# NVlabs/FoundationPose

Hardware: AMD Instinct MI355X
Metric: pose-hypotheses/sec (raster+refine+score), 252 hyp x 160x160 @ 640x480 RGB-D (higher is better)
Workload: dtype f16

## Files before the change

foundationpose_amd/_lib.py:

```python
import ctypes as C
import os

import torch

_HERE = os.path.dirname(os.path.abspath(__file__))
LIB_PATH = os.environ.get("FP_AMD_LIB") or os.path.join(_HERE, "csrc", "libfp_amd.so")
ABI_VERSION = 226
_lib = None

vp, ci, cf, cd, sz = C.c_void_p, C.c_int, C.c_float, C.c_double, C.c_size_t

SIGNATURES = {
    "fp_last_error": (C.c_char_p, []),
    "fp_version": (ci, []),
    "fp_mesh_create": (ci, [vp, vp, vp, vp, vp, vp, vp, ci, ci, ci, ci, C.POINTER(vp)]),
    "fp_mesh_destroy": (None, [vp]),
    "fp_mesh_set_create": (ci, [vp, ci, C.POINTER(vp)]),
    "fp_mesh_set_destroy": (None, [vp]),
    "fp_mesh_set_workspace_bytes": (sz, [vp, ci, ci, ci]),
    "fp_depth_erode": (ci, [vp, vp, ci, ci, ci, cf, cf, cf, vp]),
    "fp_depth_bilateral": (ci, [vp, vp, ci, ci, ci, cf, cf, cf, vp]),
    "fp_depth_to_xyz": (ci, [vp, vp, cf, ci, vp, ci, ci, vp]),
    "fp_crop_windows": (ci, [vp, vp, cd, cd, ci, ci, ci, vp, vp, vp]),
    "fp_crop_windows_multi": (ci, [vp, vp, vp, vp, ci, cd, ci, ci, ci, vp, vp, vp]),
    "fp_depth_erode_frames": (ci, [vp, vp, ci, ci, ci, ci, cf, cf, cf, vp]),
    "fp_depth_bilateral_frames": (ci, [vp, vp, ci, ci, ci, ci, cf, cf, cf, vp]),
    "fp_depth_to_xyz_frames": (ci, [vp, vp, cf, ci, vp, ci, ci, ci, vp]),
    "fp_mask_depth_stats": (ci, [vp, vp, vp, ci, ci, ci, ci, cf, vp, vp]),
    "fp_crop_windows_views": (ci, [vp, vp, vp, ci, vp, vp, ci, cd, ci, ci, ci, vp, vp, vp]),
    "fp_render_crops_views": (ci, [vp, vp, vp, vp, vp, ci, vp, vp, ci, ci, ci, ci, ci, cf, cf, cf, ci, vp, vp, vp, vp, vp, vp, vp, vp, sz, vp]),
    "fp_warp_crops_views": (ci, [vp, vp, vp, vp, vp, vp, ci, vp, vp, vp, ci, ci, ci, ci, ci, ci, ci, ci, vp, vp]),
    "fp_pose_update_views": (ci, [vp, vp, vp, ci, ci, vp, cf, vp, vp, ci, ci, vp, vp, vp, ci, vp, vp, ci, vp, cf, vp]),
    "fp_depth_agreement": (ci, [vp, vp, vp, vp, ci, ci, ci, ci, ci, ci, cf, vp, vp]),
    "fp_icp_workspace_bytes": (sz, [ci, ci, ci]),
    "fp_icp_point_plane": (ci, [vp, vp, vp, vp, vp, ci, ci, ci, vp, ci, ci, ci, cf, cd, ci, vp, vp, vp, sz, vp]),
    "fp_pose_errors_workspace_bytes": (sz, [ci, ci, ci]),
    "fp_pose_errors": (ci, [vp, ci, vp, ci, vp, vp, vp, ci, ci, ci, vp, vp, sz, vp]),
    "fp_vsd_counts": (ci, [vp, vp, vp, ci, ci, ci, ci, vp, vp, ci, ci, ci, ci, cf, vp, ci, vp, vp]),
    "fp_mspd": (ci, [vp, ci, vp, ci, vp, vp, vp, ci, ci, vp, vp, vp]),
    "fp_tsdf_integrate": (ci, [vp, vp, vp, vp, vp, ci, ci, ci, ci, ci, ci, vp, cf, cf, cf, vp, vp, vp, vp, vp]),
    "fp_tsdf_count_triangles": (ci, [vp, vp, ci, ci, ci, cf, vp, vp]),
    "fp_tsdf_emit_triangles": (ci, [vp, vp, vp, vp, ci, ci, ci, vp, cf, cf, vp, C.c_longlong, vp, vp, vp, vp, vp]),
    "fp_texture_bake": (ci, [vp, ci, vp, ci, vp, vp, vp, vp, vp, vp, ci, ci, ci, ci, ci, cf, cf, cf, vp, vp, vp]),
    "fp_workspace_bytes": (sz, [ci, ci, ci, ci, ci]),
    "fp_raster_lds_bytes": (sz, [ci]),
    "fp_render_crops": (ci, [vp, vp, vp, vp, ci, ci, ci, ci, ci, cf, cf, cf, cf, ci, vp, vp, vp, vp, vp, vp, vp, vp, sz, vp]),
    "fp_render_crops_multi": (ci, [vp, vp, vp, vp, vp, vp, ci, ci, ci, ci, ci, cf, cf, cf, ci, vp, vp, vp, vp, vp, vp, vp, vp, sz, vp]),
    "fp_warp_crops": (ci, [vp, vp, vp, vp, vp, vp, cf, ci, ci, ci, ci, ci, ci, ci, vp, vp]),
    "fp_warp_crops_multi": (ci, [vp, vp, vp, vp, vp, vp, vp, vp, ci, ci, ci, ci, ci, ci, ci, ci, vp, vp]),
    "fp_pose_update": (ci, [vp, vp, vp, ci, ci, vp, cf, cf, ci, vp, vp, vp, ci, vp, vp, cf, vp]),
    "fp_pose_update_multi": (ci, [vp, vp, vp, ci, ci, vp, cf, vp, vp, ci, ci, vp, vp, vp, ci, vp, vp, cf, vp]),
    "fp_conv7x7s2_bn_relu_fwd": (ci, [vp, vp, vp, vp, vp, vp, ci, ci, ci, ci, vp]),
    "fp_igemm_f16_fwd": (ci, [vp, vp, vp, vp, vp, ci, ci, ci, ci, vp, vp]),
    "fp_pack_conv3x3_tiles_f16": (ci, [vp, vp, ci, ci, vp]),
    "fp_conv3x3_sw_lds_bytes": (ci, []),
    "fp_igemm_splitk_workspace_bytes": (sz, [ci, ci, ci]),
    "fp_igemm_f16_splitk_fwd": (ci, [vp, vp, vp, vp, vp, ci, ci, ci, ci, vp, ci, vp, sz, vp]),
    "fp_add_pe_f16_fwd": (ci, [vp, vp, vp, ci, ci, ci, vp]),
    "fp_replicate_rows_f16": (ci, [vp, vp, ci, ci, ci, ci, ci, C.c_longlong, vp]),
    "fp_replicate_segments_f16": (ci, [vp, vp, ci, ci, ci, ci, ci, C.c_longlong, vp]),
    "fp_layernorm_res_fwd": (ci, [vp, vp, vp, ci, vp, vp, vp, cf, vp, vp, ci, ci, vp]),
    "fp_pack_linear512_f16": (ci, [vp, vp, vp]),
    "fp_linear512_f16_fwd": (ci, [vp, vp, vp, vp, ci, ci, ci, vp]),
    "fp_linear_layernorm_fwd": (ci, [vp, vp, vp, vp, vp, vp, ci, vp, vp, cf, vp, vp, ci, ci, ci, ci, vp]),
    "fp_ffn_layernorm_mean_fwd": (ci, [vp, vp, vp, vp, vp, vp, vp, vp, cf, vp, vp, C.c_size_t, ci, ci, vp]),
    "fp_encoder_tail_workspace_bytes": (sz, [ci, ci]),
    "fp_encoder_tail_mean_fwd": (ci, [vp, ci, vp, vp, vp, vp, vp, vp, vp, vp, vp, vp, vp, vp, cf, vp, vp, sz, ci, ci, vp]),
    "fp_colmean_f16_fwd": (ci, [vp, vp, vp, vp, cf, vp, ci, ci, ci, vp]),
    "fp_rows_linear_fwd": (ci, [vp, vp, vp, vp, ci, ci, ci, ci, vp]),
    "fp_attention_f16_fwd": (ci, [vp, vp, ci, ci, ci, ci, ci, vp]),
    "fp_attention_segments_f16_fwd": (ci, [vp, vp, vp, ci, ci, ci, ci, ci, vp]),
    "fp_cluster_poses": (ci, [cf, cf, vp, ci, vp, ci, vp]),
}


class FpAmdError(RuntimeError):
    pass


def lib():
    global _lib
    if _lib is None:
        if not os.path.exists(LIB_PATH):
            raise FpAmdError(
                f"{LIB_PATH} is missing: the HIP extension is not built (run __graft_entry__.build() or "
                f"`make -C foundationpose_amd/csrc`). There is no CPU fallback.")
        handle = C.CDLL(LIB_PATH)
        for name, (res, args) in SIGNATURES.items():
            fn = getattr(handle, name)
            fn.restype = res
            fn.argtypes = args
        got = int(handle.fp_version())
        if got != ABI_VERSION:
            raise FpAmdError(f"{LIB_PATH} reports ABI version {got}, this binding was written for {ABI_VERSION}: rebuild the library "
                             f"(`make -C foundationpose_amd/csrc`) -- entry points changed meaning between versions (include/fp_amd.h)")
        _lib = handle
    return _lib


def check(status, what):
    if status != 0:
        msg = lib().fp_last_error()
        raise FpAmdError(f"{what} failed ({status}): {msg.decode() if msg else '?'}")
```

foundationpose_amd/csrc/conv_sw.hip:

```cpp
#include <hip/hip_fp16.h>
#include <stdlib.h>
#include <string.h>
#include <type_traits>
#include "igemm_common.h"
#include "igemm_epilogue.h"

#ifdef FP_PROFILE_BUILD
__device__ unsigned long long sw_dbg[8];
extern "C" int fp_dbg_conv_sw(unsigned long long* out, int reset) {
  if (reset) { unsigned long long z[8] = {0, 0, 0, 0, 0, 0, ~0ull, 0}; return (int)hipMemcpyToSymbol(HIP_SYMBOL(sw_dbg), z, sizeof(z)); }
  return (int)hipMemcpyFromSymbol(out, HIP_SYMBOL(sw_dbg), 8 * sizeof(unsigned long long));
}
extern "C" int fp_dbg_conv_sw_epilogue(unsigned long long* out, int reset) {
  if (reset) { unsigned long long z[8] = {0, 0, 0, 0, 0, 0, 0, 0}; return (int)hipMemcpyToSymbol(HIP_SYMBOL(ig_epi_dbg), z, sizeof(z)); }
  return (int)hipMemcpyFromSymbol(out, HIP_SYMBOL(ig_epi_dbg), 8 * sizeof(unsigned long long));
}
#define SW_CLK(t) const unsigned long long t = wall_clock64()
#else
#define SW_CLK(t)
#endif

#ifndef SW_DEFAULT_VARIANT
#define SW_DEFAULT_VARIANT 0
#endif

namespace {

constexpr int SW_BK = 32, SW_NSTW = 4;
constexpr int sw_prows(int BM) { return BM == 256 ? 512 : 768; }

template <int N>
__device__ __forceinline__ void sw_wait_vm() {
  static_assert(N >= 0 && N < 64, "vmcnt is a 6-bit field");
  asm volatile("s_waitcnt vmcnt(%0)" ::"n"(N) : "memory");
}

typedef float sw_float4 __attribute__((ext_vector_type(4)));
__device__ __forceinline__ void sw_mfma16(sw_float4& acc, const half8& a, const half8& b) {
  asm volatile("v_mfma_f32_16x16x32_f16 %0, %1, %2, %0" : "+v"(acc) : "v"(a), "v"(b));
}

__device__ __forceinline__ int sw_div(int n, unsigned mul, unsigned shr) { return (int)(__umulhi((unsigned)n, mul) >> shr); }

struct SwGeom {
  int HoWo, Wo, Hp, Wp;
  unsigned mulP, shrP, mulW, shrW;
};

template <typename G>
__device__ __forceinline__ int sw_q(const G& g, int m) {
  const int b = sw_div(m, g.mulP, g.shrP);
  const int r = m - b * g.HoWo;
  const int oy = sw_div(r, g.mulW, g.shrW);
  const int ox = r - oy * g.Wo;
  return (b * g.Hp + oy) * g.Wp + ox;
}

template <int BM, int BN, int TM, bool S16>
__global__ __launch_bounds__(512, 1) void k_conv_sw(IgemmParams p) {
  constexpr int BK = SW_BK, NW = 8, THREADS = 512;
  constexpr int NWN = BN / 64;
  static_assert((BM / (32 * TM)) * NWN == NW, "8 waves");
  constexpr int ROWB = BK * 2;
  constexpr int W_BYTES = BN * ROWB;
  constexpr int SW_PROWS = sw_prows(BM);
  constexpr int SW_PATCH_BYTES = SW_PROWS * ROWB;
  constexpr int WI = BN / 16 / NW;
  constexpr int PI = SW_PROWS / 16 / NW;
  static_assert(WI >= 1 && PI >= 1 && PI <= 7 && SW_PROWS == PI * 16 * NW, "tile shape");
  constexpr int STAGES_BYTES = 2 * SW_PATCH_BYTES + SW_NSTW * W_BYTES;
  constexpr int LDS_MAIN = ig_lds_main_slim<BM, BN>(STAGES_BYTES);
  auto swz = [](int row) { return (row >> 2) & 3; };
  auto swzp = [](int row) { return S16 ? (row >> 1) & 2 : (row >> 2) & 3; };
  extern __shared__ __attribute__((aligned(16))) unsigned char smem[];
  SW_CLK(t_start);
  unsigned char* const patch = smem;
  unsigned char* const wring = smem + 2 * SW_PATCH_BYTES;
  const int tid = threadIdx.x, lane = tid & 63;
  const int wid = __builtin_amdgcn_readfirstlane(tid >> 6);
  const int grp = wid >> 2;
  const int wm = wid / NWN, wn = wid - wm * NWN;
  float* bias_lds = reinterpret_cast<float*>(smem + LDS_MAIN);

  const _Float16* A_ = p.A;
  const _Float16* W_ = p.Wt;
  const _Float16* Wpk_ = p.Wpk;
  const float* bias_ = p.bias;
  const float* bnsc_ = p.bn_scale;
  const float* bnsh_ = p.bn_shift;
  const int M = p.M, N = p.N, Cin = p.Cin, cstride = p.in.cstride, coff = p.in.coff;
  const SwGeom gi = {p.in.HoWo, p.in.Wo, p.in.Hp, p.in.Wp, p.in.mulP, p.in.shrP, p.in.mulW, p.in.shrW};
  asm volatile("" ::"s"(A_), "s"(W_), "s"(Wpk_), "s"(bias_), "s"(bnsc_), "s"(bnsh_), "s"(M), "s"(N), "s"(Cin), "s"(cstride), "s"(coff),
               "s"(gi.HoWo), "s"(gi.Wo), "s"(gi.Hp), "s"(gi.Wp), "s"(gi.mulP), "s"(gi.shrP), "s"(gi.mulW), "s"(gi.shrW));
  __builtin_amdgcn_sched_barrier(0);

  const int tiles_n = N / BN;
  const int nwg = (int)(((unsigned)M + BM - 1) / BM) * tiles_n;
  const int xcd = blockIdx.x & 7, loc = blockIdx.x >> 3;
  const int qd8 = nwg >> 3, r8 = nwg & 7;
  const int tile = (xcd < r8 ? xcd * (qd8 + 1) : r8 * (qd8 + 1) + (xcd - r8) * qd8) + loc;
  const int bm = __builtin_popcount(tiles_n) == 1 ? tile >> __builtin_ctz(tiles_n) : tile / tiles_n, bn = tile - bm * tiles_n;
  const int m0 = bm * BM, n0 = bn * BN;
  const int Ktot = 9 * Cin, Wp = gi.Wp;
  const int ncc = Cin / BK;
  ig_bias_to_lds(bias_, bnsc_, bnsh_, N, n0, bias_lds, wid, lane);

  const int q0 = sw_q(gi, m0);
  const int qmax = sw_div(M, gi.mulP, gi.shrP) * gi.Hp * Wp - 1;
  unsigned poff32[PI], woff32[WI];
  {
    const int row0 = wid * PI * 16 + (lane >> 2);
    const int c = (lane & 3) ^ swzp(row0);
    static_assert(((16 >> 1) & 2) == 0 && ((16 >> 2) & 3) == 0, "swzp(row0 + 16 j) == swzp(row0)");
    const unsigned ps2 = (unsigned)cstride * 2, omax = (unsigned)qmax * ps2, lane_off = (unsigned)(coff + c * 8) * 2;
    const unsigned o0 = (unsigned)(q0 + row0) * ps2;
#pragma unroll
    for (int j = 0; j < PI; ++j) {
      const unsigned o = o0 + j * 16 * ps2;
      poff32[j] = (o < omax ? o : omax) + lane_off;
    }
  }
#pragma unroll
  for (int j = 0; j < WI; ++j) {
    const int row = (wid * WI + j) * 16 + (lane >> 2);
    const int c = (lane & 3) ^ swz(row);
    woff32[j] = (unsigned)((((size_t)(n0 + row) * Ktot) + c * 8) * 2);
  }
  const bool wpk = (BN == 128) && Wpk_ != nullptr;
  if (wpk) {
#pragma unroll
    for (int j = 0; j < WI; ++j) woff32[j] = (unsigned)(((wid * WI + j) * 64 + lane) * 16);
  }
  const int wpk_base = wpk ? bn * (ncc * 9) * W_BYTES : 0;
  const __amdgpu_buffer_rsrc_t rsA = __builtin_amdgcn_make_buffer_rsrc(const_cast<_Float16*>(A_), 0, 0x7FFFFFFF, 0x00020000);
  const __amdgpu_buffer_rsrc_t rsW = __builtin_amdgcn_make_buffer_rsrc(const_cast<_Float16*>(wpk ? Wpk_ : W_), 0, 0x7FFFFFFF, 0x00020000);

  auto stage_patch = [&](int cc, int j) {
    unsigned char* dst = patch + (cc & 1) * SW_PATCH_BYTES + (wid * PI + j) * 1024;
    __builtin_amdgcn_raw_ptr_buffer_load_lds(rsA, (__attribute__((address_space(3))) void*)dst, 16, (int)poff32[j],
                                             cc * (BK * 2), 0, 0);
  };
  auto stage_w = [&](int cc, int tap, int slot) {
    const int wsoff = wpk ? wpk_base + (cc * 9 + tap) * W_BYTES : (tap * Cin + cc * BK) * 2;
    unsigned char* dst = wring + slot * W_BYTES + wid * (WI * 1024);
#pragma unroll
    for (int j = 0; j < WI; ++j)
      __builtin_amdgcn_raw_ptr_buffer_load_lds(rsW, (__attribute__((address_space(3))) void*)(dst + j * 1024), 16,
                                               (int)woff32[j], wsoff, 0, 0);
  };

#pragma unroll
  for (int j = 0; j < PI; ++j) stage_patch(0, j);
  stage_w(0, 0, 0);
  stage_w(0, 1, 1);
  stage_w(0, 2, 2);
  __builtin_amdgcn_sched_barrier(0);
  SW_CLK(t_issue);

  constexpr int NFA = S16 ? 2 * TM : TM, NFW = S16 ? 4 : 2;
  constexpr int FR = S16 ? 16 : 32;
  typedef float float4_ __attribute__((ext_vector_type(4)));
  typedef typename std::conditional<S16, float4_, float16_>::type acc_t;
  acc_t acc[NFW][NFA];
#pragma unroll
  for (int i = 0; i < NFW; ++i)
#pragma unroll
    for (int j = 0; j < NFA; ++j)
#pragma unroll
      for (int e = 0; e < (S16 ? 4 : 16); ++e) acc[i][j][e] = 0.f;

  const int frow = lane & (FR - 1), fhalf = lane >> (S16 ? 4 : 5);
  int arow[NFA], w_off[2][2];
#pragma unroll
  for (int t = 0; t < NFA; ++t) {
    int m = m0 + wm * (32 * TM) + t * FR + frow;
    m = m < M ? m : M - 1;
    arow[t] = sw_q(gi, m) - q0;
    if constexpr (S16) arow[t] = (arow[t] << 6) + (fhalf << 4);
  }
  if constexpr (S16) {
    const int quad = (0x1320 >> (4 * (frow >> 2))) & 3;
#pragma unroll
    for (int t = 0; t < 4; ++t) {
      const int rw = wn * 64 + t * 16 + 4 * quad + (frow & 3);
      w_off[t >> 1][t & 1] = rw * ROWB + ((fhalf ^ swz(rw)) << 4);
    }
  } else {
#pragma unroll
    for (int t = 0; t < 2; ++t) {
      const int rw = wn * 64 + t * 32 + frow;
#pragma unroll
      for (int kk = 0; kk < 2; ++kk) w_off[t][kk] = rw * ROWB + (((2 * kk + fhalf) ^ swz(rw)) << 4);
    }
  }
  static_assert(TM == 4, "the fragment addresses of the next tap are computed behind the MFMA groups of a k-step, one per group of four");
  int anext[NFA], aflip[NFA];
#pragma unroll
  for (int t = 0; t < NFA; ++t) {
    anext[t] = S16 ? arow[t] : (arow[t] << 6) + ((fhalf ^ swz(arow[t])) << 4);
    aflip[t] = S16 ? (arow[t] >> 3) & 32 : 0;
  }

#pragma unroll
  for (int t = 0; t < NFA; ++t) {
    asm volatile("" : "+v"(arow[t]), "+v"(anext[t]));
    if constexpr (S16) asm volatile("" : "+v"(aflip[t]));
  }
  asm volatile("" : "+v"(w_off[0][0]), "+v"(w_off[0][1]), "+v"(w_off[1][0]), "+v"(w_off[1][1]));
#pragma unroll
  for (int i = 0; i < NFW; ++i)
#pragma unroll
    for (int j = 0; j < NFA; ++j) asm volatile("" : "+v"(acc[i][j]));
  __builtin_amdgcn_sched_barrier(0);

  sw_wait_vm<2 * WI>();
  __builtin_amdgcn_s_barrier();
  SW_CLK(t_cold);
  if (grp) __builtin_amdgcn_s_barrier();

  half8 fa[2][TM], fw[2][2];
  auto kstep = [&](int cc, auto tap_c, auto last_c) {
    constexpr int T = decltype(tap_c)::value;
    constexpr bool LAST = decltype(last_c)::value;
    constexpr int ky = T / 3, kx = T - 3 * ky;
    const int s = cc * 9 + T;
    const unsigned char* pb = patch + (cc & 1) * SW_PATCH_BYTES;
    const unsigned char* wb = wring + (s & (SW_NSTW - 1)) * W_BYTES;
    const int shift = ky * Wp + kx;
    if constexpr (S16) {
#pragma unroll
      for (int t = 0; t < NFA; ++t) fa[t >> 2][t & 3] = *reinterpret_cast<const half8*>(pb + (anext[t] ^ aflip[t]));
#pragma unroll
      for (int t = 0; t < 4; ++t) fw[t >> 1][t & 1] = *reinterpret_cast<const half8*>(wb + w_off[t >> 1][t & 1]);
    } else {
#pragma unroll
      for (int t = 0; t < TM; ++t) {
        const int a0 = anext[t];
        fa[0][t] = *reinterpret_cast<const half8*>(pb + a0);
        fa[1][t] = *reinterpret_cast<const half8*>(pb + (a0 ^ 32));
      }
#pragma unroll
      for (int kk = 0; kk < 2; ++kk)
#pragma unroll
        for (int t = 0; t < 2; ++t) fw[kk][t] = *reinterpret_cast<const half8*>(wb + w_off[t][kk]);
    }
    (void)shift;
    if constexpr (!LAST) {
      if constexpr (T < PI) stage_patch(cc + 1, T);
      if constexpr (T + 3 < 9) stage_w(cc, T + 3, (s + 3) & (SW_NSTW - 1));
      else stage_w(cc + 1, T - 6, (s + 3) & (SW_NSTW - 1));
      constexpr int NP = (T < PI ? 1 : 0) + ((T >= 1 && T - 1 < PI) ? 1 : 0);
      sw_wait_vm<2 * WI + NP>();
    } else {
      if constexpr (T + 3 < 9) stage_w(cc, T + 3, (s + 3) & (SW_NSTW - 1));
      constexpr int NYOUNGER = T <= 5 ? 2 : (T == 6 ? 1 : 0);
      sw_wait_vm<NYOUNGER * WI>();
    }
    asm volatile("s_waitcnt lgkmcnt(0)" ::: "memory");
    __builtin_amdgcn_sched_barrier(0);
    __builtin_amdgcn_s_barrier();
    __builtin_amdgcn_sched_barrier(0);
    __builtin_amdgcn_s_setprio(1);
    {
      constexpr int TN = (T + 1) % 9, kyn = TN / 3, kxn = TN - 3 * kyn;
      const int shift_n = kyn * Wp + kxn;
      if constexpr (S16) {
        int sh = shift_n << 6;
        asm volatile("" : "+s"(sh));
#pragma unroll
        for (int i = 0; i < 4; ++i)
#pragma unroll
          for (int jh = 0; jh < 2; ++jh) {
            const int t = i * 2 + jh;
            int x, y;
            sw_mfma16(acc[i][jh * 4 + 0], fw[i >> 1][i & 1], fa[jh][0]);
            asm volatile("v_add_u32 %0, %1, %2" : "=v"(x) : "s"(sh), "v"(arow[t]));
            sw_mfma16(acc[i][jh * 4 + 1], fw[i >> 1][i & 1], fa[jh][1]);
            asm volatile("v_lshrrev_b32 %0, 3, %1" : "=v"(y) : "v"(x));
            sw_mfma16(acc[i][jh * 4 + 2], fw[i >> 1][i & 1], fa[jh][2]);
            asm volatile("v_and_b32 %0, 32, %0" : "+v"(y));
            sw_mfma16(acc[i][jh * 4 + 3], fw[i >> 1][i & 1], fa[jh][3]);
            anext[t] = x; aflip[t] = y;
          }
      } else {
#pragma unroll
      for (int kk = 0; kk < 2; ++kk)
#pragma unroll
        for (int i = 0; i < 2; ++i) {
#pragma unroll
          for (int j = 0; j < TM; ++j)
            acc[i][j] = __builtin_amdgcn_mfma_f32_32x32x16_f16(fw[kk][i], fa[kk][j], acc[i][j], 0, 0, 0);
          const int t = kk * 2 + i;
          {
            int ar = arow[t];
            asm volatile("" : "+v"(ar));
            const int pr = ar + shift_n;
            anext[t] = (pr << 6) + ((fhalf ^ swz(pr)) << 4);
          }
        }
      }
    }
    __builtin_amdgcn_s_setprio(0);
    __builtin_amdgcn_sched_barrier(0);
    __builtin_amdgcn_s_barrier();
    __builtin_amdgcn_sched_barrier(0);
  };
  auto chunk = [&](int cc, auto last_c) {
    kstep(cc, std::integral_constant<int, 0>{}, last_c);
    kstep(cc, std::integral_constant<int, 1>{}, last_c);
    kstep(cc, std::integral_constant<int, 2>{}, last_c);
    kstep(cc, std::integral_constant<int, 3>{}, last_c);
    kstep(cc, std::integral_constant<int, 4>{}, last_c);
    kstep(cc, std::integral_constant<int, 5>{}, last_c);
    kstep(cc, std::integral_constant<int, 6>{}, last_c);
    kstep(cc, std::integral_constant<int, 7>{}, last_c);
    kstep(cc, std::integral_constant<int, 8>{}, last_c);
  };
  for (int cc = 0; cc + 1 < ncc; ++cc) chunk(cc, std::false_type{});
  chunk(ncc - 1, std::true_type{});
  if (!grp) __builtin_amdgcn_s_barrier();
  __syncthreads();
  SW_CLK(t_loop);
  ig_epilogue<BM, BN, TM, THREADS, 0, true>(p, acc, smem, m0, n0, wm, wn, tid, lane, bias_lds);
#ifdef FP_PROFILE_BUILD
  asm volatile("s_waitcnt vmcnt(0)" ::: "memory");
  SW_CLK(t_end);
  if (tid == 0) {
    atomicAdd(&sw_dbg[0], t_cold - t_start); atomicAdd(&sw_dbg[1], t_loop - t_cold); atomicAdd(&sw_dbg[2], t_end - t_loop);
    atomicAdd(&sw_dbg[3], 1ull); atomicAdd(&sw_dbg[4], t_issue - t_start); atomicMin(&sw_dbg[6], t_start); atomicMax(&sw_dbg[7], t_end);
  }
#endif
}

constexpr int LS_PROWS = 448, LS_NSTW = 3;

template <int BM, int BN, int TM>
__global__ __launch_bounds__(256, 2) void k_conv_sw_ls(IgemmParams p) {
  constexpr int BK = SW_BK, NW = 4, THREADS = 256;
  constexpr int NWN = BN / 64;
  static_assert((BM / (32 * TM)) * NWN == NW, "4 waves");
  constexpr int ROWB = BK * 2;
  constexpr int W_BYTES = BN * ROWB;
  constexpr int PATCH_BYTES = LS_PROWS * ROWB;
  constexpr int WI = BN / 16 / NW;
  constexpr int PI = LS_PROWS / 16 / NW;
  static_assert(WI >= 1 && PI >= 1 && PI <= 8 && LS_PROWS == PI * 16 * NW, "tile shape");
  constexpr int STAGES_BYTES = 2 * PATCH_BYTES + LS_NSTW * W_BYTES;
  static_assert(STAGES_BYTES >= BM * BN * 2 + BM * 16 + IG_BIAS_LDS, "the epilogue tile, its tables and the vectors reuse the staging area");
  auto swz = [](int row) { return (row >> 2) & 3; };
  extern __shared__ __attribute__((aligned(16))) unsigned char smem[];
  unsigned char* const patch = smem;
  unsigned char* const wring = smem + 2 * PATCH_BYTES;
  const int tid = threadIdx.x, lane = tid & 63;
  const int wid = __builtin_amdgcn_readfirstlane(tid >> 6);
  const int wm = wid / NWN, wn = wid - wm * NWN;

  const int tiles_n = p.N / BN;
  const int nwg = gridDim.x;
  const int xcd = blockIdx.x & 7, loc = blockIdx.x >> 3;
  const int qd8 = nwg >> 3, r8 = nwg & 7;
  const int tile = (xcd < r8 ? xcd * (qd8 + 1) : r8 * (qd8 + 1) + (xcd - r8) * qd8) + loc;
  const int bm = tile / tiles_n, bn = tile - bm * tiles_n;
  const int m0 = bm * BM, n0 = bn * BN;
  const int Cin = p.Cin, Ktot = 9 * Cin, Wp = p.in.Wp;
  const int ncc = Cin / BK;

  const int q0 = sw_q(p.in, m0);
  const int qmax = (p.M / p.in.HoWo) * p.in.Hp * Wp - 1;
  unsigned poff32[PI], woff32[WI];
#pragma unroll
  for (int j = 0; j < PI; ++j) {
    const int row = (wid * PI + j) * 16 + (lane >> 2);
    const int c = (lane & 3) ^ swz(row);
    int q = q0 + row;
    q = q < qmax ? q : qmax;
    poff32[j] = (unsigned)(((long long)q * p.in.cstride + p.in.coff + c * 8) * 2);
  }
#pragma unroll
  for (int j = 0; j < WI; ++j) {
    const int row = (wid * WI + j) * 16 + (lane >> 2);
    const int c = (lane & 3) ^ swz(row);
    woff32[j] = (unsigned)((((size_t)(n0 + row) * Ktot) + c * 8) * 2);
  }
  const __amdgpu_buffer_rsrc_t rsA = __builtin_amdgcn_make_buffer_rsrc(const_cast<_Float16*>(p.A), 0, 0x7FFFFFFF, 0x00020000);
  const __amdgpu_buffer_rsrc_t rsW = __builtin_amdgcn_make_buffer_rsrc(const_cast<_Float16*>(p.Wt), 0, 0x7FFFFFFF, 0x00020000);

  auto stage_patch = [&](int cc, int j) {
    unsigned char* dst = patch + (cc & 1) * PATCH_BYTES + (wid * PI + j) * 1024;
    __builtin_amdgcn_raw_ptr_buffer_load_lds(rsA, (__attribute__((address_space(3))) void*)dst, 16, (int)poff32[j],
                                             cc * (BK * 2), 0, 0);
  };
  auto stage_w = [&](int cc, int tap, int slot) {
    const int wsoff = (tap * Cin + cc * BK) * 2;
    unsigned char* dst = wring + slot * W_BYTES + wid * (WI * 1024);
#pragma unroll
    for (int j = 0; j < WI; ++j)
      __builtin_amdgcn_raw_ptr_buffer_load_lds(rsW, (__attribute__((address_space(3))) void*)(dst + j * 1024), 16,
                                               (int)woff32[j], wsoff, 0, 0);
  };

  float16_ acc[2][TM];
#pragma unroll
  for (int i = 0; i < 2; ++i)
#pragma unroll
    for (int j = 0; j < TM; ++j)
#pragma unroll
      for (int e = 0; e < 16; ++e) acc[i][j][e] = 0.f;

  const int frow = lane & 31, fhalf = lane >> 5;
  int arow[TM], w_off[2][2];
#pragma unroll
  for (int t = 0; t < TM; ++t) {
    int m = m0 + wm * (32 * TM) + t * 32 + frow;
    m = m < p.M ? m : p.M - 1;
    arow[t] = sw_q(p.in, m) - q0;
  }
#pragma unroll
  for (int t = 0; t < 2; ++t) {
    const int rw = wn * 64 + t * 32 + frow;
#pragma unroll
    for (int kk = 0; kk < 2; ++kk) w_off[t][kk] = rw * ROWB + (((2 * kk + fhalf) ^ swz(rw)) << 4);
  }

#pragma unroll
  for (int j = 0; j < PI; ++j) stage_patch(0, j);
  stage_w(0, 0, 0);
  stage_w(0, 1, 1);

  auto kstep = [&](int cc, auto tap_c, auto last_c, auto first_c) {
    constexpr int T = decltype(tap_c)::value;
    constexpr bool LAST = decltype(last_c)::value;
    constexpr bool FIRST = decltype(first_c)::value;
    constexpr int ky = T / 3, kx = T - 3 * ky;
    {
      constexpr bool prev_w = FIRST || T == 0 || !LAST || (T - 1) + 2 < 9;
      constexpr bool prev_p = !FIRST && T >= 1 && !LAST && (T - 1) < PI;
      sw_wait_vm<(prev_w ? WI : 0) + (prev_p ? 1 : 0)>();
    }
    __builtin_amdgcn_sched_barrier(0);
    __builtin_amdgcn_s_barrier();
    __builtin_amdgcn_sched_barrier(0);
    if constexpr (!LAST) {
      if constexpr (T < PI) stage_patch(cc + 1, T);
      if constexpr (T + 2 < 9) stage_w(cc, T + 2, (T + 2) % LS_NSTW);
      else stage_w(cc + 1, T - 7, (T + 2) % LS_NSTW);
    } else {
      if constexpr (T + 2 < 9) stage_w(cc, T + 2, (T + 2) % LS_NSTW);
    }
    const unsigned char* pb = patch + (cc & 1) * PATCH_BYTES;
    const unsigned char* wb = wring + (T % LS_NSTW) * W_BYTES;
    const int shift = ky * Wp + kx;
    half8 fa[2][TM], fw[2][2];
    int a0[TM];
#pragma unroll
    for (int t = 0; t < TM; ++t) {
      int ar = arow[t];
      asm volatile("" : "+v"(ar));
      const int pr = ar + shift;
      a0[t] = (pr << 6) + ((fhalf ^ swz(pr)) << 4);
    }
#pragma unroll
    for (int t = 0; t < TM; ++t) fa[0][t] = *reinterpret_cast<const half8*>(pb + a0[t]);
#pragma unroll
    for (int t = 0; t < 2; ++t) fw[0][t] = *reinterpret_cast<const half8*>(wb + w_off[t][0]);
#pragma unroll
    for (int t = 0; t < TM; ++t) fa[1][t] = *reinterpret_cast<const half8*>(pb + (a0[t] ^ 32));
#pragma unroll
    for (int t = 0; t < 2; ++t) fw[1][t] = *reinterpret_cast<const half8*>(wb + w_off[t][1]);
    __builtin_amdgcn_sched_barrier(0);
#pragma unroll
    for (int kk = 0; kk < 2; ++kk)
#pragma unroll
      for (int i = 0; i < 2; ++i)
#pragma unroll
        for (int j = 0; j < TM; ++j)
          acc[i][j] = __builtin_amdgcn_mfma_f32_32x32x16_f16(fw[kk][i], fa[kk][j], acc[i][j], 0, 0, 0);
    __builtin_amdgcn_sched_barrier(0);
  };
  auto chunk = [&](int cc, auto last_c, auto first_c) {
    kstep(cc, std::integral_constant<int, 0>{}, last_c, first_c);
    kstep(cc, std::integral_constant<int, 1>{}, last_c, std::false_type{});
    kstep(cc, std::integral_constant<int, 2>{}, last_c, std::false_type{});
    kstep(cc, std::integral_constant<int, 3>{}, last_c, std::false_type{});
    kstep(cc, std::integral_constant<int, 4>{}, last_c, std::false_type{});
    kstep(cc, std::integral_constant<int, 5>{}, last_c, std::false_type{});
    kstep(cc, std::integral_constant<int, 6>{}, last_c, std::false_type{});
    kstep(cc, std::integral_constant<int, 7>{}, last_c, std::false_type{});
    kstep(cc, std::integral_constant<int, 8>{}, last_c, std::false_type{});
  };
  chunk(0, std::false_type{}, std::true_type{});
  for (int cc = 1; cc + 1 < ncc; ++cc) chunk(cc, std::false_type{}, std::false_type{});
  chunk(ncc - 1, std::true_type{}, std::false_type{});
  __syncthreads();
  float* bias_lds = reinterpret_cast<float*>(smem + BM * BN * 2 + BM * 16);
  ig_bias_to_lds(p, n0, bias_lds, wid, lane);
  asm volatile("s_waitcnt vmcnt(0)" ::: "memory");
  ig_epilogue<BM, BN, TM, THREADS, 0>(p, acc, smem, m0, n0, wm, wn, tid, lane, bias_lds);
}

template <int BM, int BN, int TM>
int sw_ls_launch(const IgemmParams& p, hipStream_t stream) {
  constexpr int LDS = 2 * LS_PROWS * SW_BK * 2 + LS_NSTW * BN * SW_BK * 2;
  static_assert(2 * LDS <= 160 * 1024, "two workgroups per CU");
  const long long tiles = (long long)fp_cdiv(p.M, BM) * (p.N / BN);
  FP_REQUIRE(tiles < (1ll << 31), "fp_igemm_f16_fwd: too many tiles");
  FP_SET_MAX_LDS((k_conv_sw_ls<BM, BN, TM>), LDS);
  hipLaunchKernelGGL((k_conv_sw_ls<BM, BN, TM>), dim3((unsigned)tiles), dim3(256), LDS, stream, p);
  FP_CHECK_LAUNCH("fp_igemm_f16_fwd(conv_sw_ls)");
  return FP_OK;
}

constexpr int sw_lds_bytes(int BM, int BN) {
  return (BM == 256 ? ig_lds_main_slim<256, 256>(2 * sw_prows(256) * SW_BK * 2 + SW_NSTW * 256 * SW_BK * 2)
                    : ig_lds_main_slim<512, 128>(2 * sw_prows(512) * SW_BK * 2 + SW_NSTW * 128 * SW_BK * 2)) + IG_BIAS_LDS;
}

template <int BM, int BN, int TM, bool S16>
int sw_launch(const IgemmParams& p, hipStream_t stream) {
  static_assert((BM == 256 && BN == 256) || (BM == 512 && BN == 128), "tile shapes of sw_lds_bytes");
  constexpr int LDS = sw_lds_bytes(BM, BN);
  static_assert(LDS <= 160 * 1024, "does not fit the 160 KiB LDS");
  const long long tiles = (long long)fp_cdiv(p.M, BM) * (p.N / BN);
  FP_REQUIRE(tiles < (1ll << 31), "fp_igemm_f16_fwd: too many tiles");
  FP_SET_MAX_LDS((k_conv_sw<BM, BN, TM, S16>), LDS);
  hipLaunchKernelGGL((k_conv_sw<BM, BN, TM, S16>), dim3((unsigned)tiles), dim3(512), LDS, stream, p);
  FP_CHECK_LAUNCH("fp_igemm_f16_fwd(conv_sw)");
  return FP_OK;
}

}

static int sw_span(const IgemmGeom& g, int BM) {
  const int row_cross = (BM - 1) / g.Wo + 1, img_cross = (BM - 1) / g.HoWo + 1;
  return (BM - 1) + 2 * row_cross + (2 * g.Wp + 2) * img_cross + 2 * g.Wp + 3;
}

static int sw_variant(const IgemmParams& p) {
  int v = SW_DEFAULT_VARIANT;
#ifdef FP_PROFILE_BUILD
  static int forced = -2;
  if (forced == -2) {
    const char* e = getenv("FP_CONV_SW");
    forced = e ? (!strcmp(e, "ls") ? 1 : (!strcmp(e, "pp") ? 0 : -1)) : -1;
  }
  if (forced >= 0) v = forced;
#endif
  if (v == 2) v = p.Cin <= 128 ? 1 : 0;
  if (v == 3) v = p.Cin <= 256 ? 1 : 0;
  if (v == 1 && sw_span(p.in, 256) > LS_PROWS) v = 0;
  return v;
}

#ifndef SW_FORCE_512
#define SW_FORCE_512 1
#endif
static bool sw_use_256(const IgemmParams& p) { return (p.N % 256) == 0 && (!SW_FORCE_512 || p.M < 2 * 512); }
static int sw_tile_rows(const IgemmParams& p) { return sw_variant(p) == 1 ? 256 : (sw_use_256(p) ? 256 : 512); }

bool fp_conv3x3_sw_applicable(const IgemmParams& p) {
  const IgemmGeom& g = p.in;
  if (p.taps != 9 || g.stride != 1 || g.off != 0 || g.bsplit != 0) return false;
  if (g.HoWo % g.Wo != 0 || g.Wp != g.Wo + 2 || g.Hp != g.HoWo / g.Wo + 2) return false;
  if (g.Wo < 2) return false;
  const int BM = sw_tile_rows(p);
  if (p.M % g.HoWo != 0 || p.M < 2 * BM) return false;
  if (p.Cin % 64 != 0 || p.N % 128 != 0) return false;
  const long long bytes = (long long)(p.M / g.HoWo) * g.Hp * g.Wp * g.cstride * 2;
  if (bytes >= (1ll << 31)) return false;
  if (g.cstride >= (1 << 19)) return false;
  const IgemmGeom& o = p.out;
  const long long imgs = o.bsplit > 0 ? o.bsplit : p.M / g.HoWo, groups = o.bsplit > 0 ? (p.M / g.HoWo) / o.bsplit + 1 : 0;
  if (imgs * o.Hp * o.Wp * o.cstride + o.coff + groups * (long long)o.cgroup >= (1ll << 31)) return false;
  if (p.R) {
    const IgemmGeom& r = p.res;
    const long long rimgs = r.bsplit > 0 ? r.bsplit : p.M / g.HoWo, rgroups = r.bsplit > 0 ? (p.M / g.HoWo) / r.bsplit + 1 : 0;
    if (rimgs * r.Hp * r.Wp * r.cstride + r.coff + rgroups * (long long)r.cgroup >= (1ll << 31)) return false;
  }
  return sw_span(g, BM) <= (sw_variant(p) == 1 ? LS_PROWS : sw_prows(BM));
}

int fp_conv3x3_sw_tile_rows(const IgemmParams& p) { return sw_tile_rows(p); }

extern "C" int fp_conv3x3_sw_lds_bytes(void) { return sw_lds_bytes(512, 128); }

int fp_conv3x3_sw_launch(const IgemmParams& p, hipStream_t stream) {
  if (sw_variant(p) == 1) return sw_ls_launch<256, 128, 4>(p, stream);
  if (sw_use_256(p)) return p.mfma16 ? sw_launch<256, 256, 4, true>(p, stream) : sw_launch<256, 256, 4, false>(p, stream);
  return p.mfma16 ? sw_launch<512, 128, 4, true>(p, stream) : sw_launch<512, 128, 4, false>(p, stream);
}

__global__ __launch_bounds__(256) void k_pack_conv3x3_tiles(const _Float16* __restrict__ w, _Float16* __restrict__ out, int N, int Cin) {
  const int nk = 9 * (Cin / 32);
  const long long total = (long long)N * nk * 4;
  const long long q = (long long)blockIdx.x * 256 + threadIdx.x;
  if (q >= total) return;
  const int pc = (int)(q & 3);
  const int r = (int)((q >> 2) & 127);
  const long long blk = q >> 9;
  const int s = (int)(blk % nk), bn = (int)(blk / nk);
  const int cc = s / 9, tap = s - 9 * cc;
  const int lc = pc ^ ((r >> 2) & 3);
  const half8 v = *reinterpret_cast<const half8*>(w + (size_t)(bn * 128 + r) * (9 * Cin) + tap * Cin + cc * 32 + lc * 8);
  *reinterpret_cast<half8*>(out + q * 8) = v;
}

extern "C" int fp_pack_conv3x3_tiles_f16(const void* w, void* w_tiles, int N, int Cin, void* stream) {
  FP_REQUIRE(w && w_tiles && w != w_tiles, "fp_pack_conv3x3_tiles_f16: NULL tensor or in-place repack");
  FP_REQUIRE(N > 0 && N % 128 == 0 && Cin > 0 && Cin % 32 == 0, "fp_pack_conv3x3_tiles_f16: N=%d must be a multiple of 128, Cin=%d of 32", N, Cin);
  FP_REQUIRE((((size_t)w | (size_t)w_tiles) & 15) == 0, "fp_pack_conv3x3_tiles_f16: tensors must be 16-byte aligned");
  const long long total = (long long)N * 9 * (Cin / 32) * 4;
  hipLaunchKernelGGL(k_pack_conv3x3_tiles, dim3((unsigned)((total + 255) / 256)), dim3(256), 0, (hipStream_t)stream, (const _Float16*)w,
                     (_Float16*)w_tiles, N, Cin);
  FP_CHECK_LAUNCH("fp_pack_conv3x3_tiles_f16");
  return FP_OK;
}
```

foundationpose_amd/csrc/igemm.hip:

```cpp
#include <hip/hip_fp16.h>
#include <stdlib.h>
#include <string.h>
#include "igemm_common.h"
#include "igemm_epilogue.h"

int fp_igemm_pp_launch(const IgemmParams& p, int variant, hipStream_t stream);
int fp_conv3x3_sw_launch(const IgemmParams& p, hipStream_t stream);
bool fp_conv3x3_sw_applicable(const IgemmParams& p);
int fp_conv3x3_sw_tile_rows(const IgemmParams& p);

template <int BM, int BN, int TM, int NST, int BK, bool SPLITK = false>
__global__ __launch_bounds__((BM / (32 * TM)) * (BN / 64) * 64, ((BM / (32 * TM)) * (BN / 64) == 4 && TM == 4) ? 2 : 1) void k_igemm_f16(IgemmParams p) {
  constexpr int NWN = BN / 64;
  constexpr int NW = (BM / (32 * TM)) * NWN;
  constexpr int THREADS = NW * 64;
  constexpr int ROWB = BK * 2;
  constexpr int CPK = BK / 8;
  constexpr int RPI = 1024 / ROWB;
  constexpr int KK = BK / 16;
  constexpr int A_BYTES = BM * ROWB;
  constexpr int STAGE_BYTES = A_BYTES + BN * ROWB;
  constexpr int AI = BM / RPI / NW;
  constexpr int WI = BN / RPI / NW;
  static_assert(AI >= 1 && WI >= 1, "tile too small for this wave count");
// ... 163 lines not shown
  typedef _Float16 half2_ __attribute__((ext_vector_type(2)));
  const size_t t = (size_t)blockIdx.x * 256 + threadIdx.x;
  const int lane = (int)(t & 63);
  size_t q = t >> 6;
  const int j = (int)(q % TM); q /= TM;
  const int g = (int)(q & 3); q >>= 2;
  const int i = (int)(q & 1); q >>= 1;
  const int wid = (int)(q % NW);
  const int tile = (int)(q / NW);
  if (tile >= ntiles) return;
  const int tiles_n = p.N / BN;
  const int bm = tile / tiles_n, bn = tile - bm * tiles_n;
  const int wm = wid / NWN, wn = wid - wm * NWN;
  const int m = bm * BM + wm * (32 * TM) + j * 32 + (lane & 31);
  const int n = bn * BN + wn * 64 + i * 32 + 8 * g + 4 * (lane >> 5);
  if (m >= p.M) return;
  const float4_* src = reinterpret_cast<const float4_*>(p.slab) + t;
  const size_t per_split = (size_t)ntiles * NW * (8 * TM) * 64;
  float4_ a = src[0];
  for (int s = 1; s < p.nsplit; ++s) {
    const float4_ b = src[(size_t)s * per_split];
    a[0] += b[0]; a[1] += b[1]; a[2] += b[2]; a[3] += b[3];
  }
  float4_ bv = {0.f, 0.f, 0.f, 0.f};
  if (p.bias) bv = *reinterpret_cast<const float4_*>(p.bias + n);
  half4 v;
  if (p.round_acc) {
    const half2_ b01 = {(_Float16)bv[0], (_Float16)bv[1]}, b23 = {(_Float16)bv[2], (_Float16)bv[3]};
    half2_ t01 = {(_Float16)a[0], (_Float16)a[1]};
    half2_ t23 = {(_Float16)a[2], (_Float16)a[3]};
    t01 = t01 + b01;
    t23 = t23 + b23;
    if (p.bn_scale) {
      const float4_ sc = *reinterpret_cast<const float4_*>(p.bn_scale + n), sh = *reinterpret_cast<const float4_*>(p.bn_shift + n);
      v[0] = (_Float16)fmaf((float)t01[0], sc[0], sh[0]);
      v[1] = (_Float16)fmaf((float)t01[1], sc[1], sh[1]);
      v[2] = (_Float16)fmaf((float)t23[0], sc[2], sh[2]);
      v[3] = (_Float16)fmaf((float)t23[1], sc[3], sh[3]);
    } else {
      v[0] = t01[0]; v[1] = t01[1]; v[2] = t23[0]; v[3] = t23[1];
    }
  } else {
#pragma unroll
    for (int e = 0; e < 4; ++e) v[e] = (_Float16)(a[e] + bv[e]);
  }
  if (p.R) v = v + *reinterpret_cast<const half4*>(p.R + ig_row_off(p.res, m) + n);
  if (p.relu) {
    const half4 zero = {0, 0, 0, 0};
    v = __builtin_elementwise_max(v, zero);
  }
  *reinterpret_cast<half4*>(p.Y + ig_row_off(p.out, m) + n) = v;
  if (p.Ype) {
    const float4_ e0 = *reinterpret_cast<const float4_*>(p.pe + (size_t)(m % p.pe_period) * p.N + n);
    half4 w;
#pragma unroll
    for (int e = 0; e < 4; ++e) w[e] = (_Float16)((float)v[e] + e0[e]);
    *reinterpret_cast<half4*>(p.Ype + (size_t)m * p.N + n) = w;
  }
}

constexpr int SK_BM = 128, SK_BN = 128, SK_TM = 2, SK_NST = 2, SK_BK = 64;
static size_t ig_splitk_bytes(int M, int N, int splits) {
  return (size_t)splits * fp_cdiv(M, SK_BM) * (N / SK_BN) * (size_t)(SK_BM * SK_BN * 4);
}
static int ig_launch_splitk(const IgemmParams& p, hipStream_t stream) {
  constexpr int LDS = ig_lds_main<SK_BM, SK_BN>(SK_NST * (SK_BM + SK_BN) * SK_BK * 2) + IG_BIAS_LDS;
  const long long tiles = (long long)fp_cdiv(p.M, SK_BM) * (p.N / SK_BN);
  FP_REQUIRE(tiles * p.nsplit < (1ll << 31) && p.nsplit <= 65535, "fp_igemm_f16_splitk_fwd: too many tiles");
  FP_SET_MAX_LDS((k_igemm_f16<SK_BM, SK_BN, SK_TM, SK_NST, SK_BK, true>), LDS);
  hipLaunchKernelGGL((k_igemm_f16<SK_BM, SK_BN, SK_TM, SK_NST, SK_BK, true>), dim3((unsigned)tiles, (unsigned)p.nsplit), dim3(256), LDS, stream, p);
  FP_CHECK_LAUNCH("fp_igemm_f16_splitk_fwd(partial products)");
  const long long threads = tiles * 4 * (8 * SK_TM) * 64;
  hipLaunchKernelGGL((k_splitk_epilogue<SK_BM, SK_BN, SK_TM>), dim3((unsigned)((threads + 255) / 256)), dim3(256), 0, stream, p, (int)tiles);
  FP_CHECK_LAUNCH("fp_igemm_f16_splitk_fwd(reduce + epilogue)");
  return FP_OK;
}

static int ig_check_geom(const fp_igemm_geom* g, const char* what, const char* who) {
  FP_REQUIRE(g->pixels_per_image > 0 && g->width > 0 && g->padded_h > 0 && g->padded_w > 0 && g->cstride > 0 &&
                 g->stride > 0 && g->offset >= 0 && g->coff >= 0 && g->bsplit >= 0,
             "%s: bad %s geometry", who, what);
  FP_REQUIRE((g->cstride % 8) == 0 && (g->coff % 8) == 0 && (g->cgroup % 8) == 0,
             "%s: %s channel stride/offset must be multiples of 8 (16-byte rows)", who, what);
  return FP_OK;
}

static IgemmGeom ig_geom(const fp_igemm_geom* g) {
  IgemmGeom o;
  o.HoWo = g->pixels_per_image; o.Wo = g->width; o.Hp = g->padded_h; o.Wp = g->padded_w; o.stride = g->stride;
  o.off = g->offset; o.cstride = g->cstride; o.coff = g->coff; o.bsplit = g->bsplit; o.cgroup = g->cgroup;
  ig_fastdiv_init(o.HoWo, &o.mulP, &o.shrP);
  ig_fastdiv_init(o.Wo, &o.mulW, &o.shrW);
  ig_fastdiv_init(o.bsplit, &o.mulB, &o.shrB);
  return o;
}

static int ig_dispatch(IgemmParams& p, hipStream_t stream) {
  int sel = 0;
#ifdef FP_PROFILE_BUILD
  static int forced = -1;
  if (forced < 0) {
    const char* e = getenv("FP_IGEMM_TILE");
    forced = 0;
    if (e) {
      if (!strcmp(e, "128x128")) forced = 1;
      else if (!strcmp(e, "256x128")) forced = 2;
      else if (!strcmp(e, "256x256")) forced = 3;
      else if (!strcmp(e, "ls256x128")) forced = 4;
      else if (!strcmp(e, "pp256x256")) forced = 7;
      else if (!strcmp(e, "pp256x128")) forced = 9;
      else if (!strcmp(e, "generic")) forced = 100;
    }
  }
  sel = forced;
#endif
  const bool sw = sel == 0 && fp_conv3x3_sw_applicable(p);
  if (sel >= 100) sel = 0;
  if (!sw && sel == 0) {
    const bool wide = (p.N % 256) == 0;
    const bool pp = wide && (p.M >= 150000 || p.N >= 1024 || (p.taps == 9 && p.Cin >= 256) || (p.taps == 1 && p.M < 75000 && p.M >= 4096));
    sel = pp ? 7 : 1;
    if ((p.taps == 9 && p.in.stride == 2 && p.Cin <= 64) || (p.taps == 1 && p.N >= 1024)) sel = 4;
  }
  if (sel == 3 && (p.N % 256) != 0) sel = 2;
  if (sel == 7 && (p.N % 256) != 0) sel = 9;
  if (sw) return fp_conv3x3_sw_launch(p, stream);
  if (sel >= 7) return fp_igemm_pp_launch(p, sel - 7, stream);
#ifdef FP_PROFILE_BUILD
  if (sel == 2) return ig_launch<256, 128, 2, 3, 64>(p, stream);
  if (sel == 3) return ig_launch<256, 256, 4, 2, 64>(p, stream);
#endif
  if (sel == 4) return ig_launch<256, 128, 4, 3, 32>(p, stream);
  return ig_launch<128, 128, 2, 2, 64>(p, stream);
}


static int ig_epilogue_mode(const IgemmParams& p, int flags) {
  if (flags & FP_IGEMM_EPILOGUE_GENERIC) return 0;
  if (!p.round_acc || !p.bias || !p.relu || (p.Ype && !p.R)) return 0;
  return IG_EPI_CONV | (p.bn_scale ? IG_EPI_BN : 0) | (p.R ? IG_EPI_RES : 0) | (p.Ype ? IG_EPI_PE : 0);
}

static int ig_build_params(const void* x, const fp_igemm_geom* x_geom, const void* w, void* y, const fp_igemm_geom* y_geom,
                           int M, int N, int Cin, int taps, const fp_igemm_epilogue* ep, IgemmParams& p, const char* who) {
  FP_REQUIRE(x && w && y && x_geom && y_geom, "%s: NULL tensor / geometry", who);
  FP_REQUIRE(taps == 1 || taps == 9, "%s: taps must be 1 (GEMM) or 9 (3x3 conv), got %d", who, taps);
  FP_REQUIRE(N > 0 && N % 128 == 0, "%s: N=%d must be a multiple of 128", who, N);
  FP_REQUIRE(Cin > 0 && Cin % 64 == 0, "%s: Cin=%d must be a multiple of 64", who, Cin);
  static const fp_igemm_epilogue no_epilogue = {nullptr, nullptr, nullptr, nullptr, nullptr, 0, nullptr, 0, nullptr, nullptr};
  const fp_igemm_epilogue& e = ep ? *ep : no_epilogue;
  FP_REQUIRE(!e.residual || e.r_geom, "%s: residual without geometry", who);
  FP_REQUIRE((e.bn_scale == nullptr) == (e.bn_shift == nullptr), "%s: bn_scale and bn_shift go together", who);
  FP_REQUIRE(!e.bn_scale || (e.flags & FP_IGEMM_ROUND_ACC), "%s: BatchNorm needs FP_IGEMM_ROUND_ACC (conv semantics)", who);
  FP_REQUIRE((e.flags & ~(FP_IGEMM_RELU | FP_IGEMM_ROUND_ACC | FP_IGEMM_HAS_W_TILES | FP_IGEMM_MFMA_16X16X32 | FP_IGEMM_MFMA_32X32X16 | FP_IGEMM_EPILOGUE_GENERIC)) == 0,
             "%s: unknown flags 0x%x", who, e.flags);
  FP_REQUIRE((e.flags & (FP_IGEMM_MFMA_16X16X32 | FP_IGEMM_MFMA_32X32X16)) != (FP_IGEMM_MFMA_16X16X32 | FP_IGEMM_MFMA_32X32X16),
             "%s: FP_IGEMM_MFMA_16X16X32 and FP_IGEMM_MFMA_32X32X16 exclude each other", who);
  FP_REQUIRE((e.pe == nullptr) == (e.y_pe == nullptr) && (!e.pe || e.pe_period > 0), "%s: pe, pe_period and y_pe go together", who);
  FP_REQUIRE((((size_t)x | (size_t)w | (size_t)y | (size_t)e.residual | (size_t)e.bias | (size_t)e.bn_scale | (size_t)e.bn_shift |
               (size_t)e.pe | (size_t)e.y_pe) & 15) == 0, "%s: tensors must be 16-byte aligned", who);
  if (int err = ig_check_geom(x_geom, "input", who)) return err;
  if (int err = ig_check_geom(y_geom, "output", who)) return err;
  if (e.residual) if (int err = ig_check_geom(e.r_geom, "residual", who)) return err;
  const void* w_tiles = (e.flags & FP_IGEMM_HAS_W_TILES) ? e.w_tiles : nullptr;
  FP_REQUIRE(!w_tiles || (taps == 9 && (((size_t)w_tiles) & 15) == 0 && w_tiles != w), "%s: w_tiles is for 3x3 convolutions, 16-byte aligned, not w itself", who);
  p.A = (const _Float16*)x; p.Wt = (const _Float16*)w; p.Wpk = (const _Float16*)w_tiles; p.bias = e.bias; p.bn_scale = e.bn_scale; p.bn_shift = e.bn_shift;
  p.R = (const _Float16*)e.residual; p.Y = (_Float16*)y;
  p.pe = e.pe; p.Ype = (_Float16*)e.y_pe; p.pe_period = e.pe_period;
  p.M = M; p.N = N; p.Cin = Cin; p.taps = taps; p.relu = (e.flags & FP_IGEMM_RELU) ? 1 : 0;
  p.round_acc = (e.flags & FP_IGEMM_ROUND_ACC) ? 1 : 0;
  p.mfma16 = (e.flags & FP_IGEMM_MFMA_32X32X16) ? 0 : ((e.flags & FP_IGEMM_MFMA_16X16X32) ? 1 : SW_DEFAULT_MFMA16);
  p.in = ig_geom(x_geom); p.out = ig_geom(y_geom); p.res = e.residual ? ig_geom(e.r_geom) : ig_geom(y_geom);
  p.slab = nullptr; p.nsplit = 0;
  p.epi = ig_epilogue_mode(p, e.flags);
  ig_fastdiv_init(p.pe_period, &p.pe_mul, &p.pe_shr);
  return FP_OK;
}

extern "C" int fp_igemm_f16_fwd(const void* x, const fp_igemm_geom* x_geom, const void* w, void* y, const fp_igemm_geom* y_geom,
                                int M, int N, int Cin, int taps, const fp_igemm_epilogue* ep, void* stream) {
  FP_REQUIRE(M >= 0, "fp_igemm_f16_fwd: M < 0");
  if (M == 0) return FP_OK;
  IgemmParams p;
  if (int err = ig_build_params(x, x_geom, w, y, y_geom, M, N, Cin, taps, ep, p, "fp_igemm_f16_fwd")) return err;
  return ig_dispatch(p, (hipStream_t)stream);
}

extern "C" size_t fp_igemm_splitk_workspace_bytes(int M, int N, int splits) {
  if (M <= 0 || N <= 0 || N % SK_BN != 0 || splits <= 0) return 0;
  return ig_splitk_bytes(M, N, splits);
}

extern "C" int fp_igemm_f16_splitk_fwd(const void* x, const fp_igemm_geom* x_geom, const void* w, void* y, const fp_igemm_geom* y_geom,
                                       int M, int N, int Cin, int taps, const fp_igemm_epilogue* ep, int splits, void* workspace,
                                       size_t workspace_bytes, void* stream) {
  FP_REQUIRE(M >= 0, "fp_igemm_f16_splitk_fwd: M < 0");
  if (M == 0) return FP_OK;
  IgemmParams p;
  if (int err = ig_build_params(x, x_geom, w, y, y_geom, M, N, Cin, taps, ep, p, "fp_igemm_f16_splitk_fwd")) return err;
  FP_REQUIRE(!p.Wpk, "fp_igemm_f16_splitk_fwd: w_tiles is the operand layout of the shifted-window kernel; the split-K kernels do not take it");
  const int nk = taps * (Cin / SK_BK);
  FP_REQUIRE(splits >= 1 && splits <= nk, "fp_igemm_f16_splitk_fwd: splits=%d must be in [1, %d] (k-steps of 64)", splits, nk);
  const size_t need = ig_splitk_bytes(M, N, splits);
  if (!workspace || workspace_bytes < need || ((size_t)workspace & 15)) {
    fp_set_error("fp_igemm_f16_splitk_fwd: workspace too small or unaligned (%zu < %zu bytes, see fp_igemm_splitk_workspace_bytes)", workspace_bytes, need);
    return FP_ERR_WORKSPACE;
  }
  p.slab = (float*)workspace; p.nsplit = splits;
  return ig_launch_splitk(p, (hipStream_t)stream);
}
```

foundationpose_amd/csrc/igemm_common.h:

```cpp
#pragma once
#include <hip/hip_fp16.h>
#include <stddef.h>
#include "fp_common.h"

typedef _Float16 half8 __attribute__((ext_vector_type(8)));
typedef _Float16 half4 __attribute__((ext_vector_type(4)));
typedef float float16_ __attribute__((ext_vector_type(16)));

#define IG_BK 64
#ifndef SW_DEFAULT_MFMA16
#define SW_DEFAULT_MFMA16 1
#endif

struct IgemmGeom {
  int HoWo, Wo;
  int Hp, Wp;
  int stride;
  int off;
  int cstride;
  int coff;
  int bsplit;
  int cgroup;
  unsigned mulP, shrP;
  unsigned mulW, shrW;
  unsigned mulB, shrB;
};

static inline void ig_fastdiv_init(int d, unsigned* mul, unsigned* shr) {
  if (d <= 1) { *mul = 0; *shr = 0; return; }
  int lg = 0;
  while ((1u << lg) < (unsigned)d) ++lg;
  const int p = 31 + lg;
  *mul = (unsigned)(((1ull << p) + (unsigned)d - 1) / (unsigned)d);
  *shr = (unsigned)(p - 32);
}
__device__ __forceinline__ int ig_fastdiv(int n, unsigned mul, unsigned shr) {
  return mul ? (int)(__umulhi((unsigned)n, mul) >> shr) : n;
}

struct IgemmParams {
  const _Float16* A;
  const _Float16* Wt;
  const _Float16* Wpk;
  const float* bias;
  const float* bn_scale;
  const float* bn_shift;
  int M, N, Cin, taps;
  IgemmGeom in;
  IgemmGeom out, res;
  const _Float16* R;
  _Float16* Y;
  const float* pe;
  _Float16* Ype;
  int pe_period;
  int relu;
  int round_acc;
  int mfma16;
  int epi;
  unsigned pe_mul, pe_shr;
  float* slab;
  int nsplit;
};
static_assert(sizeof(IgemmGeom) == 64 && offsetof(IgemmParams, in) == 64 && offsetof(IgemmParams, out) == 128, "the head of IgemmParams is its first 128 bytes");

#define IG_EPI_SPEC 1
#define IG_EPI_ROUND_ACC 2
#define IG_EPI_BIAS 4
#define IG_EPI_BN 8
#define IG_EPI_RES 16
#define IG_EPI_RELU 32
#define IG_EPI_PE 64
#define IG_EPI_CONV (IG_EPI_SPEC | IG_EPI_ROUND_ACC | IG_EPI_BIAS | IG_EPI_RELU)

__device__ __forceinline__ long long ig_row_off(const IgemmGeom& g, int m) {
  const int b = ig_fastdiv(m, g.mulP, g.shrP);
  const int r = m - b * g.HoWo;
  const int oy = ig_fastdiv(r, g.mulW, g.shrW);
  const int ox = r - oy * g.Wo;
  int bb = b, cg = 0;
  if (g.bsplit > 0) { cg = ig_fastdiv(b, g.mulB, g.shrB); bb = b - cg * g.bsplit; }
  return (((long long)bb * g.Hp + (oy * g.stride + g.off)) * g.Wp + (ox * g.stride + g.off)) * g.cstride + g.coff +
         (long long)cg * g.cgroup;
}
```

foundationpose_amd/csrc/igemm_epilogue.h:

```cpp
#pragma once
#include <type_traits>
#include "igemm_common.h"

#ifdef FP_PROFILE_BUILD
static __device__ unsigned long long ig_epi_dbg[8];
#define IG_CLK(t) const unsigned long long t = wall_clock64()
#else
#define IG_CLK(t)
#endif

#define IG_VEC_FLOATS 256
#define IG_BIAS_LDS (3 * IG_VEC_FLOATS * 4)

template <int BM, int BN>
constexpr int ig_lds_main(int stage_bytes) {
  return stage_bytes > BM * BN * 2 + BM * 16 ? stage_bytes : BM * BN * 2 + BM * 16;
}

template <int BM, int BN>
constexpr int ig_lds_main_slim(int stage_bytes) {
  return stage_bytes > BM * BN * 2 + BM * 4 ? stage_bytes : BM * BN * 2 + BM * 4;
}
#define IG_ROW_NONE ((int)0x80000000)

typedef float ig_float4 __attribute__((ext_vector_type(4)));
struct IgEpiArgs {
  IgemmGeom out, res;
  const _Float16* R;
  _Float16* Y;
  const float* pe;
  _Float16* Ype;
  int pe_period;
  unsigned pe_mul, pe_shr;
  int N;
};

template <typename T>
__device__ __forceinline__ T* ig_uniform_ptr(const T* ptr) {
  const unsigned long long a = reinterpret_cast<unsigned long long>(ptr);
  const unsigned lo = __builtin_amdgcn_readfirstlane((unsigned)a), hi = __builtin_amdgcn_readfirstlane((unsigned)(a >> 32));
  return reinterpret_cast<T*>(((unsigned long long)hi << 32) | lo);
}

__device__ __forceinline__ half8 ig_relu8(const half8& v) {
  typedef _Float16 half2_ __attribute__((ext_vector_type(2)));
  half8 r;
#pragma unroll
  for (int e = 0; e < 4; ++e) {
    const half2_ x = {v[2 * e], v[2 * e + 1]};
    half2_ y;
    asm("v_pk_max_f16 %0, %1, 0" : "=v"(y) : "v"(x));
    r[2 * e] = y[0]; r[2 * e + 1] = y[1];
  }
  return r;
}

template <int BM, int BN, int TM, int THREADS, bool SLIM, int EPI, typename Acc>
__device__ __forceinline__ void ig_epilogue_spec(const IgEpiArgs& p, Acc& acc, unsigned char* smem, int m0, int n0,
                                                 int wm, int wn, int tid, int lane, const float* bias_lds) {
  constexpr bool S16 = std::is_same<Acc, ig_float4[4][2 * TM]>::value;
  static_assert(S16 || std::is_same<Acc, float16_[2][TM]>::value, "accumulator layout");
  static_assert((EPI & IG_EPI_SPEC) && (EPI & IG_EPI_BIAS), "a layer kind with a bias");
  constexpr bool ROUND_ACC = (EPI & IG_EPI_ROUND_ACC) != 0, HAS_BN = (EPI & IG_EPI_BN) != 0, RES = (EPI & IG_EPI_RES) != 0;
  constexpr bool RELU = (EPI & IG_EPI_RELU) != 0, PE = (EPI & IG_EPI_PE) != 0;
  static_assert(ROUND_ACC || !HAS_BN, "BatchNorm follows the conv rounding");
  constexpr int CPR = BN / 8;
  constexpr int NIT = (BM * CPR) / THREADS;
  constexpr int RPI = THREADS / CPR;
  static_assert(THREADS % CPR == 0 && RPI % 16 == 0 && NIT * RPI == BM, "the store loop's swizzle term must not depend on the iteration");
  constexpr int ROWB = 2 * BN;
  typedef float float4_ __attribute__((ext_vector_type(4)));
  typedef _Float16 half2_ __attribute__((ext_vector_type(2)));
  typedef unsigned uint4_ __attribute__((ext_vector_type(4)));
  unsigned char* E = smem;
  long long* rowY = reinterpret_cast<long long*>(smem + BM * ROWB);
  long long* rowR = SLIM ? reinterpret_cast<long long*>(smem) : rowY + BM;
  int* rowY32 = reinterpret_cast<int*>(smem + BM * ROWB);
  const long long baseY = SLIM ? ig_row_off(p.out, m0) + n0 : 0;
  IG_CLK(te0);
  for (int r = tid; r < BM; r += THREADS) {
    const int m = m0 + r;
    if constexpr (SLIM) rowY32[r] = (int)(ig_row_off(p.out, m) + n0 - baseY);
    else rowY[r] = ig_row_off(p.out, m) + n0;
    if constexpr (RES) rowR[r] = ig_row_off(p.res, m) + n0;
  }
  __syncthreads();
  IG_CLK(te1);
  const int ml0 = tid / CPR, ch = tid % CPR;
  half8 rv[RES ? NIT : 1];
  constexpr int NRG = S16 ? 4 : 8;
  static_assert(NIT % NRG == 0, "residual loads per channel group");
  unsigned roff[RES && SLIM ? NIT : 1];
  const __amdgpu_buffer_rsrc_t rsR = __builtin_amdgcn_make_buffer_rsrc(ig_uniform_ptr(p.R), 0, -1, 0x00020000);
  auto res_group = [&](int g) {
    if constexpr (RES && SLIM) {
#pragma unroll
      for (int it = g * (NIT / NRG); it < (g + 1) * (NIT / NRG); ++it)
        rv[it] = __builtin_bit_cast(half8, __builtin_amdgcn_raw_buffer_load_b128(rsR, (int)roff[it], 0, 0));
      __builtin_amdgcn_sched_barrier(0);
    }
  };
  if constexpr (RES) {
    if constexpr (SLIM) {
      const int* rR = reinterpret_cast<const int*>(rowR + ml0);
#pragma unroll
      for (int it = 0; it < NIT; ++it) roff[it] = ((unsigned)rR[it * RPI * 2] + ch * 8) << 1;
      __builtin_amdgcn_sched_barrier(0);
      asm volatile("s_waitcnt lgkmcnt(0)" ::: "memory");
      __builtin_amdgcn_s_barrier();
      __builtin_amdgcn_sched_barrier(0);
    } else {
      const long long* rR = rowR + ml0;
#pragma unroll
      for (int it = 0; it < NIT; ++it) rv[it] = *reinterpret_cast<const half8*>(p.R + rR[it * RPI] + ch * 8);
    }
  }
  IG_CLK(te2);
  struct Vecs { float4_ bv, sc, sh; half2_ b01, b23; };
  auto vecs = [&](int nl) {
    Vecs c;
    c.bv = *reinterpret_cast<const float4_*>(bias_lds + nl);
    c.b01 = half2_{(_Float16)c.bv[0], (_Float16)c.bv[1]};
    c.b23 = half2_{(_Float16)c.bv[2], (_Float16)c.bv[3]};
    if constexpr (HAS_BN) {
      c.sc = *reinterpret_cast<const float4_*>(bias_lds + IG_VEC_FLOATS + nl);
      c.sh = *reinterpret_cast<const float4_*>(bias_lds + 2 * IG_VEC_FLOATS + nl);
    }
    return c;
  };
  auto put4 = [&](unsigned char* dst, float a0, float a1, float a2, float a3, const Vecs& c) {
    half4 v;
    if constexpr (ROUND_ACC) {
      half2_ t01 = {(_Float16)a0, (_Float16)a1};
      half2_ t23 = {(_Float16)a2, (_Float16)a3};
      t01 = t01 + c.b01;
      t23 = t23 + c.b23;
      if constexpr (HAS_BN) {
        v[0] = (_Float16)fmaf((float)t01[0], c.sc[0], c.sh[0]);
        v[1] = (_Float16)fmaf((float)t01[1], c.sc[1], c.sh[1]);
        v[2] = (_Float16)fmaf((float)t23[0], c.sc[2], c.sh[2]);
        v[3] = (_Float16)fmaf((float)t23[1], c.sc[3], c.sh[3]);
      } else {
        v[0] = t01[0]; v[1] = t01[1]; v[2] = t23[0]; v[3] = t23[1];
      }
    } else {
      v[0] = (_Float16)(a0 + c.bv[0]); v[1] = (_Float16)(a1 + c.bv[1]); v[2] = (_Float16)(a2 + c.bv[2]); v[3] = (_Float16)(a3 + c.bv[3]);
    }
    *reinterpret_cast<half4*>(dst) = v;
  };
  const int r15 = lane & 15;
  if constexpr (S16) {
    const int quad = (0x1320 >> (4 * (lane >> 4))) & 3;
    unsigned char* Erow = E + (wm * (32 * TM) + r15) * ROWB + ((quad & 1) << 3);
    const int cx = (wn * 8 + (quad >> 1)) ^ r15;
#pragma unroll
    for (int i = 0; i < 4; ++i) {
      res_group(i);
      const Vecs c = vecs(wn * 64 + i * 16 + 4 * quad);
      unsigned char* Ei = Erow + ((cx ^ (2 * i)) << 4);
#pragma unroll
      for (int j = 0; j < 2 * TM; ++j) put4(Ei + j * (16 * ROWB), acc[i][j][0], acc[i][j][1], acc[i][j][2], acc[i][j][3], c);
    }
  } else {
    unsigned char* Erow = E + (wm * (32 * TM) + (lane & 31)) * ROWB + ((lane >> 5) << 3);
    const int cx = (wn * 8) ^ r15;
#pragma unroll
    for (int i = 0; i < 2; ++i) {
#pragma unroll
      for (int g = 0; g < 4; ++g) {
        res_group(i * 4 + g);
        const Vecs c = vecs(wn * 64 + i * 32 + 8 * g + 4 * (lane >> 5));
        unsigned char* Ei = Erow + ((cx ^ (4 * i + g)) << 4);
#pragma unroll
        for (int j = 0; j < TM; ++j)
          put4(Ei + j * (32 * ROWB), acc[i][j][g * 4 + 0], acc[i][j][g * 4 + 1], acc[i][j][g * 4 + 2], acc[i][j][g * 4 + 3], c);
      }
    }
  }
  __syncthreads();
  IG_CLK(te3);
  const unsigned char* Erd = E + ml0 * ROWB + ((ch ^ (ml0 & 15)) << 4);
  const __amdgpu_buffer_rsrc_t rsY = __builtin_amdgcn_make_buffer_rsrc(ig_uniform_ptr(p.Y), 0, -1, 0x00020000);
  const unsigned cbY = ((unsigned)baseY + ch * 8) << 1;
#pragma unroll
  for (int it = 0; it < NIT; ++it) {
    half8 v = *reinterpret_cast<const half8*>(Erd + it * (RPI * ROWB));
    if constexpr (RES) v = v + rv[it];
    if constexpr (RELU) v = ig_relu8(v);
    if constexpr (SLIM) __builtin_amdgcn_raw_buffer_store_b128(__builtin_bit_cast(uint4_, v), rsY, (int)(cbY + ((unsigned)rowY32[ml0 + it * RPI] << 1)), 0, 0);
    else *reinterpret_cast<half8*>(p.Y + rowY[ml0 + it * RPI] + ch * 8) = v;
    if constexpr (PE) {
      const int m = m0 + ml0 + it * RPI;
      const int mp = m - ig_fastdiv(m, p.pe_mul, p.pe_shr) * p.pe_period;
      const float* per = p.pe + (size_t)mp * p.N + n0 + ch * 8;
      const float4_ e0 = *reinterpret_cast<const float4_*>(per), e1 = *reinterpret_cast<const float4_*>(per + 4);
      half8 w;
#pragma unroll
      for (int e = 0; e < 4; ++e) { w[e] = (_Float16)((float)v[e] + e0[e]); w[4 + e] = (_Float16)((float)v[4 + e] + e1[e]); }
      *reinterpret_cast<half8*>(p.Ype + (size_t)m * p.N + n0 + ch * 8) = w;
      __builtin_amdgcn_sched_barrier(0);
    }
  }
#ifdef FP_PROFILE_BUILD
  IG_CLK(te4);
  if (tid == 0) {
    atomicAdd(&ig_epi_dbg[0], te1 - te0); atomicAdd(&ig_epi_dbg[1], te2 - te1); atomicAdd(&ig_epi_dbg[2], te3 - te2);
    atomicAdd(&ig_epi_dbg[3], te4 - te3); atomicAdd(&ig_epi_dbg[4], 1ull);
  }
#endif
}
template <int BM, int BN, int TM, int THREADS, int DBG, bool FULL, bool SLIM, int EPI = 0, typename Acc, typename P>
__device__ __forceinline__ void ig_epilogue_body(const P& p, Acc& acc, unsigned char* smem, int m0, int n0,
                                                 int wm, int wn, int tid, int lane, const float* bias_lds) {
  if constexpr (EPI != 0) {
    static_assert(FULL && std::is_same<P, IgEpiArgs>::value, "the layer-kind bodies take whole tiles and their own argument block");
    ig_epilogue_spec<BM, BN, TM, THREADS, SLIM, EPI>(p, acc, smem, m0, n0, wm, wn, tid, lane, bias_lds);
  } else {
  static_assert(std::is_same<P, IgemmParams>::value, "the generic body reads IgemmParams");
  constexpr bool S16 = std::is_same<Acc, ig_float4[4][2 * TM]>::value;
  static_assert(S16 || std::is_same<Acc, float16_[2][TM]>::value, "accumulator layout");
  constexpr int CPR = BN / 8;
  constexpr int NIT = (BM * CPR) / THREADS;
  unsigned char* E = smem;
  typedef float float4_ __attribute__((ext_vector_type(4)));
  const bool round_acc = p.round_acc != 0, has_bn = p.bn_scale != nullptr;
  long long* rowY = reinterpret_cast<long long*>(smem + BM * 2 * BN);
  long long* rowR = SLIM ? reinterpret_cast<long long*>(smem) : rowY + BM;
  int* rowY32 = reinterpret_cast<int*>(smem + BM * 2 * BN);
  const long long baseY = SLIM ? ig_row_off(p.out, m0) + n0 : 0;
  auto row_exists = [&](int ml) { return SLIM ? rowY32[ml] != IG_ROW_NONE : rowY[ml] >= 0; };
  IG_CLK(te0);
  for (int r = tid; r < BM; r += THREADS) {
    const int m = m0 + r;
    const bool in = m < p.M;
    if constexpr (SLIM) rowY32[r] = in ? (int)(ig_row_off(p.out, m) + n0 - baseY) : IG_ROW_NONE;
    else rowY[r] = in ? ig_row_off(p.out, m) + n0 : -1;
    if (p.R) rowR[r] = in ? ig_row_off(p.res, m) + n0 : 0;
  }
  __syncthreads();
  IG_CLK(te1);
  half8 rv[NIT];
  if (p.R) {
#pragma unroll
    for (int it = 0; it < NIT; ++it) {
      const int qd = tid + it * THREADS;
      const int ml = qd / CPR, ch = qd % CPR;
      if (FULL || row_exists(ml)) rv[it] = *reinterpret_cast<const half8*>(p.R + rowR[ml] + ch * 8);
    }
    if constexpr (SLIM) {
      __builtin_amdgcn_sched_barrier(0);
      asm volatile("s_waitcnt lgkmcnt(0)" ::: "memory");
      __builtin_amdgcn_s_barrier();
      __builtin_amdgcn_sched_barrier(0);
    }
  }
  IG_CLK(te2);
  auto put4 = [&](int nl, int ml, float a0, float a1, float a2, float a3, const float4_& bv, const float4_& sc, const float4_& sh) {
    half4 v;
    if (round_acc) {
      typedef _Float16 half2_ __attribute__((ext_vector_type(2)));
      const half2_ b01 = {(_Float16)bv[0], (_Float16)bv[1]}, b23 = {(_Float16)bv[2], (_Float16)bv[3]};
      half2_ t01 = {(_Float16)a0, (_Float16)a1};
      half2_ t23 = {(_Float16)a2, (_Float16)a3};
      t01 = t01 + b01;
      t23 = t23 + b23;
      if (has_bn) {
        v[0] = (_Float16)fmaf((float)t01[0], sc[0], sh[0]);
        v[1] = (_Float16)fmaf((float)t01[1], sc[1], sh[1]);
        v[2] = (_Float16)fmaf((float)t23[0], sc[2], sh[2]);
        v[3] = (_Float16)fmaf((float)t23[1], sc[3], sh[3]);
      } else {
        v[0] = t01[0]; v[1] = t01[1]; v[2] = t23[0]; v[3] = t23[1];
      }
    } else {
      v[0] = (_Float16)(a0 + bv[0]); v[1] = (_Float16)(a1 + bv[1]); v[2] = (_Float16)(a2 + bv[2]); v[3] = (_Float16)(a3 + bv[3]);
    }
    const int chunk = (nl >> 3) ^ (ml & 15);
    *reinterpret_cast<half4*>(E + ml * (2 * BN) + (chunk << 4) + ((nl & 4) << 1)) = v;
  };
  auto vecs = [&](int nl, float4_& bv, float4_& sc, float4_& sh) {
    bv = *reinterpret_cast<const float4_*>(bias_lds + nl);
    sc = float4_{1.f, 1.f, 1.f, 1.f}; sh = float4_{0.f, 0.f, 0.f, 0.f};
    if (has_bn) {
      sc = *reinterpret_cast<const float4_*>(bias_lds + IG_VEC_FLOATS + nl);
      sh = *reinterpret_cast<const float4_*>(bias_lds + 2 * IG_VEC_FLOATS + nl);
    }
  };
  if constexpr (S16) {
    const int quad = (0x1320 >> (4 * (lane >> 4))) & 3;
#pragma unroll
    for (int i = 0; i < 4; ++i) {
      const int nl = wn * 64 + i * 16 + 4 * quad;
      float4_ bv, sc, sh;
      vecs(nl, bv, sc, sh);
#pragma unroll
      for (int j = 0; j < 2 * TM; ++j) {
        const int ml = wm * (32 * TM) + j * 16 + (lane & 15);
        put4(nl, ml, acc[i][j][0], acc[i][j][1], acc[i][j][2], acc[i][j][3], bv, sc, sh);
      }
    }
  } else {
#pragma unroll
    for (int i = 0; i < 2; ++i) {
#pragma unroll
      for (int g = 0; g < 4; ++g) {
        const int nl = wn * 64 + i * 32 + 8 * g + 4 * (lane >> 5);
        float4_ bv, sc, sh;
        vecs(nl, bv, sc, sh);
#pragma unroll
        for (int j = 0; j < TM; ++j) {
          const int ml = wm * (32 * TM) + j * 32 + (lane & 31);
          put4(nl, ml, acc[i][j][g * 4 + 0], acc[i][j][g * 4 + 1], acc[i][j][g * 4 + 2], acc[i][j][g * 4 + 3], bv, sc, sh);
        }
      }
    }
  }
  __syncthreads();
  IG_CLK(te3);
  const half8 zero = {0, 0, 0, 0, 0, 0, 0, 0};
#pragma unroll
  for (int it = 0; it < NIT; ++it) {
    const int qd = tid + it * THREADS;
    const int ml = qd / CPR, ch = qd % CPR;
    if (!FULL && !row_exists(ml)) continue;
    const long long yo = SLIM ? baseY + rowY32[ml] : rowY[ml];
    half8 v = *reinterpret_cast<const half8*>(E + ml * (2 * BN) + ((ch ^ (ml & 15)) << 4));
    if (p.R) v = v + rv[it];
    if (p.relu) v = __builtin_elementwise_max(v, zero);
    *reinterpret_cast<half8*>(p.Y + yo + ch * 8) = v;
    if (p.Ype) {
      const int m = m0 + ml;
      const float* per = p.pe + (size_t)(m % p.pe_period) * p.N + n0 + ch * 8;
      const float4_ e0 = *reinterpret_cast<const float4_*>(per), e1 = *reinterpret_cast<const float4_*>(per + 4);
      half8 w;
#pragma unroll
      for (int e = 0; e < 4; ++e) { w[e] = (_Float16)((float)v[e] + e0[e]); w[4 + e] = (_Float16)((float)v[4 + e] + e1[e]); }
      *reinterpret_cast<half8*>(p.Ype + (size_t)m * p.N + n0 + ch * 8) = w;
    }
  }
#ifdef FP_PROFILE_BUILD
  IG_CLK(te4);
  if (tid == 0) {
    atomicAdd(&ig_epi_dbg[0], te1 - te0); atomicAdd(&ig_epi_dbg[1], te2 - te1); atomicAdd(&ig_epi_dbg[2], te3 - te2);
    atomicAdd(&ig_epi_dbg[3], te4 - te3); atomicAdd(&ig_epi_dbg[4], 1ull);
  }
#endif
  }
}

template <int BM, int BN, int TM, int THREADS, int DBG = 0, bool SLIM = false, typename Acc>
__device__ __forceinline__ void ig_epilogue(const IgemmParams& p, Acc& acc, unsigned char* smem, int m0, int n0,
                                            int wm, int wn, int tid, int lane, const float* bias_lds) {
  if (m0 + BM <= p.M) {
    if constexpr (DBG == 0) {
#define IG_EPI_CASE(E) case E: ig_epilogue_body<BM, BN, TM, THREADS, DBG, true, SLIM, E>(q, acc, smem, m0, n0, wm, wn, tid, lane, bias_lds); return
      const IgEpiArgs q = {p.out, p.res, p.R, p.Y, p.pe, p.Ype, p.pe_period, p.pe_mul, p.pe_shr, p.N};
      switch (p.epi) {
        IG_EPI_CASE(IG_EPI_CONV);
        IG_EPI_CASE(IG_EPI_CONV | IG_EPI_RES);
        IG_EPI_CASE(IG_EPI_CONV | IG_EPI_RES | IG_EPI_PE);
        IG_EPI_CASE(IG_EPI_CONV | IG_EPI_BN);
        IG_EPI_CASE(IG_EPI_CONV | IG_EPI_BN | IG_EPI_RES);
        IG_EPI_CASE(IG_EPI_CONV | IG_EPI_BN | IG_EPI_RES | IG_EPI_PE);
// ... 25 lines not shown
```

foundationpose_amd/engine.py:

```python
import contextlib

import torch
import torch.nn.functional as F

from . import ops

USE_MIOPEN = False


FUSED_OUT_PROJ_LN = True


FUSED_FFN = True


ROWS_QKV = True
ROWS_QKV_MIN_ROWS = 4096
PACKED_CONV_TILES = True
MERGED_HEAD_QKV = True
FUSED_TAIL = True
CONV_MFMA_16X16X32 = True
SPECIALIZED_EPILOGUE = True


def _conv_backend():
    if USE_MIOPEN or not torch.backends.cudnn.is_available():
        return contextlib.nullcontext()
    return torch.backends.cudnn.flags(enabled=False)


def _bn_affine(sd, bn_p):
    if bn_p is None or (bn_p + ".weight") not in sd:
        return None, None
    scale = sd[bn_p + ".weight"].float() / torch.sqrt(sd[bn_p + ".running_var"].float() + 1e-5)
    shift = sd[bn_p + ".bias"].float() - sd[bn_p + ".running_mean"].float() * scale
    return scale.contiguous(), shift.contiguous()


def _r16(t):
    return t.to(torch.float16).to(torch.float32).contiguous()


class _Conv:

    def __init__(self, sd, conv_p, bn_p, stride, dtype, channels_last):
        w = sd[conv_p + ".weight"].float()
        b = sd.get(conv_p + ".bias")
        b = torch.zeros(w.shape[0], device=w.device) if b is None else b.float()
        scale, shift = _bn_affine(sd, bn_p)
        if scale is not None:
            w, b = w * scale[:, None, None, None], b * scale + shift
        wf = w.to(dtype)
        self.w = wf.contiguous(memory_format=torch.channels_last) if channels_last else wf.contiguous()
        self.b = b.to(dtype)
        self.stride = stride
        self.pad = (w.shape[-1] - 1) // 2

    def __call__(self, x, relu=True):
        y = F.conv2d(x, self.w, self.b, stride=self.stride, padding=self.pad)
        return F.relu_(y) if relu else y


class _Block:
    def __init__(self, sd, p, dtype, cl):
        self.c1 = _Conv(sd, p + ".conv1", p + ".bn1", 1, dtype, cl)
        self.c2 = _Conv(sd, p + ".conv2", p + ".bn2", 1, dtype, cl)

    def __call__(self, x):
        y = self.c2(self.c1(x), relu=False)
        y += x
        return F.relu_(y)


class _Encoder:

    def __init__(self, sd, stem, joint, dtype, channels_last):
        cl = channels_last
        self.dtype, self.cl = dtype, cl
        self.c1 = _Conv(sd, stem + ".0.net.0", stem + ".0.net.1", 2, dtype, cl)
        self.c2 = _Conv(sd, stem + ".1.net.0", stem + ".1.net.1", 2, dtype, cl)
        self.s2, self.s3 = _Block(sd, stem + ".2", dtype, cl), _Block(sd, stem + ".3", dtype, cl)
        self.j0, self.j1 = _Block(sd, joint + ".0", dtype, cl), _Block(sd, joint + ".1", dtype, cl)
        self.j2 = _Conv(sd, joint + ".2.net.0", joint + ".2.net.1", 2, dtype, cl)
        self.j3, self.j4 = _Block(sd, joint + ".3", dtype, cl), _Block(sd, joint + ".4", dtype, cl)
        self.pe = sd["pos_embed.pe"].to(dtype)

    def __call__(self, AB):
        n = AB.shape[0] // 2
        if self.cl:
            AB = AB.contiguous(memory_format=torch.channels_last)
        x = self.s3(self.s2(self.c2(self.c1(AB))))
        ab = torch.cat((x[:n], x[n:]), dim=1)
        ab = self.j4(self.j3(self.j2(self.j1(self.j0(ab)))))
        tok = ab.permute(0, 2, 3, 1).reshape(n, -1, ab.shape[1])
        return tok + self.pe[:, : tok.shape[1]]


class _TorchMHA:

    def __init__(self, sd, p, dtype, nhead=4):
        self.wi, self.bi = sd[p + ".in_proj_weight"].to(dtype), sd[p + ".in_proj_bias"].to(dtype)
        self.wo, self.bo = sd[p + ".out_proj.weight"].to(dtype), sd[p + ".out_proj.bias"].to(dtype)
        self.nhead = nhead

    def __call__(self, x):
        Bn, L, D = x.shape
        hd = D // self.nhead
        qkv = F.linear(x, self.wi, self.bi).reshape(Bn, L, 3, self.nhead, hd)
        q, k, v = (qkv[:, :, i].permute(0, 2, 1, 3) for i in range(3))
        ctx = F.scaled_dot_product_attention(q, k, v).permute(0, 2, 1, 3).reshape(Bn, L, D)
        return F.linear(ctx, self.wo, self.bo)


class _TorchEncoderLayer:

    def __init__(self, sd, p, dtype):
        self.att = _TorchMHA(sd, p + ".self_attn", dtype)
        self.l1 = (sd[p + ".linear1.weight"].to(dtype), sd[p + ".linear1.bias"].to(dtype))
        self.l2 = (sd[p + ".linear2.weight"].to(dtype), sd[p + ".linear2.bias"].to(dtype))
        self.n1 = (sd[p + ".norm1.weight"].to(dtype), sd[p + ".norm1.bias"].to(dtype))
        self.n2 = (sd[p + ".norm2.weight"].to(dtype), sd[p + ".norm2.bias"].to(dtype))

    def __call__(self, x):
        x = F.layer_norm(x + self.att(x), (x.shape[-1],), self.n1[0], self.n1[1], 1e-5)
        ff = F.linear(F.relu(F.linear(x, *self.l1)), *self.l2)
        return F.layer_norm(x + ff, (x.shape[-1],), self.n2[0], self.n2[1], 1e-5)


def _conv_params(sd, conv_p, bn_p):
    w = sd[conv_p + ".weight"].float()
    b = sd.get(conv_p + ".bias")
    scale, shift = _bn_affine(sd, bn_p)
    wk = w.permute(0, 2, 3, 1).reshape(w.shape[0], -1).to(torch.float16).contiguous()
    tiles = None
    if wk.is_cuda and w.shape[2] == 3 and w.shape[3] == 3 and w.shape[0] % 128 == 0 and w.shape[1] % 32 == 0 and PACKED_CONV_TILES:
        tiles = ops.pack_conv3x3_tiles(wk, w.shape[0], w.shape[1])
    return dict(w=wk, w_tiles=tiles, bias=None if b is None else _r16(b.float()), scale=scale, shift=shift)


SPLITK_MAX_HYPS = 12
HEADS_TWO_STREAMS_MAX_HYPS = 12
SPLITK_TARGET_WGS = 384
SMALL_CALL_CEILING = 31

_SWITCHES = ("FUSED_OUT_PROJ_LN", "FUSED_FFN", "ROWS_QKV", "PACKED_CONV_TILES", "MERGED_HEAD_QKV", "FUSED_TAIL", "CONV_MFMA_16X16X32", "SPECIALIZED_EPILOGUE", "SPLITK_MAX_HYPS", "HEADS_TWO_STREAMS_MAX_HYPS")


@contextlib.contextmanager
def overrides(**kw):
    g = globals()
    for k, v in kw.items():
        if k not in _SWITCHES:
            raise KeyError(f"engine.overrides: unknown switch {k!r} (known: {', '.join(_SWITCHES)})")
        if k.endswith("_MAX_HYPS") and not (0 <= int(v) <= SMALL_CALL_CEILING):
            raise ValueError(f"engine.overrides: {k} = {v} is outside 0..{SMALL_CALL_CEILING}")
    saved = {k: g[k] for k in kw}
    g.update(kw)
    try:
        yield
    finally:
        g.update(saved)


def small_call(n, limit):
    return n <= min(int(limit), SMALL_CALL_CEILING)


def splitk_pieces(rows, cout, cin):
    tiles = -(-rows // 128) * (cout // 128)
    nk = 9 * cin // 64
    return max(1, min(nk // 2, round(SPLITK_TARGET_WGS / tiles)))


class _HipEncoder:

    def __init__(self, sd, stem, joint, device):
        c1 = sd[stem + ".0.net.0.weight"].float()
        self.c1_w = c1.to(torch.float16).reshape(64, -1).contiguous()
        b1 = sd.get(stem + ".0.net.0.bias")
        self.c1_b = None if b1 is None else _r16(b1.float())
        self.c1_scale, self.c1_shift = _bn_affine(sd, stem + ".0.net.1")
        names = [("c2", stem + ".1.net.0", stem + ".1.net.1")]
        for blk, pre in (("s2", stem + ".2"), ("s3", stem + ".3"), ("j0", joint + ".0"), ("j1", joint + ".1"),
                         ("j3", joint + ".3"), ("j4", joint + ".4")):
            names += [(blk + "a", pre + ".conv1", pre + ".bn1"), (blk + "b", pre + ".conv2", pre + ".bn2")]
        names.append(("j2", joint + ".2.net.0", joint + ".2.net.1"))
        self.w = {k: _conv_params(sd, c, b) for k, c, b in names}
        self.pe = sd["pos_embed.pe"].float().reshape(-1, sd["pos_embed.pe"].shape[-1]).contiguous()
        self.device = device
        self._bufs = {}

    def _buffers(self, n, H, W, slot, small=True):
        small = bool(small) and small_call(n, SPLITK_MAX_HYPS)
        key = (n, H, W, slot, small)
        b = self._bufs.get(key)
        if b is None:
            z = lambda *shape: torch.zeros(shape, dtype=torch.float16, device=self.device)
            h1, w1, h2, w2, h3, w3 = H // 2, W // 2, H // 4, W // 4, H // 8, W // 8
            sk = None
            if small:
                need = max(ops.igemm_splitk_workspace_bytes(r, co, splitk_pieces(r, co, ci))
                           for r, co, ci in ((2 * n * h2 * w2, 128, 64), (2 * n * h2 * w2, 128, 128), (n * h2 * w2, 256, 256),
                                             (n * h3 * w3, 512, 256), (n * h3 * w3, 512, 512)))
                sk = torch.empty(need, dtype=torch.uint8, device=self.device)
            b = dict(SK=sk, P1=z(2 * n, h1 + 2, w1 + 2, 64), P2=z(2 * n, h2 + 2, w2 + 2, 128), P3=z(2 * n, h2 + 2, w2 + 2, 128),
                     T=z(2 * n, h2 + 2, w2 + 2, 128), CAT=z(n, h2 + 2, w2 + 2, 256), J0=z(n, h2 + 2, w2 + 2, 256),
                     T2=z(n, h2 + 2, w2 + 2, 256), Q0=z(n, h3 + 2, w3 + 2, 512), Q1=z(n, h3 + 2, w3 + 2, 512),
                     T3=z(n, h3 + 2, w3 + 2, 512), dims=(h1, w1, h2, w2, h3, w3))
            self._bufs[key] = b
        return b

    def _conv(self, name, x, Bn, Ho, Wo, Cin, Cout, y, stride=1, res=None, relu=True, gout=None, gres=None, pe=None, y_pe=None, sk=None,
              sk_rows=None):
        c = self.w[name]
        G = ops.IgemmGeom.image
        gin = G(Ho, Wo, 1, Cin, stride=stride, offset=0)
        gout = gout if gout is not None else G(Ho, Wo, 1, Cout)
        if res is not None and gres is None:
            gres = G(Ho, Wo, 1, Cout)
        if sk is not None:
            return ops.igemm_f16_splitk(x, gin, c["w"], c["bias"], y, gout, Bn * Ho * Wo, Cout, Cin, 9,
                                        splitk_pieces(sk_rows if sk_rows is not None else Bn * Ho * Wo, Cout, Cin), sk,
                                        relu=relu, residual=res, r_geom=gres, bn_scale=c["scale"], bn_shift=c["shift"],
                                        conv_rounding=True, pe=pe, y_pe=y_pe)
        return ops.igemm_f16(x, gin, c["w"], c["bias"], y, gout, Bn * Ho * Wo, Cout, Cin, 9, relu=relu, residual=res, r_geom=gres,
                             bn_scale=c["scale"], bn_shift=c["shift"], conv_rounding=True, pe=pe, y_pe=y_pe,
                             w_tiles=c["w_tiles"] if stride == 1 else None)

    def __call__(self, AB, slot=0, shared_b=False, small_calls=True):
        n2, _, H, W = AB.shape
        segs = shared_b if isinstance(shared_b, ops.Segments) else None
        if segs is not None:
            n = n2 - len(segs)
            if segs.total != n:
                raise ValueError(f"shared_b: {n2} images and {len(segs)} segments, but the segments cover {segs.total} pairs")
        else:
            n = n2 - 1 if shared_b else n2 // 2
        b = self._buffers(n, H, W, slot, small_calls)
        h1, w1, h2, w2, h3, w3 = b["dims"]
        G = ops.IgemmGeom.image
        ops.conv7x7s2_bn_relu(AB, self.c1_w, self.c1_b, self.c1_scale, self.c1_shift, b["P1"][:n2], 1)
        self._conv("c2", b["P1"], n2, h2, w2, 64, 128, b["P2"], stride=2, sk=b["SK"], sk_rows=2 * n * h2 * w2)
        self._conv("s2a", b["P2"], n2, h2, w2, 128, 128, b["T"], sk=b["SK"], sk_rows=2 * n * h2 * w2)
        self._conv("s2b", b["T"], n2, h2, w2, 128, 128, b["P3"], res=b["P2"], sk=b["SK"], sk_rows=2 * n * h2 * w2)
        self._conv("s3a", b["P3"], n2, h2, w2, 128, 128, b["T"], sk=b["SK"], sk_rows=2 * n * h2 * w2)
        self._conv("s3b", b["T"], n2, h2, w2, 128, 128, b["CAT"], res=b["P3"],
                   gout=G(h2, w2, 1, 256, bsplit=n, cgroup=128), gres=G(h2, w2, 1, 128), sk=b["SK"], sk_rows=2 * n * h2 * w2)
        if segs is not None:
            ops.replicate_segments(b["CAT"], segs, 128, 256)
        elif shared_b and n > 1:
            ops.replicate_channels(b["CAT"], n, 128, 256)
        self._conv("j0a", b["CAT"], n, h2, w2, 256, 256, b["T2"], sk=b["SK"])
        self._conv("j0b", b["T2"], n, h2, w2, 256, 256, b["J0"], res=b["CAT"], sk=b["SK"])
        self._conv("j1a", b["J0"], n, h2, w2, 256, 256, b["T2"], sk=b["SK"])
        self._conv("j1b", b["T2"], n, h2, w2, 256, 256, b["CAT"], res=b["J0"], sk=b["SK"])
        self._conv("j2", b["CAT"], n, h3, w3, 256, 512, b["Q0"], stride=2, sk=b["SK"])
        self._conv("j3a", b["Q0"], n, h3, w3, 512, 512, b["T3"], sk=b["SK"])
        self._conv("j3b", b["T3"], n, h3, w3, 512, 512, b["Q1"], res=b["Q0"], sk=b["SK"])
        self._conv("j4a", b["Q1"], n, h3, w3, 512, 512, b["T3"], sk=b["SK"])
        tok = torch.empty((n, h3 * w3, 512), dtype=torch.float16, device=AB.device)
        x16 = torch.empty_like(tok)
        self._conv("j4b", b["T3"], n, h3, w3, 512, 512, tok, res=b["Q1"], gout=G(h3, w3, 0, 512), gres=G(h3, w3, 1, 512),
                   pe=self.pe[: h3 * w3], y_pe=x16, sk=b["SK"])
        return tok, x16


class _HipLinear:

    def __init__(self, w, b):
        assert w.shape[0] % 128 == 0 and w.shape[1] % 64 == 0
        self.w = w.to(torch.float16).contiguous()
        self.b = _r16(b.float())

    def __call__(self, x, relu=False):
        x2 = x.reshape(-1, x.shape[-1])
        M, K = x2.shape
        No = self.w.shape[0]
        y = torch.empty((M, No), dtype=torch.float16, device=x.device)
        Gm = ops.IgemmGeom.matrix
        ops.igemm_f16(x2, Gm(K), self.w, self.b, y, Gm(No), M, No, K, 1, relu=relu)
        return y.reshape(*x.shape[:-1], No)


class _HipRowsLinear:

    def __init__(self, w, b):
        self.w = w.to(torch.float16).contiguous()
        self.b = _r16(b.float())

    def __call__(self, x, round_f16=True, out_f16=False, out=None):
        return ops.rows_linear(x, self.w, self.b, round_f16=round_f16, out_f16=out_f16, out=out)


class _HipMHA:
    def __init__(self, sd, p, fp16_scores, nhead=4, small_calls=True):
        self.qkv = _HipLinear(sd[p + ".in_proj_weight"], sd[p + ".in_proj_bias"])
        self.out = _HipLinear(sd[p + ".out_proj.weight"], sd[p + ".out_proj.bias"])
        self.out_rows = _HipRowsLinear(sd[p + ".out_proj.weight"], sd[p + ".out_proj.bias"])
        self.nhead, self.fp16_scores = nhead, fp16_scores
        self.qkv_p = ops.PackedLinear512(self.qkv.w) if tuple(self.qkv.w.shape) == (1536, 512) else None
        self.small_calls = small_calls
        self._sk = {}

    def context(self, x16, slot=0, small_calls=True):
        Bn, L, D = x16.shape
        qkv = self.in_proj(x16, slot, small_calls)
        return ops.attention_f16(qkv.reshape(Bn, L, 3 * D), self.nhead, fp16_scores=self.fp16_scores)

    def in_proj(self, x16, slot=0, small_calls=True):
        Bn, L, D = x16.shape
        if ROWS_QKV and self.qkv_p is not None and Bn * L >= ROWS_QKV_MIN_ROWS:
            qkv = ops.linear512(x16, self.qkv_p, self.qkv.b)
        elif self.small_calls and small_calls and small_call(Bn, SPLITK_MAX_HYPS) and D % 64 == 0 and D // 64 >= 4:
            M, No = Bn * L, self.qkv.w.shape[0]
            pieces = max(1, min(D // 64 // 2, round(SPLITK_TARGET_WGS / (-(-M // 128) * (No // 128)))))
            key = (M, No, pieces, x16.device, slot)
            ws = self._sk.get(key)
            if ws is None:
                ws = self._sk[key] = torch.empty(ops.igemm_splitk_workspace_bytes(M, No, pieces), dtype=torch.uint8, device=x16.device)
            qkv = torch.empty((M, No), dtype=torch.float16, device=x16.device)
            Gm = ops.IgemmGeom.matrix
            ops.igemm_f16_splitk(x16.reshape(M, D), Gm(D), self.qkv.w, self.qkv.b, qkv, Gm(No), M, No, D, 1, pieces, ws)
        else:
            qkv = self.qkv(x16)
        return qkv

    def __call__(self, x16, slot=0, small_calls=True):
        return self.out(self.context(x16, slot, small_calls))


class _HipEncoderLayer:

    def __init__(self, sd, p):
        self.att = _HipMHA(sd, p + ".self_attn", fp16_scores=False)
        self.l1 = _HipLinear(sd[p + ".linear1.weight"], sd[p + ".linear1.bias"])
        self.l2 = _HipLinear(sd[p + ".linear2.weight"], sd[p + ".linear2.bias"])
        self.n1 = (sd[p + ".norm1.weight"].float().contiguous(), sd[p + ".norm1.bias"].float().contiguous())
        self.n2 = (sd[p + ".norm2.weight"].float().contiguous(), sd[p + ".norm2.bias"].float().contiguous())
        self.out_p, self.l1_p, self.l2_p = (ops.PackedLinear512(m.w) for m in (self.att.out, self.l1, self.l2))

    def pooled(self, tok16, x16, pe, slot=0, small_calls=True):
        return self.pooled_from_context(self.att.context(x16, slot, small_calls), tok16, pe)

    def pooled_from_context(self, ctx16, tok16, pe):
        if FUSED_TAIL and FUSED_OUT_PROJ_LN and FUSED_FFN and ctx16.shape[1] % 16 == 0 and tuple(pe.shape) == (ctx16.shape[1], 512):
            return ops.encoder_tail_mean(ctx16, self.out_p, self.att.out.b, tok16, pe, self.n1[0], self.n1[1], self.l1_p, self.l1.b,
                                         self.l2_p, self.l2.b, self.n2[0], self.n2[1], 1e-5)
        if FUSED_OUT_PROJ_LN:
            y32, y16 = ops.linear_layernorm_res(ctx16, self.out_p, self.att.out.b, self.n1[0], self.n1[1], 1e-5, tok16=tok16, pe=pe)
        else:
            sa = self.att.out(ctx16.contiguous())
            y32, y16 = ops.layernorm_res(sa, self.n1[0], self.n1[1], 1e-5, tok16=tok16, pe=pe)
        if FUSED_FFN and y16.shape[1] % 16 == 0:
            return ops.ffn_layernorm_mean(y16, self.l1_p, self.l1.b, self.l2_p, self.l2.b, y32, self.n2[0], self.n2[1], 1e-5)
        ff = self.l2(self.l1(y16, relu=True))
        return ops.colmean_f16(ff, self.n2[0], self.n2[1], 1e-5, resid32=y32)


def _check_precision(precision):
    if precision not in ("fp16", "fp32", "torch_amp"):
        raise ValueError(f"precision must be 'fp16', 'fp32' or 'torch_amp', got {precision!r}")


def _dev_sd(module_or_sd, device):
    sd = module_or_sd.state_dict() if hasattr(module_or_sd, "state_dict") else module_or_sd
    return {k: v.detach().to(device) for k, v in sd.items()}


class RefinePlan:
    small_calls = True

    def __init__(self, model, device, precision="fp16", channels_last=True):
        _check_precision(precision)
        self.dtype = torch.float16 if precision == "fp16" else torch.float32
        self.hip = self.dtype == torch.float16
        self.module = model if precision == "torch_amp" else None
        if self.module is not None:
            return
        sd = _dev_sd(model, device)
        self.heads = {}
# ... 155 lines not shown
```

foundationpose_amd/ops.py:

```python
import ctypes as C
from typing import NamedTuple

import numpy as np
import torch

from . import _lib

FLAG_NORMALIZE_XYZ = 1
FLAG_OUT_F16 = 2
MODE_REFINE = 0
MODE_SCORE = 1
ROT_AXIS_ANGLE = 0
ROT_6D = 1
TRANS_TRACKNET, TRANS_DEEPIM, TRANS_RAW = 0, 1, 2


def _stream(t=None):
    if t is None:
        return C.c_void_p(torch.cuda.current_stream().cuda_stream)
    dev = t.device
    if dev.index is not None and dev.index != torch.cuda.current_device():
        raise _lib.FpAmdError(f"tensor on {dev} but the current device is cuda:{torch.cuda.current_device()}: wrap the call in "
                              f"`with torch.cuda.device({dev.index}):` (kernels launch on the current device)")
    return C.c_void_p(torch.cuda.current_stream(dev).cuda_stream)
# ... 960 lines not shown
    bx, by = torch.remainder(f, Bx), torch.div(f, Bx, rounding_mode="floor")
    dx = torch.tensor([0.0, T - 1.0, 0.0], dtype=torch.float64, device=device)
    dy = torch.tensor([0.0, 0.0, T - 1.0], dtype=torch.float64, device=device)
    uv = torch.stack([(bx[:, None] * T + 0.5 + dx[None]) / Wt, (by[:, None] * T + 0.5 + dy[None]) / Ht], -1)
    return uv.reshape(3 * int(F), 2).float().contiguous(), torch.arange(3 * int(F), dtype=torch.int32, device=device).view(int(F), 3)


def texture_bake(pos, faces, vertex_color, depth, rgb, masks, ob_in_cams, Ks, tol, min_cos, texels=4, Bx=None, min_depth=0.001):
    what = "texture_bake"
    for name, t, nd in (("pos", pos, 2), ("faces", faces, 2), ("depth", depth, 3), ("rgb", rgb, 4), ("ob_in_cams", ob_in_cams, 3)):
        if not torch.is_tensor(t):
            raise _lib.FpAmdError(f"{what}: {name} must be a tensor, got {type(t).__name__}")
        if t.dim() != nd:
            raise _lib.FpAmdError(f"{what}: {name} must have {nd} dimensions, got {tuple(t.shape)}")
    if pos.shape[1] != 3 or faces.shape[1] != 3:
        raise _lib.FpAmdError(f"{what}: pos must be (Nv,3) and faces (F,3), got {tuple(pos.shape)} and {tuple(faces.shape)}")
    Nv, F = int(pos.shape[0]), int(faces.shape[0])
    if vertex_color is not None and (not torch.is_tensor(vertex_color) or tuple(vertex_color.shape) != (Nv, 3)):
        raise _lib.FpAmdError(f"{what}: vertex_color must be a ({Nv},3) tensor like pos or None")
    V, H, W = (int(x) for x in depth.shape)
    if V > 4096:
        raise _lib.FpAmdError(f"{what}: {V} views in one call, at most 4096")
    if H < 1 or W < 1 or H * W > 1 << 28:
        raise _lib.FpAmdError(f"{what}: frames of {H} x {W} pixels (1 .. 2^28 pixels are supported)")
    if tuple(rgb.shape) != (V, H, W, 3):
        raise _lib.FpAmdError(f"{what}: rgb must be ({V},{H},{W},3) like depth, got {tuple(rgb.shape)}")
    if masks is not None and (not torch.is_tensor(masks) or tuple(masks.shape) != (V, H, W)):
        raise _lib.FpAmdError(f"{what}: masks must be a ({V},{H},{W}) tensor like depth or None")
    if tuple(ob_in_cams.shape) != (V, 4, 4):
        raise _lib.FpAmdError(f"{what}: ob_in_cams must be ({V},4,4), got {tuple(ob_in_cams.shape)}")
    Bx, Ht, Wt = texture_atlas_layout(F, texels, Bx)
    tl, mc, md = float(tol), float(min_cos), float(min_depth)
    if not (np.isfinite(tl) and tl >= 0 and np.isfinite(np.float32(tl))):
        raise ValueError(f"{what}: tol must be finite and >= 0 (metres), got {tol!r}")
    if not (0 < np.float32(mc) <= 1):
        raise ValueError(f"{what}: min_cos must be in (0, 1], got {min_cos!r}")
    if not (np.isfinite(md) and md >= 0):
        raise ValueError(f"{what}: min_depth must be finite and >= 0 (metres), got {min_depth!r}")
    K_dev = None
    if torch.is_tensor(Ks) and Ks.is_cuda:
        if tuple(Ks.shape) != (V, 3, 3):
            raise _lib.FpAmdError(f"{what}: device Ks must be ({V},3,3), got {tuple(Ks.shape)}")
        K_dev = Ks
    else:
        Kh = [_hostK33(K, what, "the projection of a texel is defined without one") for K in Ks]
        if len(Kh) != V:
            raise _lib.FpAmdError(f"{what}: {len(Kh)} intrinsic matrices for {V} views")
    p = _dev(pos, torch.float32, "pos")
    fc = _dev(faces, torch.int32, "faces")
    vc = _dev(vertex_color, torch.float32, "vertex_color")
    d = _dev(depth, torch.float32, "depth")
    c = _dev(rgb, torch.float32, "rgb")
    m = _dev(masks, torch.uint8, "masks")
    P = _dev(ob_in_cams, torch.float32, "ob_in_cams")
    K_dev = _dev(K_dev, torch.float64, "Ks")
    tex = torch.empty((Ht, Wt, 3), dtype=torch.float32, device=p.device)
    coverage = torch.empty((Ht, Wt), dtype=torch.uint8, device=p.device)
    uv, uv_idx = texture_atlas_uv(F, texels, Bx, p.device)
    if F == 0:
        return tex, coverage, uv, uv_idx
    if K_dev is None and V > 0:
        K_dev = torch.as_tensor(np.stack(Kh), device=p.device)
    _lib.check(_lib.lib().fp_texture_bake(_ptr(p), Nv, _ptr(fc), F, _ptr(vc), _ptr(d), _ptr(c), _ptr(m), _ptr(P), _ptr(K_dev), V, H, W,
                                          int(texels), Bx, tl, mc, md, _ptr(tex), _ptr(coverage), _stream(p)), "fp_texture_bake")
    return tex, coverage, uv, uv_idx


def pose_update(trans, rot, poses, rot_rep="axis_angle", normalize_xyz=True, trans_normalizer=(1.0, 1.0, 1.0),
                rot_normalizer=1.0, mesh_diameter=1.0, out=None, trans_delta_out=None, rot_delta_out=None, trans_rep="tracknet",
                K=None, tf_to_crops=None, input_w=0, obj=None, views=None):
    if _overlap(out, poses):
        raise _lib.FpAmdError("pose_update: out must not overlap poses (poses_in / poses_out are __restrict__; there is no in-place update)")
    tr = _dev(trans, torch.float32, "trans")
    ro = _dev(rot, torch.float32, "rot")
    P = _dev(poses, torch.float32, "poses")
    N = int(P.shape[0])
    if rot_rep == "axis_angle":
        rr = ROT_AXIS_ANGLE
    elif rot_rep == "6d":
        rr = ROT_6D
    else:
        raise RuntimeError(f"unknown rot_rep {rot_rep}")
    tn = np.ascontiguousarray(np.broadcast_to(np.asarray(trans_normalizer, dtype=np.float32).reshape(-1), (3,)))
    O = out if out is not None else torch.empty_like(P)
    deepim = trans_rep == "deepim"
    K9 = _hostK32(K) if deepim and views is None else None
    tf = _dev(tf_to_crops, torch.float32, "tf_to_crops") if deepim else None
    tro = TRANS_DEEPIM if deepim else (TRANS_TRACKNET if trans_rep == "tracknet" else TRANS_RAW)
    if views is not None:
        vt = _views(views, "pose_update", N)
        d, o, M = _objects_views(mesh_diameter, obj, "pose_update")
        st = _lib.lib().fp_pose_update_views(_ptr(tr), _ptr(ro), _ptr(P), rr, int(bool(normalize_xyz)), tn.ctypes.data_as(C.c_void_p),
                                             float(rot_normalizer), _ptr(d), _ptr(o), M, N, _ptr(O),
                                             _ptr(_dev(trans_delta_out, torch.float32, "trans_delta_out")),
                                             _ptr(_dev(rot_delta_out, torch.float32, "rot_delta_out")), tro, _ptr(vt.K32), _ptr(vt.dev),
                                             vt.V, _ptr(tf), float(input_w), _stream(P))
        _lib.check(st, "fp_pose_update_views")
        return O
    objs = _objects(mesh_diameter, obj, "pose_update")
    if objs is not None:
        d, o, M = objs
        st = _lib.lib().fp_pose_update_multi(_ptr(tr), _ptr(ro), _ptr(P), rr, int(bool(normalize_xyz)), tn.ctypes.data_as(C.c_void_p),
                                             float(rot_normalizer), _ptr(d), _ptr(o), M, N, _ptr(O),
                                             _ptr(_dev(trans_delta_out, torch.float32, "trans_delta_out")),
                                             _ptr(_dev(rot_delta_out, torch.float32, "rot_delta_out")), tro,
                                             K9.ctypes.data_as(C.c_void_p) if deepim else None, _ptr(tf), float(input_w), _stream(P))
        _lib.check(st, "fp_pose_update_multi")
        return O
    st = _lib.lib().fp_pose_update(_ptr(tr), _ptr(ro), _ptr(P), rr, int(bool(normalize_xyz)),
                                   tn.ctypes.data_as(C.c_void_p), float(rot_normalizer), float(np.float32(mesh_diameter)),
                                   N, _ptr(O), _ptr(_dev(trans_delta_out, torch.float32, "trans_delta_out")),
                                   _ptr(_dev(rot_delta_out, torch.float32, "rot_delta_out")), tro,
                                   K9.ctypes.data_as(C.c_void_p) if deepim else None, _ptr(tf), float(input_w), _stream(P))
    _lib.check(st, "fp_pose_update")
    return O


def conv7x7s2_bn_relu(x, w_flat, bias, scale, shift, out, pad):
    x = _dev(x, torch.float16, "x")
    w = _dev(w_flat, torch.float16, "w")
    y = _dev(out, torch.float16, "out")
    Bn, Cin, H, W = x.shape
    if Cin != 6:
        raise _lib.FpAmdError("conv7x7s2_bn_relu: C_in must be 6")
    if tuple(y.shape) != (Bn, H // 2 + 2 * pad, W // 2 + 2 * pad, 64):
        raise _lib.FpAmdError(f"conv7x7s2_bn_relu: out has shape {tuple(y.shape)}")
    st = _lib.lib().fp_conv7x7s2_bn_relu_fwd(_ptr(x), _ptr(w), _ptr(_dev(bias, torch.float32, "bias")),
                                             _ptr(_dev(scale, torch.float32, "scale")), _ptr(_dev(shift, torch.float32, "shift")),
                                             _ptr(y), int(Bn), int(H), int(W), int(pad), _stream(x))
    _lib.check(st, "fp_conv7x7s2_bn_relu_fwd")
    return y


class IgemmGeom(C.Structure):
    _fields_ = [(n, C.c_int) for n in ("pixels_per_image", "width", "padded_h", "padded_w", "stride", "offset", "cstride",
                                       "coff", "bsplit", "cgroup")]

    @staticmethod
    def matrix(ld):
        return IgemmGeom(1, 1, 1, 1, 1, 0, int(ld), 0, 0, 0)

    @staticmethod
    def image(Ho, Wo, pad, C_, stride=1, offset=None, coff=0, bsplit=0, cgroup=0):
        return IgemmGeom(Ho * Wo, Wo, Ho * stride + 2 * pad, Wo * stride + 2 * pad, stride, pad if offset is None else offset,
                         C_, coff, bsplit, cgroup)


IGEMM_RELU = 1
IGEMM_ROUND_ACC = 2
IGEMM_HAS_W_TILES = 4
IGEMM_MFMA_16X16X32 = 16
IGEMM_MFMA_32X32X16 = 32
IGEMM_EPILOGUE_GENERIC = 64


class IgemmEpilogue(C.Structure):
    _fields_ = [("bias", C.c_void_p), ("bn_scale", C.c_void_p), ("bn_shift", C.c_void_p), ("residual", C.c_void_p),
                ("r_geom", C.POINTER(IgemmGeom)), ("flags", C.c_int), ("pe", C.c_void_p), ("pe_period", C.c_int), ("y_pe", C.c_void_p),
                ("w_tiles", C.c_void_p)]


def pack_conv3x3_tiles(w, N, Cin):
    w = _dev(w, torch.float16, "w")
    out = torch.empty_like(w)
    _lib.check(_lib.lib().fp_pack_conv3x3_tiles_f16(_ptr(w), _ptr(out), int(N), int(Cin), _stream(w)), "fp_pack_conv3x3_tiles_f16")
    return out


def _igemm_epilogue(bias, residual, r_geom, bn_scale, bn_shift, pe, y_pe, flags, w_tiles=None):
    pe = _dev(pe, torch.float32, "pe")
    ep = IgemmEpilogue()
    ep.bias, ep.bn_scale = _ptr(_dev(bias, torch.float32, "bias")), _ptr(_dev(bn_scale, torch.float32, "bn_scale"))
    ep.bn_shift, ep.residual = _ptr(_dev(bn_shift, torch.float32, "bn_shift")), _ptr(_dev(residual, torch.float16, "residual"))
    ep.r_geom = C.pointer(r_geom) if r_geom is not None else None
    ep.flags = flags
    ep.pe, ep.pe_period, ep.y_pe = _ptr(pe), (int(pe.shape[-2]) if pe is not None else 0), _ptr(_dev(y_pe, torch.float16, "y_pe"))
    ep.w_tiles = _ptr(_dev(w_tiles, torch.float16, "w_tiles"))
    return ep


def igemm_f16(x, x_geom, w, bias, y, y_geom, M, N, Cin, taps, relu=False, residual=None, r_geom=None, bn_scale=None,
              bn_shift=None, conv_rounding=False, pe=None, y_pe=None, w_tiles=None, mfma16=None):
    x = _dev(x, torch.float16, "x"); w = _dev(w, torch.float16, "w"); y = _dev(y, torch.float16, "y")
    from . import engine
    if mfma16 is None:
        mfma16 = engine.CONV_MFMA_16X16X32
    ep = _igemm_epilogue(bias, residual, r_geom, bn_scale, bn_shift, pe, y_pe,
                         (IGEMM_RELU if relu else 0) | (IGEMM_ROUND_ACC if conv_rounding else 0) | IGEMM_HAS_W_TILES |
                         (IGEMM_MFMA_16X16X32 if mfma16 else IGEMM_MFMA_32X32X16) |
                         (0 if engine.SPECIALIZED_EPILOGUE else IGEMM_EPILOGUE_GENERIC), w_tiles)
    st = _lib.lib().fp_igemm_f16_fwd(_ptr(x), C.byref(x_geom), _ptr(w), _ptr(y), C.byref(y_geom), int(M), int(N), int(Cin),
                                     int(taps), C.byref(ep), _stream(x))
    _lib.check(st, "fp_igemm_f16_fwd")
    return y


def igemm_splitk_workspace_bytes(M, N, splits):
    return int(_lib.lib().fp_igemm_splitk_workspace_bytes(int(M), int(N), int(splits)))


def igemm_f16_splitk(x, x_geom, w, bias, y, y_geom, M, N, Cin, taps, splits, workspace, relu=False, residual=None, r_geom=None,
                     bn_scale=None, bn_shift=None, conv_rounding=False, pe=None, y_pe=None):
    x = _dev(x, torch.float16, "x"); w = _dev(w, torch.float16, "w"); y = _dev(y, torch.float16, "y")
    ws = _dev(workspace, torch.uint8, "workspace")
    ep = _igemm_epilogue(bias, residual, r_geom, bn_scale, bn_shift, pe, y_pe, (IGEMM_RELU if relu else 0) | (IGEMM_ROUND_ACC if conv_rounding else 0))
    st = _lib.lib().fp_igemm_f16_splitk_fwd(_ptr(x), C.byref(x_geom), _ptr(w), _ptr(y), C.byref(y_geom), int(M), int(N), int(Cin),
                                            int(taps), C.byref(ep), int(splits), _ptr(ws), ws.numel(), _stream(x))
    _lib.check(st, "fp_igemm_f16_splitk_fwd")
    return y


def _work_igemm_splitk(x, x_geom, w, bias, y, y_geom, M, N, Cin, taps, splits, workspace, relu=False, residual=None, r_geom=None, **k):
    return _work_igemm(x, x_geom, w, bias, y, y_geom, M, N, Cin, taps, relu=relu, residual=residual, r_geom=r_geom)


def _work_igemm(x, x_geom, w, bias, y, y_geom, M, N, Cin, taps, relu=False, residual=None, r_geom=None, **k):
    by = 2 * (M * Cin * (1 if taps == 1 else 1.0 / (x_geom.stride ** 2)) + N * Cin * taps + M * N * (2 if residual is not None else 1))
    return by, 2.0 * M * N * Cin * taps


def add_pe_f16(tok, pe):
    tok = _dev(tok, torch.float16, "tok")
    pe = _dev(pe, torch.float32, "pe")
    S, D = int(pe.shape[-2]), int(pe.shape[-1])
    M = tok.numel() // D
    out = torch.empty_like(tok)
    _lib.check(_lib.lib().fp_add_pe_f16_fwd(_ptr(tok), _ptr(pe), _ptr(out), M, S, D, _stream(tok)), "fp_add_pe_f16_fwd")
    return out


def replicate_channels(buf, n, c0, c1):
    buf = _dev(buf, torch.float16, "buf")
    if buf.dim() != 4 or not buf.is_contiguous() or buf.shape[0] < n:
        raise _lib.FpAmdError(f"replicate_channels: buf must be a contiguous (>= {n}, Hp, Wp, C) tensor, got {tuple(buf.shape)}")
    if n <= 1:
        return buf
    _, Hp, Wp, Ct = (int(v) for v in buf.shape)
    src = buf.data_ptr() + 2 * int(c0)
    st = _lib.lib().fp_replicate_rows_f16(C.c_void_p(src), C.c_void_p(src + 2 * Hp * Wp * Ct), int(n) - 1, Hp * Wp, int(c1) - int(c0), Ct, Ct,
                                          Hp * Wp * Ct, _stream(buf))
    _lib.check(st, "fp_replicate_rows_f16")
    return buf


def replicate_segments(buf, segments, c0, c1):
    buf = _dev(buf, torch.float16, "buf")
    n = int(segments.total)
    if buf.dim() != 4 or not buf.is_contiguous() or buf.shape[0] < n:
        raise _lib.FpAmdError(f"replicate_segments: buf must be a contiguous (>= {n}, Hp, Wp, C) tensor, got {tuple(buf.shape)}")
    if int(segments.lengths.min()) < 1:
        raise _lib.FpAmdError("replicate_segments: every segment must hold at least one image (its source)")
    if segments.dev.device != buf.device:
        raise _lib.FpAmdError(f"replicate_segments: offsets on {segments.dev.device}, buf on {buf.device}")
    _, Hp, Wp, Ct = (int(v) for v in buf.shape)
    st = _lib.lib().fp_replicate_segments_f16(C.c_void_p(buf.data_ptr() + 2 * int(c0)), _ptr(segments.dev), len(segments), n, Hp * Wp,
                                              int(c1) - int(c0), Ct, Hp * Wp * Ct, _stream(buf))
    _lib.check(st, "fp_replicate_segments_f16")
    return buf


def layernorm_res(branch16, gamma, beta, eps=1e-5, x32=None, tok16=None, pe=None, want32=True, want16=True):
    br = _dev(branch16, torch.float16, "branch16")
    D = int(br.shape[-1])
    M = br.numel() // D
    x32 = _dev(x32, torch.float32, "x32"); tok16 = _dev(tok16, torch.float16, "tok16"); pe = _dev(pe, torch.float32, "pe")
    S = int(pe.shape[-2]) if pe is not None else 0
    y32 = torch.empty(br.shape, dtype=torch.float32, device=br.device) if want32 else None
    y16 = torch.empty_like(br) if want16 else None
    st = _lib.lib().fp_layernorm_res_fwd(_ptr(x32), _ptr(tok16), _ptr(pe), S, _ptr(br), _ptr(_dev(gamma, torch.float32, "gamma")),
                                         _ptr(_dev(beta, torch.float32, "beta")), float(eps), _ptr(y32), _ptr(y16), M, D, _stream(br))
    _lib.check(st, "fp_layernorm_res_fwd")
    return y32, y16


class PackedLinear512:

    def __init__(self, w16):
        w = _dev(w16, torch.float16, "w16")
        if w.dim() != 2 or int(w.shape[1]) != 512 or int(w.shape[0]) % 512 or int(w.shape[0]) == 0:
            raise _lib.FpAmdError(f"PackedLinear512: weight {tuple(w.shape)}, must be (512 n, 512)")
        self.out_features = int(w.shape[0])
        self.data = torch.empty_like(w)
        for blk in range(self.out_features // 512):
            _lib.check(_lib.lib().fp_pack_linear512_f16(_ptr(w[blk * 512:]), _ptr(self.data[blk * 512:]), _stream(w)), "fp_pack_linear512_f16")


def _packed(w, name, out_features=512):
    if not isinstance(w, PackedLinear512):
        raise _lib.FpAmdError(f"{name}: the weight must be a PackedLinear512 (ops.PackedLinear512(w16))")
    if out_features is not None and w.out_features != out_features:
        raise _lib.FpAmdError(f"{name}: packed weight has {w.out_features} output features, expected {out_features}")
    return w.data


def linear512(x16, w_packed, bias, relu=False, out=None):
    x = _dev(x16, torch.float16, "x16")
    w = _packed(w_packed, "linear512", None)
    if int(x.shape[-1]) != 512:
        raise _lib.FpAmdError(f"linear512: x16 (..., {int(x.shape[-1])}), must be (..., 512)")
    N = w_packed.out_features
    M = x.numel() // 512
    y = out if out is not None else torch.empty(tuple(x.shape[:-1]) + (N,), dtype=torch.float16, device=x.device)
    if y.dtype != torch.float16 or y.numel() != M * N or not y.is_contiguous():
        raise _lib.FpAmdError("linear512: out must be a contiguous fp16 tensor of M x N elements")
    _lib.check(_lib.lib().fp_linear512_f16_fwd(_ptr(x), _ptr(w), _ptr(_dev(bias, torch.float32, "bias")), _ptr(y), M, N, 1 if relu else 0,
                                               _stream(x)), "fp_linear512_f16_fwd")
    return y


def linear_layernorm_res(x16, w_packed, bias, gamma, beta, eps=1e-5, x32=None, tok16=None, pe=None, want32=True, want16=True):
    w = _packed(w_packed, "linear_layernorm_res")
    if not (torch.is_tensor(x16) and x16.is_cuda and x16.dtype == torch.float16):
        raise _lib.FpAmdError("linear_layernorm_res: x16 must be a CUDA float16 tensor")
    K = int(x16.shape[-1])
    D = 512
    if K != 512:
        raise _lib.FpAmdError(f"linear_layernorm_res: x16 (..., {K}), must be (..., 512)")
    M = x16.numel() // K
    x, ldx = x16, _column_block(x16, "linear_layernorm_res: x16", sep="")
    x32 = _dev(x32, torch.float32, "x32"); tok16 = _dev(tok16, torch.float16, "tok16"); pe = _dev(pe, torch.float32, "pe")
    S = int(pe.shape[-2]) if pe is not None else 0
    shape = tuple(x.shape[:-1]) + (D,)
    y32 = torch.empty(shape, dtype=torch.float32, device=x.device) if want32 else None
    y16 = torch.empty(shape, dtype=torch.float16, device=x.device) if want16 else None
    st = _lib.lib().fp_linear_layernorm_fwd(_ptr(x), _ptr(w), _ptr(_dev(bias, torch.float32, "bias")), _ptr(x32), _ptr(tok16), _ptr(pe), S,
                                            _ptr(_dev(gamma, torch.float32, "gamma")), _ptr(_dev(beta, torch.float32, "beta")), float(eps),
                                            _ptr(y32), _ptr(y16), M, K, D, ldx, _stream(x))
    _lib.check(st, "fp_linear_layernorm_fwd")
    return y32, y16


def ffn_layernorm_mean(y16, w1_packed, b1, w2_packed, b2, x32, gamma, beta, eps=1e-5):
    y = _dev(y16, torch.float16, "y16")
    G_, R, D = (int(v) for v in y.shape)
    if D != 512:
        raise _lib.FpAmdError("ffn_layernorm_mean: d_model must be 512")
    x32 = _dev(x32, torch.float32, "x32")
    out = torch.empty((G_, D), dtype=torch.float32, device=y.device)
    if R % 16:
        raise _lib.FpAmdError(f"ffn_layernorm_mean: {R} rows per group, must be a multiple of 16")
    ws = torch.empty((max(G_ * R // 16, 1), 512), dtype=torch.float32, device=y.device)
    st = _lib.lib().fp_ffn_layernorm_mean_fwd(_ptr(y), _ptr(_packed(w1_packed, "ffn_layernorm_mean")), _ptr(_dev(b1, torch.float32, "b1")),
                                              _ptr(_packed(w2_packed, "ffn_layernorm_mean")), _ptr(_dev(b2, torch.float32, "b2")), _ptr(x32),
# ... 283 lines not shown
```

include/fp_amd.h:

```cpp
#ifndef FP_AMD_H
#define FP_AMD_H

#include <stddef.h>
#include <stdint.h>

#ifdef __cplusplus
extern "C" {
#endif

typedef enum {
  FP_OK = 0,
  FP_ERR_INVALID_ARG = -1,
  FP_ERR_WORKSPACE = -2,
  FP_ERR_LAUNCH = -3,
  FP_ERR_UNSUPPORTED = -4
} fp_status;

#define FP_FLAG_NORMALIZE_XYZ 1
#define FP_FLAG_OUT_F16 2

#define FP_MODE_REFINE 0
#define FP_MODE_SCORE 1

#define FP_ROT_AXIS_ANGLE 0
#define FP_ROT_6D 1
#define FP_TRANS_TRACKNET 0
#define FP_TRANS_DEEPIM 1
#define FP_TRANS_RAW 2

#define FP_SUBPIXEL_BITS 4
#define FP_ZBUF_STEPS_PER_METRE 1048576
#define FP_ZBUF_EMPTY 0xFFFFFFFFu

typedef struct fp_mesh fp_mesh;
typedef struct fp_mesh_set fp_mesh_set;

const char* fp_last_error(void);
#define FP_AMD_ABI_VERSION 226
int fp_version(void);

int fp_mesh_create(const float* pos , const float* nrm , const int32_t* faces ,
                   const float* uv , const int32_t* uv_idx ,
                   const float* tex , const float* vcol , int V, int T, int Ht,
                   int Wt, fp_mesh** out);
void fp_mesh_destroy(fp_mesh* mesh);

#define FP_MESH_SET_MAX_ELEMS (1 << 26)
int fp_mesh_set_create(const fp_mesh* const* meshes , int M, fp_mesh_set** out);
void fp_mesh_set_destroy(fp_mesh_set* set);
size_t fp_mesh_set_workspace_bytes(const fp_mesh_set* set, int N, int oh, int ow);

int fp_depth_erode(const float* depth , float* out , int H, int W, int radius,
                   float depth_diff_thres, float ratio_thres, float zfar, void* stream);
int fp_depth_bilateral(const float* depth , float* out , int H, int W, int radius,
                       float zfar, float sigmaD, float sigmaR, void* stream);
int fp_depth_to_xyz(const float* depth , const double* K , float zfar,
                    int f64_internal, float* xyz , int H, int W, void* stream);

int fp_depth_erode_frames(const float* depth , float* out , int H, int W, int V, int radius,
                          float depth_diff_thres, float ratio_thres, float zfar, void* stream);
int fp_depth_bilateral_frames(const float* depth , float* out , int H, int W, int V, int radius,
                              float zfar, float sigmaD, float sigmaR, void* stream);
int fp_depth_to_xyz_frames(const float* depth , const double* Ks , float zfar, int f64_internal,
                           float* xyz , int H, int W, int V, void* stream);

int fp_mask_depth_stats(const float* depth , const uint8_t* masks , const int32_t* view ,
                        int V, int M, int H, int W, float min_depth, int32_t* out , void* stream);

int fp_crop_windows_views(const float* poses , const double* Ks , const int32_t* view , int V,
                          const double* diameters , const int32_t* obj , int M, double crop_ratio, int out_w,
                          int out_h, int N, float* tf_to_crops , float* bbox2d , void* stream);
int fp_render_crops_views(const fp_mesh_set* set, const int32_t* obj , const double* diameters ,
                          const float* Ks , const int32_t* view , int V, const float* poses ,
                          const float* bbox2d , int H, int W, int N, int oh, int ow, float w_ambient, float w_diffuse,
                          float xyz_thr, int flags, void* A , float* color , float* depth , float* xyz ,
                          float* normal , uint32_t* zbuf , int32_t* tri_id , void* workspace ,
                          size_t workspace_bytes, void* stream);
int fp_warp_crops_views(const float* rgb , const float* xyz_map , const float* depth ,
                        const float* tf_to_crops , const float* Ks , const int32_t* view , int V,
                        const float* poses , const double* diameters , const int32_t* obj , int M,
                        int flags, int mode, int H, int W, int N, int oh, int ow, void* B , void* stream);
int fp_depth_agreement(const float* depth_crops , const float* xyz_map , const float* tf_to_crops ,
                       const int32_t* view , int V, int H, int W, int N, int oh, int ow, float tol,
                       int32_t* counts , void* stream);
size_t fp_icp_workspace_bytes(int N, int oh, int ow);
int fp_icp_point_plane(const float* xyz_crops , const float* normal_crops ,
                       const float* xyz_map , const float* tf_to_crops ,
                       const int32_t* view , int V, int H, int W, const float* poses_in ,
                       int N, int oh, int ow, float max_dist, double damping, int min_pairs,
                       double* system , float* poses_out ,
                       void* workspace, size_t workspace_bytes, void* stream);
#define FP_ERR_ADD 1
#define FP_ERR_ADDS 2
#define FP_ERR_SYM 4
size_t fp_pose_errors_workspace_bytes(int N, int P, int S);
int fp_pose_errors(const float* model_pts , int P, const double* sym_tfs , int S,
                   const float* poses , const double* gt , const int32_t* gt_index , int G, int N,
                   int flags, double* out , void* workspace , size_t workspace_bytes, void* stream);
#define FP_VSD_MAX_T 16
int fp_vsd_counts(const float* est , const float* gt , const int32_t* gt_index , int G, int N,
                  int h, int w, const float* obs , const float* fac , int H, int W, int x0, int y0, float delta,
                  const float* thr , int T, int32_t* counts , void* stream);
int fp_mspd(const float* model_pts , int P, const double* sym_tfs , int S, const float* poses ,
            const double* gt , const int32_t* gt_index , int G, int N, const float* K ,
            double* out , void* stream);

#define FP_TSDF_MAX_DIM 4096
int fp_tsdf_integrate(const float* depth , const float* rgb , const uint8_t* masks ,
                      const float* ob_in_cams , const double* Ks , int V, int H, int W, int nz, int ny, int nx,
                      const float* origin , float voxel, float trunc, float min_depth, float* tsdf ,
                      float* weight , float* color , float* color_weight , void* stream);
int fp_tsdf_count_triangles(const float* tsdf , const float* weight , int nz, int ny, int nx,
                            float min_weight, int32_t* counts , void* stream);
int fp_tsdf_emit_triangles(const float* tsdf , const float* weight , const float* color ,
                           const float* color_weight , int nz, int ny, int nx, const float* origin , float voxel,
                           float min_weight, const int64_t* offsets , long long total, int64_t* keys ,
                           float* pos , float* col , float* nrm , void* stream);
#define FP_TEXTURE_BAKE_MAX_TEXELS 16
#define FP_TEXTURE_BAKE_MAX_SIDE 16384
int fp_texture_bake(const float* pos , int Nv, const int32_t* faces , int F,
                    const float* vertex_color , const float* depth ,
                    const float* rgb , const uint8_t* masks ,
                    const float* ob_in_cams , const double* Ks , int V, int H, int W, int T, int Bx, float tol,
                    float min_cos, float min_depth, float* tex , uint8_t* coverage , void* stream);
int fp_pose_update_views(const float* trans , const float* rot , const float* poses_in ,
                         int rot_rep, int normalize_xyz, const float* trans_normalizer , float rot_normalizer,
                         const double* diameters , const int32_t* obj , int M, int N,
                         float* poses_out , float* trans_delta_out , float* rot_delta_out ,
                         int trans_rep, const float* Ks , const int32_t* view , int V,
                         const float* tf_to_crops , float input_w, void* stream);

int fp_crop_windows(const float* poses , const double* K , double mesh_diameter,
                    double crop_ratio, int out_w, int out_h, int N, float* tf_to_crops ,
                    float* bbox2d , void* stream);
int fp_crop_windows_multi(const float* poses , const double* K , const double* diameters ,
                          const int32_t* obj , int M, double crop_ratio, int out_w, int out_h, int N,
                          float* tf_to_crops , float* bbox2d , void* stream);

size_t fp_workspace_bytes(int N, int V, int T, int oh, int ow);
size_t fp_raster_lds_bytes(int ow);

int fp_render_crops(const fp_mesh* mesh, const float* poses , const float* bbox2d ,
                    const float* K9 , int H, int W, int N, int oh, int ow, float w_ambient,
                    float w_diffuse, float mesh_diameter, float xyz_thr, int flags, void* A ,
                    float* color , float* depth , float* xyz , float* normal ,
                    uint32_t* zbuf , int32_t* tri_id , void* workspace ,
                    size_t workspace_bytes, void* stream);

int fp_render_crops_multi(const fp_mesh_set* set, const int32_t* obj , const double* diameters ,
                          const float* poses , const float* bbox2d , const float* K9 ,
                          int H, int W, int N, int oh, int ow, float w_ambient, float w_diffuse, float xyz_thr, int flags,
                          void* A , float* color , float* depth , float* xyz , float* normal ,
                          uint32_t* zbuf , int32_t* tri_id , void* workspace , size_t workspace_bytes,
                          void* stream);

int fp_warp_crops(const float* rgb , const float* xyz_map , const float* depth ,
                  const float* tf_to_crops , const float* K9 ,
                  const float* poses , float mesh_diameter, int flags, int mode, int H, int W,
                  int N, int oh, int ow, void* B , void* stream);

int fp_warp_crops_multi(const float* rgb , const float* xyz_map , const float* depth ,
                        const float* tf_to_crops , const float* K9 , const float* poses ,
                        const double* diameters , const int32_t* obj , int M, int flags, int mode, int H,
                        int W, int N, int oh, int ow, void* B , void* stream);

int fp_pose_update(const float* trans , const float* rot ,
                   const float* poses_in , int rot_rep, int normalize_xyz,
                   const float* trans_normalizer , float rot_normalizer, float mesh_diameter, int N,
                   float* poses_out , float* trans_delta_out ,
                   float* rot_delta_out , int trans_rep, const float* K9 ,
                   const float* tf_to_crops , float input_w , void* stream);
int fp_pose_update_multi(const float* trans , const float* rot , const float* poses_in ,
                         int rot_rep, int normalize_xyz, const float* trans_normalizer , float rot_normalizer,
                         const double* diameters , const int32_t* obj , int M, int N,
                         float* poses_out , float* trans_delta_out , float* rot_delta_out ,
                         int trans_rep, const float* K9 , const float* tf_to_crops ,
                         float input_w, void* stream);


int fp_conv7x7s2_bn_relu_fwd(const void* x , const void* w , const float* bias ,
                             const float* bn_scale , const float* bn_shift , void* y ,
                             int B, int Hin, int Win, int pad, void* stream);

typedef struct {
  int pixels_per_image, width, padded_h, padded_w, stride, offset, cstride, coff, bsplit, cgroup;
} fp_igemm_geom;

#define FP_IGEMM_RELU 1
#define FP_IGEMM_HAS_W_TILES 4
#define FP_IGEMM_ROUND_ACC 2

#define FP_IGEMM_MFMA_16X16X32 16
#define FP_IGEMM_MFMA_32X32X16 32

#define FP_IGEMM_EPILOGUE_GENERIC 64

typedef struct {
  const float* bias;
  const float* bn_scale;
  const float* bn_shift;
  const void* residual;
  const fp_igemm_geom* r_geom;
  int flags;
  const float* pe;
  int pe_period;
  void* y_pe;
  const void* w_tiles;
} fp_igemm_epilogue;

int fp_igemm_f16_fwd(const void* x , const fp_igemm_geom* x_geom , const void* w , void* y ,
                     const fp_igemm_geom* y_geom , int M, int N, int Cin, int taps,
                     const fp_igemm_epilogue* epilogue , void* stream);

int fp_pack_conv3x3_tiles_f16(const void* w , void* w_tiles , int N, int Cin, void* stream);
int fp_conv3x3_sw_lds_bytes(void);

size_t fp_igemm_splitk_workspace_bytes(int M, int N, int splits);
int fp_igemm_f16_splitk_fwd(const void* x , const fp_igemm_geom* x_geom , const void* w , void* y ,
                            const fp_igemm_geom* y_geom , int M, int N, int Cin, int taps,
                            const fp_igemm_epilogue* epilogue , int splits, void* workspace ,
                            size_t workspace_bytes, void* stream);

int fp_add_pe_f16_fwd(const void* tok , const float* pe , void* out , int M, int S, int D, void* stream);

int fp_replicate_rows_f16(const void* src , void* dst , int copies, int rows, int channels, int src_row_stride,
                          int dst_row_stride, long long dst_copy_stride, void* stream);

int fp_replicate_segments_f16(void* buf , const int32_t* seg_offsets , int segments, int images, int pixels,
                              int channels, int pixel_stride, long long image_stride, void* stream);

int fp_layernorm_res_fwd(const float* x32 , const void* tok16 , const float* pe , int S,
                         const void* branch16 , const float* gamma , const float* beta , float eps,
                         float* y32 , void* y16 , int M, int D, void* stream);

int fp_pack_linear512_f16(const void* w16 , void* packed , void* stream);

int fp_linear512_f16_fwd(const void* x16 , const void* w_packed , const float* bias , void* y16 ,
                         int M, int N, int relu, void* stream);

int fp_linear_layernorm_fwd(const void* x16 , const void* w16_packed , const float* bias ,
                            const float* x32 , const void* tok16 , const float* pe , int S,
                            const float* gamma , const float* beta , float eps, float* y32 ,
                            void* y16 , int M, int K, int D, int ldx ,
                            void* stream);

size_t fp_encoder_tail_workspace_bytes(int groups, int rows_per_group);
int fp_encoder_tail_mean_fwd(const void* ctx16 , int ldx, const void* wo_packed , const float* bo ,
                             const void* tok16 , const float* pe , const float* gamma1 , const float* beta1 ,
                             const void* w1_packed , const float* b1 , const void* w2_packed ,
                             const float* b2 , const float* gamma2 , const float* beta2 , float eps,
                             float* out , void* workspace , size_t workspace_bytes, int groups, int rows_per_group,
                             void* stream);

int fp_ffn_layernorm_mean_fwd(const void* y16 , const void* w1_packed , const float* b1 ,
                              const void* w2_packed , const float* b2 , const float* x32 ,
                              const float* gamma , const float* beta , float eps, float* out ,
                              float* workspace , size_t workspace_bytes, int groups, int rows_per_group, void* stream);

int fp_colmean_f16_fwd(const void* x , const float* resid32 , const float* gamma ,
                       const float* beta , float eps, float* out , int groups, int rows_per_group,
                       int D, void* stream);

#define FP_ROWS_ROUND_F16 1
#define FP_ROWS_X_F16 2
#define FP_ROWS_Y_F16 4

int fp_rows_linear_fwd(const void* x , const void* w , const float* bias , void* y ,
                       int M, int K, int N, int flags, void* stream);

#define FP_ATT_FP16_SCORES 1

int fp_attention_f16_fwd(const void* qkv , void* out , int B, int S, int H, int head_dim, int flags,
                         void* stream);

int fp_attention_segments_f16_fwd(const void* qkv , void* out ,
                                  const int32_t* seg_offsets , int B, int max_S, int H, int head_dim, int flags,
                                  void* stream);

int fp_cluster_poses(float angle_diff_deg, float dist_diff, const float* poses , int N,
                     const float* symmetry_tfs , int S, int* keep_idx );

#ifdef __cplusplus
}
#endif
#endif
```

Measured before the change: 8024.

## Add direct-store conv3x3 kernel with transposed MFMA operands and repacked weight tiles

Adds a k_conv_sw_direct variant of the 3x3 sliding-window conv that swaps the MFMA operand order, so each lane's accumulators hold consecutive output channels for one pixel. A matching weight-tile packing permutes rows so the epilogue can write 4 channels as a b64 store straight from registers, skipping the LDS staging round trip in the specialized epilogue. It is enabled by default for conv layers that have a bias and no second output. The cost is more narrow global stores, an extra kernel instantiation, and a pack layout that has to match the kernel variant.

```diff
diff --git a/foundationpose_amd/_lib.py b/foundationpose_amd/_lib.py
--- a/foundationpose_amd/_lib.py
+++ b/foundationpose_amd/_lib.py
@@ -5,7 +5,7 @@
 
 _HERE = os.path.dirname(os.path.abspath(__file__))
 LIB_PATH = os.environ.get("FP_AMD_LIB") or os.path.join(_HERE, "csrc", "libfp_amd.so")
-ABI_VERSION = 226
+ABI_VERSION = 227
 _lib = None
 
 vp, ci, cf, cd, sz = C.c_void_p, C.c_int, C.c_float, C.c_double, C.c_size_t
@@ -53,6 +53,7 @@
     "fp_conv7x7s2_bn_relu_fwd": (ci, [vp, vp, vp, vp, vp, vp, ci, ci, ci, ci, vp]),
     "fp_igemm_f16_fwd": (ci, [vp, vp, vp, vp, vp, ci, ci, ci, ci, vp, vp]),
     "fp_pack_conv3x3_tiles_f16": (ci, [vp, vp, ci, ci, vp]),
+    "fp_pack_conv3x3_tiles_direct_f16": (ci, [vp, vp, ci, ci, vp]),
     "fp_conv3x3_sw_lds_bytes": (ci, []),
     "fp_igemm_splitk_workspace_bytes": (sz, [ci, ci, ci]),
     "fp_igemm_f16_splitk_fwd": (ci, [vp, vp, vp, vp, vp, ci, ci, ci, ci, vp, ci, vp, sz, vp]),
diff --git a/foundationpose_amd/csrc/conv_sw.hip b/foundationpose_amd/csrc/conv_sw.hip
--- a/foundationpose_amd/csrc/conv_sw.hip
+++ b/foundationpose_amd/csrc/conv_sw.hip
@@ -6,10 +6,13 @@
 #include "igemm_epilogue.h"
 
 #ifdef FP_PROFILE_BUILD
-__device__ unsigned long long sw_dbg[8];
+__device__ unsigned long long sw_dbg[10];
 extern "C" int fp_dbg_conv_sw(unsigned long long* out, int reset) {
-  if (reset) { unsigned long long z[8] = {0, 0, 0, 0, 0, 0, ~0ull, 0}; return (int)hipMemcpyToSymbol(HIP_SYMBOL(sw_dbg), z, sizeof(z)); }
+  if (reset) { unsigned long long z[10] = {0, 0, 0, 0, 0, 0, ~0ull, 0, 0, 0}; return (int)hipMemcpyToSymbol(HIP_SYMBOL(sw_dbg), z, sizeof(z)); }
   return (int)hipMemcpyFromSymbol(out, HIP_SYMBOL(sw_dbg), 8 * sizeof(unsigned long long));
+}
+extern "C" int fp_dbg_conv_sw_direct(unsigned long long* out) {
+  return (int)hipMemcpyFromSymbol(out, HIP_SYMBOL(sw_dbg), 2 * sizeof(unsigned long long), 8 * sizeof(unsigned long long));
 }
 extern "C" int fp_dbg_conv_sw_epilogue(unsigned long long* out, int reset) {
   if (reset) { unsigned long long z[8] = {0, 0, 0, 0, 0, 0, 0, 0}; return (int)hipMemcpyToSymbol(HIP_SYMBOL(ig_epi_dbg), z, sizeof(z)); }
@@ -38,6 +41,16 @@
 typedef float sw_float4 __attribute__((ext_vector_type(4)));
 __device__ __forceinline__ void sw_mfma16(sw_float4& acc, const half8& a, const half8& b) {
   asm volatile("v_mfma_f32_16x16x32_f16 %0, %1, %2, %0" : "+v"(acc) : "v"(a), "v"(b));
+}
+
+template <bool DIRECT>
+__device__ __forceinline__ void sw_mfma16x(sw_float4& acc, const half8& w, const half8& a) {
+  if constexpr (DIRECT) sw_mfma16(acc, a, w);
+  else sw_mfma16(acc, w, a);
+}
+
+__host__ __device__ constexpr int sw_direct_row(int r) {
+  return (r & 64) + 4 * (4 * ((0x2130 >> (4 * ((r >> 2) & 3))) & 3) + (r & 3)) + ((r >> 4) & 3);
 }
 
 __device__ __forceinline__ int sw_div(int n, unsigned mul, unsigned shr) { return (int)(__umulhi((unsigned)n, mul) >> shr); }
@@ -58,278 +71,14 @@
 
 template <int BM, int BN, int TM, bool S16>
 __global__ __launch_bounds__(512, 1) void k_conv_sw(IgemmParams p) {
-  constexpr int BK = SW_BK, NW = 8, THREADS = 512;
-  constexpr int NWN = BN / 64;
-  static_assert((BM / (32 * TM)) * NWN == NW, "8 waves");
-  constexpr int ROWB = BK * 2;
-  constexpr int W_BYTES = BN * ROWB;
-  constexpr int SW_PROWS = sw_prows(BM);
-  constexpr int SW_PATCH_BYTES = SW_PROWS * ROWB;
-  constexpr int WI = BN / 16 / NW;
-  constexpr int PI = SW_PROWS / 16 / NW;
-  static_assert(WI >= 1 && PI >= 1 && PI <= 7 && SW_PROWS == PI * 16 * NW, "tile shape");
-  constexpr int STAGES_BYTES = 2 * SW_PATCH_BYTES + SW_NSTW * W_BYTES;
-  constexpr int LDS_MAIN = ig_lds_main_slim<BM, BN>(STAGES_BYTES);
-  auto swz = [](int row) { return (row >> 2) & 3; };
-  auto swzp = [](int row) { return S16 ? (row >> 1) & 2 : (row >> 2) & 3; };
-  extern __shared__ __attribute__((aligned(16))) unsigned char smem[];
-  SW_CLK(t_start);
-  unsigned char* const patch = smem;
-  unsigned char* const wring = smem + 2 * SW_PATCH_BYTES;
-  const int tid = threadIdx.x, lane = tid & 63;
-  const int wid = __builtin_amdgcn_readfirstlane(tid >> 6);
-  const int grp = wid >> 2;
-  const int wm = wid / NWN, wn = wid - wm * NWN;
-  float* bias_lds = reinterpret_cast<float*>(smem + LDS_MAIN);
-
-  const _Float16* A_ = p.A;
-  const _Float16* W_ = p.Wt;
-  const _Float16* Wpk_ = p.Wpk;
-  const float* bias_ = p.bias;
-  const float* bnsc_ = p.bn_scale;
-  const float* bnsh_ = p.bn_shift;
-  const int M = p.M, N = p.N, Cin = p.Cin, cstride = p.in.cstride, coff = p.in.coff;
-  const SwGeom gi = {p.in.HoWo, p.in.Wo, p.in.Hp, p.in.Wp, p.in.mulP, p.in.shrP, p.in.mulW, p.in.shrW};
-  asm volatile("" ::"s"(A_), "s"(W_), "s"(Wpk_), "s"(bias_), "s"(bnsc_), "s"(bnsh_), "s"(M), "s"(N), "s"(Cin), "s"(cstride), "s"(coff),
-               "s"(gi.HoWo), "s"(gi.Wo), "s"(gi.Hp), "s"(gi.Wp), "s"(gi.mulP), "s"(gi.shrP), "s"(gi.mulW), "s"(gi.shrW));
-  __builtin_amdgcn_sched_barrier(0);
-
-  const int tiles_n = N / BN;
-  const int nwg = (int)(((unsigned)M + BM - 1) / BM) * tiles_n;
-  const int xcd = blockIdx.x & 7, loc = blockIdx.x >> 3;
-  const int qd8 = nwg >> 3, r8 = nwg & 7;
-  const int tile = (xcd < r8 ? xcd * (qd8 + 1) : r8 * (qd8 + 1) + (xcd - r8) * qd8) + loc;
-  const int bm = __builtin_popcount(tiles_n) == 1 ? tile >> __builtin_ctz(tiles_n) : tile / tiles_n, bn = tile - bm * tiles_n;
-  const int m0 = bm * BM, n0 = bn * BN;
-  const int Ktot = 9 * Cin, Wp = gi.Wp;
-  const int ncc = Cin / BK;
-  ig_bias_to_lds(bias_, bnsc_, bnsh_, N, n0, bias_lds, wid, lane);
-
-  const int q0 = sw_q(gi, m0);
-  const int qmax = sw_div(M, gi.mulP, gi.shrP) * gi.Hp * Wp - 1;
-  unsigned poff32[PI], woff32[WI];
-  {
-    const int row0 = wid * PI * 16 + (lane >> 2);
-    const int c = (lane & 3) ^ swzp(row0);
-    static_assert(((16 >> 1) & 2) == 0 && ((16 >> 2) & 3) == 0, "swzp(row0 + 16 j) == swzp(row0)");
-    const unsigned ps2 = (unsigned)cstride * 2, omax = (unsigned)qmax * ps2, lane_off = (unsigned)(coff + c * 8) * 2;
-    const unsigned o0 = (unsigned)(q0 + row0) * ps2;
-#pragma unroll
-    for (int j = 0; j < PI; ++j) {
-      const unsigned o = o0 + j * 16 * ps2;
-      poff32[j] = (o < omax ? o : omax) + lane_off;
-    }
-  }
-#pragma unroll
-  for (int j = 0; j < WI; ++j) {
-    const int row = (wid * WI + j) * 16 + (lane >> 2);
-    const int c = (lane & 3) ^ swz(row);
-    woff32[j] = (unsigned)((((size_t)(n0 + row) * Ktot) + c * 8) * 2);
-  }
-  const bool wpk = (BN == 128) && Wpk_ != nullptr;
-  if (wpk) {
-#pragma unroll
-    for (int j = 0; j < WI; ++j) woff32[j] = (unsigned)(((wid * WI + j) * 64 + lane) * 16);
-  }
-  const int wpk_base = wpk ? bn * (ncc * 9) * W_BYTES : 0;
-  const __amdgpu_buffer_rsrc_t rsA = __builtin_amdgcn_make_buffer_rsrc(const_cast<_Float16*>(A_), 0, 0x7FFFFFFF, 0x00020000);
-  const __amdgpu_buffer_rsrc_t rsW = __builtin_amdgcn_make_buffer_rsrc(const_cast<_Float16*>(wpk ? Wpk_ : W_), 0, 0x7FFFFFFF, 0x00020000);
-
-  auto stage_patch = [&](int cc, int j) {
-    unsigned char* dst = patch + (cc & 1) * SW_PATCH_BYTES + (wid * PI + j) * 1024;
-    __builtin_amdgcn_raw_ptr_buffer_load_lds(rsA, (__attribute__((address_space(3))) void*)dst, 16, (int)poff32[j],
-                                             cc * (BK * 2), 0, 0);
-  };
-  auto stage_w = [&](int cc, int tap, int slot) {
-    const int wsoff = wpk ? wpk_base + (cc * 9 + tap) * W_BYTES : (tap * Cin + cc * BK) * 2;
-    unsigned char* dst = wring + slot * W_BYTES + wid * (WI * 1024);
-#pragma unroll
-    for (int j = 0; j < WI; ++j)
-      __builtin_amdgcn_raw_ptr_buffer_load_lds(rsW, (__attribute__((address_space(3))) void*)(dst + j * 1024), 16,
-                                               (int)woff32[j], wsoff, 0, 0);
-  };
-
-#pragma unroll
-  for (int j = 0; j < PI; ++j) stage_patch(0, j);
-  stage_w(0, 0, 0);
-  stage_w(0, 1, 1);
-  stage_w(0, 2, 2);
-  __builtin_amdgcn_sched_barrier(0);
-  SW_CLK(t_issue);
-
-  constexpr int NFA = S16 ? 2 * TM : TM, NFW = S16 ? 4 : 2;
-  constexpr int FR = S16 ? 16 : 32;
-  typedef float float4_ __attribute__((ext_vector_type(4)));
-  typedef typename std::conditional<S16, float4_, float16_>::type acc_t;
-  acc_t acc[NFW][NFA];
-#pragma unroll
-  for (int i = 0; i < NFW; ++i)
-#pragma unroll
-    for (int j = 0; j < NFA; ++j)
-#pragma unroll
-      for (int e = 0; e < (S16 ? 4 : 16); ++e) acc[i][j][e] = 0.f;
-
-  const int frow = lane & (FR - 1), fhalf = lane >> (S16 ? 4 : 5);
-  int arow[NFA], w_off[2][2];
-#pragma unroll
-  for (int t = 0; t < NFA; ++t) {
-    int m = m0 + wm * (32 * TM) + t * FR + frow;
-    m = m < M ? m : M - 1;
-    arow[t] = sw_q(gi, m) - q0;
-    if constexpr (S16) arow[t] = (arow[t] << 6) + (fhalf << 4);
-  }
-  if constexpr (S16) {
-    const int quad = (0x1320 >> (4 * (frow >> 2))) & 3;
-#pragma unroll
-    for (int t = 0; t < 4; ++t) {
-      const int rw = wn * 64 + t * 16 + 4 * quad + (frow & 3);
-      w_off[t >> 1][t & 1] = rw * ROWB + ((fhalf ^ swz(rw)) << 4);
-    }
-  } else {
-#pragma unroll
-    for (int t = 0; t < 2; ++t) {
-      const int rw = wn * 64 + t * 32 + frow;
-#pragma unroll
-      for (int kk = 0; kk < 2; ++kk) w_off[t][kk] = rw * ROWB + (((2 * kk + fhalf) ^ swz(rw)) << 4);
-    }
-  }
-  static_assert(TM == 4, "the fragment addresses of the next tap are computed behind the MFMA groups of a k-step, one per group of four");
-  int anext[NFA], aflip[NFA];
-#pragma unroll
-  for (int t = 0; t < NFA; ++t) {
-    anext[t] = S16 ? arow[t] : (arow[t] << 6) + ((fhalf ^ swz(arow[t])) << 4);
-    aflip[t] = S16 ? (arow[t] >> 3) & 32 : 0;
-  }
-
-#pragma unroll
-  for (int t = 0; t < NFA; ++t) {
-    asm volatile("" : "+v"(arow[t]), "+v"(anext[t]));
-    if constexpr (S16) asm volatile("" : "+v"(aflip[t]));
-  }
-  asm volatile("" : "+v"(w_off[0][0]), "+v"(w_off[0][1]), "+v"(w_off[1][0]), "+v"(w_off[1][1]));
-#pragma unroll
-  for (int i = 0; i < NFW; ++i)
-#pragma unroll
-    for (int j = 0; j < NFA; ++j) asm volatile("" : "+v"(acc[i][j]));
-  __builtin_amdgcn_sched_barrier(0);
-
-  sw_wait_vm<2 * WI>();
-  __builtin_amdgcn_s_barrier();
-  SW_CLK(t_cold);
-  if (grp) __builtin_amdgcn_s_barrier();
-
-  half8 fa[2][TM], fw[2][2];
-  auto kstep = [&](int cc, auto tap_c, auto last_c) {
-    constexpr int T = decltype(tap_c)::value;
-    constexpr bool LAST = decltype(last_c)::value;
-    constexpr int ky = T / 3, kx = T - 3 * ky;
-    const int s = cc * 9 + T;
-    const unsigned char* pb = patch + (cc & 1) * SW_PATCH_BYTES;
-    const unsigned char* wb = wring + (s & (SW_NSTW - 1)) * W_BYTES;
-    const int shift = ky * Wp + kx;
-    if constexpr (S16) {
-#pragma unroll
-      for (int t = 0; t < NFA; ++t) fa[t >> 2][t & 3] = *reinterpret_cast<const half8*>(pb + (anext[t] ^ aflip[t]));
-#pragma unroll
-      for (int t = 0; t < 4; ++t) fw[t >> 1][t & 1] = *reinterpret_cast<const half8*>(wb + w_off[t >> 1][t & 1]);
-    } else {
-#pragma unroll
-      for (int t = 0; t < TM; ++t) {
-        const int a0 = anext[t];
-        fa[0][t] = *reinterpret_cast<const half8*>(pb + a0);
-        fa[1][t] = *reinterpret_cast<const half8*>(pb + (a0 ^ 32));
-      }
-#pragma unroll
-      for (int kk = 0; kk < 2; ++kk)
-#pragma unroll
-        for (int t = 0; t < 2; ++t) fw[kk][t] = *reinterpret_cast<const half8*>(wb + w_off[t][kk]);
-    }
-    (void)shift;
-    if constexpr (!LAST) {
-      if constexpr (T < PI) stage_patch(cc + 1, T);
-      if constexpr (T + 3 < 9) stage_w(cc, T + 3, (s + 3) & (SW_NSTW - 1));
-      else stage_w(cc + 1, T - 6, (s + 3) & (SW_NSTW - 1));
-      constexpr int NP = (T < PI ? 1 : 0) + ((T >= 1 && T - 1 < PI) ? 1 : 0);
-      sw_wait_vm<2 * WI + NP>();
-    } else {
-      if constexpr (T + 3 < 9) stage_w(cc, T + 3, (s + 3) & (SW_NSTW - 1));
-      constexpr int NYOUNGER = T <= 5 ? 2 : (T == 6 ? 1 : 0);
-      sw_wait_vm<NYOUNGER * WI>();
-    }
-    asm volatile("s_waitcnt lgkmcnt(0)" ::: "memory");
-    __builtin_amdgcn_sched_barrier(0);
-    __builtin_amdgcn_s_barrier();
-    __builtin_amdgcn_sched_barrier(0);
-    __builtin_amdgcn_s_setprio(1);
-    {
-      constexpr int TN = (T + 1) % 9, kyn = TN / 3, kxn = TN - 3 * kyn;
-      const int shift_n = kyn * Wp + kxn;
-      if constexpr (S16) {
-        int sh = shift_n << 6;
-        asm volatile("" : "+s"(sh));
-#pragma unroll
-        for (int i = 0; i < 4; ++i)
-#pragma unroll
-          for (int jh = 0; jh < 2; ++jh) {
-            const int t = i * 2 + jh;
-            int x, y;
-            sw_mfma16(acc[i][jh * 4 + 0], fw[i >> 1][i & 1], fa[jh][0]);
-            asm volatile("v_add_u32 %0, %1, %2" : "=v"(x) : "s"(sh), "v"(arow[t]));
-            sw_mfma16(acc[i][jh * 4 + 1], fw[i >> 1][i & 1], fa[jh][1]);
-            asm volatile("v_lshrrev_b32 %0, 3, %1" : "=v"(y) : "v"(x));
-            sw_mfma16(acc[i][jh * 4 + 2], fw[i >> 1][i & 1], fa[jh][2]);
-            asm volatile("v_and_b32 %0, 32, %0" : "+v"(y));
-            sw_mfma16(acc[i][jh * 4 + 3], fw[i >> 1][i & 1], fa[jh][3]);
-            anext[t] = x; aflip[t] = y;
-          }
-      } else {
-#pragma unroll
-      for (int kk = 0; kk < 2; ++kk)
-#pragma unroll
-        for (int i = 0; i < 2; ++i) {
-#pragma unroll
-          for (int j = 0; j < TM; ++j)
-            acc[i][j] = __builtin_amdgcn_mfma_f32_32x32x16_f16(fw[kk][i], fa[kk][j], acc[i][j], 0, 0, 0);
-          const int t = kk * 2 + i;
-          {
-            int ar = arow[t];
-            asm volatile("" : "+v"(ar));
-            const int pr = ar + shift_n;
-            anext[t] = (pr << 6) + ((fhalf ^ swz(pr)) << 4);
-          }
-        }
-      }
-    }
-    __builtin_amdgcn_s_setprio(0);
-    __builtin_amdgcn_sched_barrier(0);
-    __builtin_amdgcn_s_barrier();
-    __builtin_amdgcn_sched_barrier(0);
-  };
-  auto chunk = [&](int cc, auto last_c) {
-    kstep(cc, std::integral_constant<int, 0>{}, last_c);
-    kstep(cc, std::integral_constant<int, 1>{}, last_c);
-    kstep(cc, std::integral_constant<int, 2>{}, last_c);
-    kstep(cc, std::integral_constant<int, 3>{}, last_c);
-    kstep(cc, std::integral_constant<int, 4>{}, last_c);
-    kstep(cc, std::integral_constant<int, 5>{}, last_c);
-    kstep(cc, std::integral_constant<int, 6>{}, last_c);
-    kstep(cc, std::integral_constant<int, 7>{}, last_c);
-    kstep(cc, std::integral_constant<int, 8>{}, last_c);
-  };
-  for (int cc = 0; cc + 1 < ncc; ++cc) chunk(cc, std::false_type{});
-  chunk(ncc - 1, std::true_type{});
-  if (!grp) __builtin_amdgcn_s_barrier();
-  __syncthreads();
-  SW_CLK(t_loop);
-  ig_epilogue<BM, BN, TM, THREADS, 0, true>(p, acc, smem, m0, n0, wm, wn, tid, lane, bias_lds);
-#ifdef FP_PROFILE_BUILD
-  asm volatile("s_waitcnt vmcnt(0)" ::: "memory");
-  SW_CLK(t_end);
-  if (tid == 0) {
-    atomicAdd(&sw_dbg[0], t_cold - t_start); atomicAdd(&sw_dbg[1], t_loop - t_cold); atomicAdd(&sw_dbg[2], t_end - t_loop);
-    atomicAdd(&sw_dbg[3], 1ull); atomicAdd(&sw_dbg[4], t_issue - t_start); atomicMin(&sw_dbg[6], t_start); atomicMax(&sw_dbg[7], t_end);
-  }
-#endif
+  constexpr bool DIRECT = false;
+#include "conv_sw_tile.inc"
+}
+
+template <int BM, int BN, int TM, bool S16>
+__global__ __launch_bounds__(512, 1) void k_conv_sw_direct(IgemmParams p) {
+  constexpr bool DIRECT = true;
+#include "conv_sw_tile.inc"
 }
 
 constexpr int LS_PROWS = 448, LS_NSTW = 3;
@@ -583,12 +332,33 @@
 
 extern "C" int fp_conv3x3_sw_lds_bytes(void) { return sw_lds_bytes(512, 128); }
 
+static bool sw_direct(const IgemmParams& p) {
+  if (!p.direct || !p.mfma16 || sw_variant(p) == 1 || sw_use_256(p)) return false;
+  return p.epi == IG_EPI_CONV || p.epi == (IG_EPI_CONV | IG_EPI_RES) || p.epi == (IG_EPI_CONV | IG_EPI_BN) || p.epi == (IG_EPI_CONV | IG_EPI_BN | IG_EPI_RES);
+}
+
+static int sw_direct_launch(const IgemmParams& p, hipStream_t stream) {
+  constexpr int LDS = sw_lds_bytes(512, 128);
+  const long long tiles = (long long)fp_cdiv(p.M, 512) * (p.N / 128);
+  FP_REQUIRE(tiles < (1ll << 31), "fp_igemm_f16_fwd: too many tiles");
+  FP_SET_MAX_LDS((k_conv_sw_direct<512, 128, 4, true>), LDS);
+  hipLaunchKernelGGL((k_conv_sw_direct<512, 128, 4, true>), dim3((unsigned)tiles), dim3(512), LDS, stream, p);
+  FP_CHECK_LAUNCH("fp_igemm_f16_fwd(conv_sw_direct)");
+  return FP_OK;
+}
+
 int fp_conv3x3_sw_launch(const IgemmParams& p, hipStream_t stream) {
+  const bool direct = sw_direct(p);
+  if (p.Wpk && sw_variant(p) != 1 && !sw_use_256(p))
+    FP_REQUIRE((p.wpk_direct != 0) == direct, "fp_igemm_f16_fwd: w_tiles is in the layout of %s but this launch runs %s (FP_IGEMM_W_TILES_DIRECT, FP_IGEMM_DIRECT_STORE)",
+               p.wpk_direct ? "fp_pack_conv3x3_tiles_direct_f16" : "fp_pack_conv3x3_tiles_f16", direct ? "k_conv_sw_direct" : "k_conv_sw");
+  if (direct) return sw_direct_launch(p, stream);
   if (sw_variant(p) == 1) return sw_ls_launch<256, 128, 4>(p, stream);
   if (sw_use_256(p)) return p.mfma16 ? sw_launch<256, 256, 4, true>(p, stream) : sw_launch<256, 256, 4, false>(p, stream);
   return p.mfma16 ? sw_launch<512, 128, 4, true>(p, stream) : sw_launch<512, 128, 4, false>(p, stream);
 }
 
+template <bool DIRECT>
 __global__ __launch_bounds__(256) void k_pack_conv3x3_tiles(const _Float16* __restrict__ w, _Float16* __restrict__ out, int N, int Cin) {
   const int nk = 9 * (Cin / 32);
   const long long total = (long long)N * nk * 4;
@@ -600,17 +370,27 @@
   const int s = (int)(blk % nk), bn = (int)(blk / nk);
   const int cc = s / 9, tap = s - 9 * cc;
   const int lc = pc ^ ((r >> 2) & 3);
-  const half8 v = *reinterpret_cast<const half8*>(w + (size_t)(bn * 128 + r) * (9 * Cin) + tap * Cin + cc * 32 + lc * 8);
+  const int src = DIRECT ? sw_direct_row(r) : r;
+  const half8 v = *reinterpret_cast<const half8*>(w + (size_t)(bn * 128 + src) * (9 * Cin) + tap * Cin + cc * 32 + lc * 8);
   *reinterpret_cast<half8*>(out + q * 8) = v;
 }
 
+template <bool DIRECT>
+static int sw_pack_tiles(const void* w, void* w_tiles, int N, int Cin, void* stream, const char* who) {
+  FP_REQUIRE(w && w_tiles && w != w_tiles, "%s: NULL tensor or in-place repack", who);
+  FP_REQUIRE(N > 0 && N % 128 == 0 && Cin > 0 && Cin % 32 == 0, "%s: N=%d must be a multiple of 128, Cin=%d of 32", who, N, Cin);
+  FP_REQUIRE((((size_t)w | (size_t)w_tiles) & 15) == 0, "%s: tensors must be 16-byte aligned", who);
+  const long long total = (long long)N * 9 * (Cin / 32) * 4;
+  hipLaunchKernelGGL(k_pack_conv3x3_tiles<DIRECT>, dim3((unsigned)((total + 255) / 256)), dim3(256), 0, (hipStream_t)stream, (const _Float16*)w,
+                     (_Float16*)w_tiles, N, Cin);
+  FP_CHECK_LAUNCH(who);
+  return FP_OK;
+}
+
 extern "C" int fp_pack_conv3x3_tiles_f16(const void* w, void* w_tiles, int N, int Cin, void* stream) {
-  FP_REQUIRE(w && w_tiles && w != w_tiles, "fp_pack_conv3x3_tiles_f16: NULL tensor or in-place repack");
-  FP_REQUIRE(N > 0 && N % 128 == 0 && Cin > 0 && Cin % 32 == 0, "fp_pack_conv3x3_tiles_f16: N=%d must be a multiple of 128, Cin=%d of 32", N, Cin);
-  FP_REQUIRE((((size_t)w | (size_t)w_tiles) & 15) == 0, "fp_pack_conv3x3_tiles_f16: tensors must be 16-byte aligned");
-  const long long total = (long long)N * 9 * (Cin / 32) * 4;
-  hipLaunchKernelGGL(k_pack_conv3x3_tiles, dim3((unsigned)((total + 255) / 256)), dim3(256), 0, (hipStream_t)stream, (const _Float16*)w,
-                     (_Float16*)w_tiles, N, Cin);
-  FP_CHECK_LAUNCH("fp_pack_conv3x3_tiles_f16");
-  return FP_OK;
-}
+  return sw_pack_tiles<false>(w, w_tiles, N, Cin, stream, "fp_pack_conv3x3_tiles_f16");
+}
+
+extern "C" int fp_pack_conv3x3_tiles_direct_f16(const void* w, void* w_tiles, int N, int Cin, void* stream) {
+  return sw_pack_tiles<true>(w, w_tiles, N, Cin, stream, "fp_pack_conv3x3_tiles_direct_f16");
+}
diff --git a/foundationpose_amd/csrc/conv_sw_tile.inc b/foundationpose_amd/csrc/conv_sw_tile.inc
--- /dev/null
+++ b/foundationpose_amd/csrc/conv_sw_tile.inc
@@ -0,0 +1,298 @@
+  static_assert(!DIRECT || (S16 && BM == 512 && BN == 128 && TM == 4), "the direct epilogue is the 512 x 128 tile's, on 16x16x32 MFMAs");
+  constexpr int BK = SW_BK, NW = 8, THREADS = 512;
+  constexpr int NWN = BN / 64;
+  static_assert((BM / (32 * TM)) * NWN == NW, "8 waves");
+  constexpr int ROWB = BK * 2;
+  constexpr int W_BYTES = BN * ROWB;
+  constexpr int SW_PROWS = sw_prows(BM);
+  constexpr int SW_PATCH_BYTES = SW_PROWS * ROWB;
+  constexpr int WI = BN / 16 / NW;
+  constexpr int PI = SW_PROWS / 16 / NW;
+  static_assert(WI >= 1 && PI >= 1 && PI <= 7 && SW_PROWS == PI * 16 * NW, "tile shape");
+  constexpr int STAGES_BYTES = 2 * SW_PATCH_BYTES + SW_NSTW * W_BYTES;
+  constexpr int LDS_MAIN = ig_lds_main_slim<BM, BN>(STAGES_BYTES);
+  auto swz = [](int row) { return (row >> 2) & 3; };
+  auto swzp = [](int row) { return S16 ? (row >> 1) & 2 : (row >> 2) & 3; };
+  extern __shared__ __attribute__((aligned(16))) unsigned char smem[];
+  SW_CLK(t_start);
+  unsigned char* const patch = smem;
+  unsigned char* const wring = smem + 2 * SW_PATCH_BYTES;
+  const int tid = threadIdx.x, lane = tid & 63;
+  const int wid = __builtin_amdgcn_readfirstlane(tid >> 6);
+  const int grp = wid >> 2;
+  const int wm = wid / NWN, wn = wid - wm * NWN;
+  float* bias_lds = reinterpret_cast<float*>(smem + LDS_MAIN);
+
+  const _Float16* A_ = p.A;
+  const _Float16* W_ = p.Wt;
+  const _Float16* Wpk_ = p.Wpk;
+  const float* bias_ = p.bias;
+  const float* bnsc_ = p.bn_scale;
+  const float* bnsh_ = p.bn_shift;
+  const int M = p.M, N = p.N, Cin = p.Cin, cstride = p.in.cstride, coff = p.in.coff;
+  const SwGeom gi = {p.in.HoWo, p.in.Wo, p.in.Hp, p.in.Wp, p.in.mulP, p.in.shrP, p.in.mulW, p.in.shrW};
+  asm volatile("" ::"s"(A_), "s"(W_), "s"(Wpk_), "s"(bias_), "s"(bnsc_), "s"(bnsh_), "s"(M), "s"(N), "s"(Cin), "s"(cstride), "s"(coff),
+               "s"(gi.HoWo), "s"(gi.Wo), "s"(gi.Hp), "s"(gi.Wp), "s"(gi.mulP), "s"(gi.shrP), "s"(gi.mulW), "s"(gi.shrW));
+  __builtin_amdgcn_sched_barrier(0);
+
+  const int tiles_n = N / BN;
+  const int nwg = (int)(((unsigned)M + BM - 1) / BM) * tiles_n;
+  const int xcd = blockIdx.x & 7, loc = blockIdx.x >> 3;
+  const int qd8 = nwg >> 3, r8 = nwg & 7;
+  const int tile = (xcd < r8 ? xcd * (qd8 + 1) : r8 * (qd8 + 1) + (xcd - r8) * qd8) + loc;
+  const int bm = __builtin_popcount(tiles_n) == 1 ? tile >> __builtin_ctz(tiles_n) : tile / tiles_n, bn = tile - bm * tiles_n;
+  const int m0 = bm * BM, n0 = bn * BN;
+  const int Ktot = 9 * Cin, Wp = gi.Wp;
+  const int ncc = Cin / BK;
+  ig_bias_to_lds(bias_, bnsc_, bnsh_, N, n0, bias_lds, wid, lane);
+
+  const int q0 = sw_q(gi, m0);
+  const int qmax = sw_div(M, gi.mulP, gi.shrP) * gi.Hp * Wp - 1;
+  unsigned poff32[PI], woff32[WI];
+  {
+    const int row0 = wid * PI * 16 + (lane >> 2);
+    const int c = (lane & 3) ^ swzp(row0);
+    static_assert(((16 >> 1) & 2) == 0 && ((16 >> 2) & 3) == 0, "swzp(row0 + 16 j) == swzp(row0)");
+    const unsigned ps2 = (unsigned)cstride * 2, omax = (unsigned)qmax * ps2, lane_off = (unsigned)(coff + c * 8) * 2;
+    const unsigned o0 = (unsigned)(q0 + row0) * ps2;
+#pragma unroll
+    for (int j = 0; j < PI; ++j) {
+      const unsigned o = o0 + j * 16 * ps2;
+      poff32[j] = (o < omax ? o : omax) + lane_off;
+    }
+  }
+#pragma unroll
+  for (int j = 0; j < WI; ++j) {
+    const int row = (wid * WI + j) * 16 + (lane >> 2);
+    const int c = (lane & 3) ^ swz(row);
+    const int src = DIRECT ? sw_direct_row(row) : row;
+    woff32[j] = (unsigned)((((size_t)(n0 + src) * Ktot) + c * 8) * 2);
+  }
+  const bool wpk = (BN == 128) && Wpk_ != nullptr;
+  if (wpk) {
+#pragma unroll
+    for (int j = 0; j < WI; ++j) woff32[j] = (unsigned)(((wid * WI + j) * 64 + lane) * 16);
+  }
+  const int wpk_base = wpk ? bn * (ncc * 9) * W_BYTES : 0;
+  const __amdgpu_buffer_rsrc_t rsA = __builtin_amdgcn_make_buffer_rsrc(const_cast<_Float16*>(A_), 0, 0x7FFFFFFF, 0x00020000);
+  const __amdgpu_buffer_rsrc_t rsW = __builtin_amdgcn_make_buffer_rsrc(const_cast<_Float16*>(wpk ? Wpk_ : W_), 0, 0x7FFFFFFF, 0x00020000);
+
+  auto stage_patch = [&](int cc, int j) {
+    unsigned char* dst = patch + (cc & 1) * SW_PATCH_BYTES + (wid * PI + j) * 1024;
+    __builtin_amdgcn_raw_ptr_buffer_load_lds(rsA, (__attribute__((address_space(3))) void*)dst, 16, (int)poff32[j],
+                                             cc * (BK * 2), 0, 0);
+  };
+  auto stage_w = [&](int cc, int tap, int slot) {
+    const int wsoff = wpk ? wpk_base + (cc * 9 + tap) * W_BYTES : (tap * Cin + cc * BK) * 2;
+    unsigned char* dst = wring + slot * W_BYTES + wid * (WI * 1024);
+#pragma unroll
+    for (int j = 0; j < WI; ++j)
+      __builtin_amdgcn_raw_ptr_buffer_load_lds(rsW, (__attribute__((address_space(3))) void*)(dst + j * 1024), 16,
+                                               (int)woff32[j], wsoff, 0, 0);
+  };
+
+#pragma unroll
+  for (int j = 0; j < PI; ++j) stage_patch(0, j);
+  stage_w(0, 0, 0);
+  stage_w(0, 1, 1);
+  stage_w(0, 2, 2);
+  __builtin_amdgcn_sched_barrier(0);
+  SW_CLK(t_issue);
+
+  constexpr int NFA = S16 ? 2 * TM : TM, NFW = S16 ? 4 : 2;
+  constexpr int FR = S16 ? 16 : 32;
+  typedef float float4_ __attribute__((ext_vector_type(4)));
+  typedef typename std::conditional<S16, float4_, float16_>::type acc_t;
+  acc_t acc[NFW][NFA];
+#pragma unroll
+  for (int i = 0; i < NFW; ++i)
+#pragma unroll
+    for (int j = 0; j < NFA; ++j)
+#pragma unroll
+      for (int e = 0; e < (S16 ? 4 : 16); ++e) acc[i][j][e] = 0.f;
+
+  const int frow = lane & (FR - 1), fhalf = lane >> (S16 ? 4 : 5);
+  int arow[NFA], w_off[2][2];
+#pragma unroll
+  for (int t = 0; t < NFA; ++t) {
+    int m = m0 + wm * (32 * TM) + t * FR + frow;
+    m = m < M ? m : M - 1;
+    arow[t] = sw_q(gi, m) - q0;
+    if constexpr (S16) arow[t] = (arow[t] << 6) + (fhalf << 4);
+  }
+  if constexpr (S16) {
+    const int quad = (0x1320 >> (4 * (frow >> 2))) & 3;
+#pragma unroll
+    for (int t = 0; t < 4; ++t) {
+      const int rw = wn * 64 + t * 16 + 4 * quad + (frow & 3);
+      w_off[t >> 1][t & 1] = rw * ROWB + ((fhalf ^ swz(rw)) << 4);
+    }
+  } else {
+#pragma unroll
+    for (int t = 0; t < 2; ++t) {
+      const int rw = wn * 64 + t * 32 + frow;
+#pragma unroll
+      for (int kk = 0; kk < 2; ++kk) w_off[t][kk] = rw * ROWB + (((2 * kk + fhalf) ^ swz(rw)) << 4);
+    }
+  }
+  static_assert(TM == 4, "the fragment addresses of the next tap are computed behind the MFMA groups of a k-step, one per group of four");
+  int anext[NFA], aflip[NFA];
+#pragma unroll
+  for (int t = 0; t < NFA; ++t) {
+    anext[t] = S16 ? arow[t] : (arow[t] << 6) + ((fhalf ^ swz(arow[t])) << 4);
+    aflip[t] = S16 ? (arow[t] >> 3) & 32 : 0;
+  }
+
+#pragma unroll
+  for (int t = 0; t < NFA; ++t) {
+    asm volatile("" : "+v"(arow[t]), "+v"(anext[t]));
+    if constexpr (S16) asm volatile("" : "+v"(aflip[t]));
+  }
+  asm volatile("" : "+v"(w_off[0][0]), "+v"(w_off[0][1]), "+v"(w_off[1][0]), "+v"(w_off[1][1]));
+#pragma unroll
+  for (int i = 0; i < NFW; ++i)
+#pragma unroll
+    for (int j = 0; j < NFA; ++j) asm volatile("" : "+v"(acc[i][j]));
+  if constexpr (DIRECT) {
+    static_assert(THREADS == BM && STAGES_BYTES + BM * 4 <= LDS_MAIN, "one thread per row; the table lies behind the stages");
+    const int m = m0 + tid;
+    reinterpret_cast<int*>(smem + STAGES_BYTES)[tid] = m < M ? (int)(ig_row_off(p.out, m) + n0) : IG_ROW_NONE;
+  }
+  __builtin_amdgcn_sched_barrier(0);
+
+  sw_wait_vm<2 * WI>();
+  __builtin_amdgcn_s_barrier();
+  SW_CLK(t_cold);
+  if (grp) __builtin_amdgcn_s_barrier();
+
+  half8 fa[2][TM], fw[2][2];
+  auto kstep = [&](int cc, auto tap_c, auto last_c) {
+    constexpr int T = decltype(tap_c)::value;
+    constexpr bool LAST = decltype(last_c)::value;
+    constexpr int ky = T / 3, kx = T - 3 * ky;
+    const int s = cc * 9 + T;
+    const unsigned char* pb = patch + (cc & 1) * SW_PATCH_BYTES;
+    const unsigned char* wb = wring + (s & (SW_NSTW - 1)) * W_BYTES;
+    const int shift = ky * Wp + kx;
+    if constexpr (S16) {
+#pragma unroll
+      for (int t = 0; t < NFA; ++t) fa[t >> 2][t & 3] = *reinterpret_cast<const half8*>(pb + (anext[t] ^ aflip[t]));
+#pragma unroll
+      for (int t = 0; t < 4; ++t) fw[t >> 1][t & 1] = *reinterpret_cast<const half8*>(wb + w_off[t >> 1][t & 1]);
+    } else {
+#pragma unroll
+      for (int t = 0; t < TM; ++t) {
+        const int a0 = anext[t];
+        fa[0][t] = *reinterpret_cast<const half8*>(pb + a0);
+        fa[1][t] = *reinterpret_cast<const half8*>(pb + (a0 ^ 32));
+      }
+#pragma unroll
+      for (int kk = 0; kk < 2; ++kk)
+#pragma unroll
+        for (int t = 0; t < 2; ++t) fw[kk][t] = *reinterpret_cast<const half8*>(wb + w_off[t][kk]);
+    }
+    (void)shift;
+    if constexpr (!LAST) {
+      if constexpr (T < PI) stage_patch(cc + 1, T);
+      if constexpr (T + 3 < 9) stage_w(cc, T + 3, (s + 3) & (SW_NSTW - 1));
+      else stage_w(cc + 1, T - 6, (s + 3) & (SW_NSTW - 1));
+      constexpr int NP = (T < PI ? 1 : 0) + ((T >= 1 && T - 1 < PI) ? 1 : 0);
+      sw_wait_vm<2 * WI + NP>();
+    } else {
+      if constexpr (T + 3 < 9) stage_w(cc, T + 3, (s + 3) & (SW_NSTW - 1));
+      constexpr int NYOUNGER = T <= 5 ? 2 : (T == 6 ? 1 : 0);
+      sw_wait_vm<NYOUNGER * WI>();
+    }
+    asm volatile("s_waitcnt lgkmcnt(0)" ::: "memory");
+    __builtin_amdgcn_sched_barrier(0);
+    __builtin_amdgcn_s_barrier();
+    __builtin_amdgcn_sched_barrier(0);
+    __builtin_amdgcn_s_setprio(1);
+    {
+      constexpr int TN = (T + 1) % 9, kyn = TN / 3, kxn = TN - 3 * kyn;
+      const int shift_n = kyn * Wp + kxn;
+      if constexpr (S16) {
+        int sh = shift_n << 6;
+        asm volatile("" : "+s"(sh));
+#pragma unroll
+        for (int i = 0; i < 4; ++i)
+#pragma unroll
+          for (int jh = 0; jh < 2; ++jh) {
+            const int t = i * 2 + jh;
+            int x, y;
+            sw_mfma16x<DIRECT>(acc[i][jh * 4 + 0], fw[i >> 1][i & 1], fa[jh][0]);
+            asm volatile("v_add_u32 %0, %1, %2" : "=v"(x) : "s"(sh), "v"(arow[t]));
+            sw_mfma16x<DIRECT>(acc[i][jh * 4 + 1], fw[i >> 1][i & 1], fa[jh][1]);
+            asm volatile("v_lshrrev_b32 %0, 3, %1" : "=v"(y) : "v"(x));
+            sw_mfma16x<DIRECT>(acc[i][jh * 4 + 2], fw[i >> 1][i & 1], fa[jh][2]);
+            asm volatile("v_and_b32 %0, 32, %0" : "+v"(y));
+            sw_mfma16x<DIRECT>(acc[i][jh * 4 + 3], fw[i >> 1][i & 1], fa[jh][3]);
+            anext[t] = x; aflip[t] = y;
+          }
+      } else {
+#pragma unroll
+      for (int kk = 0; kk < 2; ++kk)
+#pragma unroll
+        for (int i = 0; i < 2; ++i) {
+#pragma unroll
+          for (int j = 0; j < TM; ++j)
+            acc[i][j] = __builtin_amdgcn_mfma_f32_32x32x16_f16(fw[kk][i], fa[kk][j], acc[i][j], 0, 0, 0);
+          const int t = kk * 2 + i;
+          {
+            int ar = arow[t];
+            asm volatile("" : "+v"(ar));
+            const int pr = ar + shift_n;
+            anext[t] = (pr << 6) + ((fhalf ^ swz(pr)) << 4);
+          }
+        }
+      }
+    }
+    __builtin_amdgcn_s_setprio(0);
+    __builtin_amdgcn_sched_barrier(0);
+    __builtin_amdgcn_s_barrier();
+    __builtin_amdgcn_sched_barrier(0);
+  };
+  auto chunk = [&](int cc, auto last_c) {
+    kstep(cc, std::integral_constant<int, 0>{}, last_c);
+    kstep(cc, std::integral_constant<int, 1>{}, last_c);
+    kstep(cc, std::integral_constant<int, 2>{}, last_c);
+    kstep(cc, std::integral_constant<int, 3>{}, last_c);
+    kstep(cc, std::integral_constant<int, 4>{}, last_c);
+    kstep(cc, std::integral_constant<int, 5>{}, last_c);
+    kstep(cc, std::integral_constant<int, 6>{}, last_c);
+    kstep(cc, std::integral_constant<int, 7>{}, last_c);
+    kstep(cc, std::integral_constant<int, 8>{}, last_c);
+  };
+  for (int cc = 0; cc + 1 < ncc; ++cc) chunk(cc, std::false_type{});
+  chunk(ncc - 1, std::true_type{});
+  if (!grp) __builtin_amdgcn_s_barrier();
+  __syncthreads();
+  SW_CLK(t_loop);
+  if constexpr (DIRECT) {
+    const IgEpiArgs q = {p.out, p.res, p.R, p.Y, p.pe, p.Ype, p.pe_period, p.pe_mul, p.pe_shr, p.N};
+    const int* rowY32 = reinterpret_cast<const int*>(smem + STAGES_BYTES);
+#define SW_DIRECT_CASE(E)                                                                                     \
+    case E:                                                                                                   \
+      if (m0 + BM <= M) ig_epilogue_direct<E, true>(q, acc, smem, rowY32, m0, n0, M, wm, wn, tid, lane, bias_lds);  \
+      else ig_epilogue_direct<E, false>(q, acc, smem, rowY32, m0, n0, M, wm, wn, tid, lane, bias_lds);         \
+      break
+    switch (p.epi) {
+      SW_DIRECT_CASE(IG_EPI_CONV);
+      SW_DIRECT_CASE(IG_EPI_CONV | IG_EPI_RES);
+      SW_DIRECT_CASE(IG_EPI_CONV | IG_EPI_BN);
+      SW_DIRECT_CASE(IG_EPI_CONV | IG_EPI_BN | IG_EPI_RES);
+      default: break;
+    }
+#undef SW_DIRECT_CASE
+  } else {
+    ig_epilogue<BM, BN, TM, THREADS, 0, true>(p, acc, smem, m0, n0, wm, wn, tid, lane, bias_lds);
+  }
+#ifdef FP_PROFILE_BUILD
+  asm volatile("s_waitcnt vmcnt(0)" ::: "memory");
+  SW_CLK(t_end);
+  if (tid == 0) {
+    atomicAdd(&sw_dbg[0], t_cold - t_start); atomicAdd(&sw_dbg[1], t_loop - t_cold); atomicAdd(&sw_dbg[2], t_end - t_loop);
+    atomicAdd(&sw_dbg[3], 1ull); atomicAdd(&sw_dbg[4], t_issue - t_start); atomicMin(&sw_dbg[6], t_start); atomicMax(&sw_dbg[7], t_end);
+    if constexpr (DIRECT) { atomicAdd(&sw_dbg[8], t_end - t_loop); atomicAdd(&sw_dbg[9], 1ull); }
+  }
+#endif
diff --git a/foundationpose_amd/csrc/igemm.hip b/foundationpose_amd/csrc/igemm.hip
--- a/foundationpose_amd/csrc/igemm.hip
+++ b/foundationpose_amd/csrc/igemm.hip
@@ -339,7 +339,8 @@
   FP_REQUIRE(!e.residual || e.r_geom, "%s: residual without geometry", who);
   FP_REQUIRE((e.bn_scale == nullptr) == (e.bn_shift == nullptr), "%s: bn_scale and bn_shift go together", who);
   FP_REQUIRE(!e.bn_scale || (e.flags & FP_IGEMM_ROUND_ACC), "%s: BatchNorm needs FP_IGEMM_ROUND_ACC (conv semantics)", who);
-  FP_REQUIRE((e.flags & ~(FP_IGEMM_RELU | FP_IGEMM_ROUND_ACC | FP_IGEMM_HAS_W_TILES | FP_IGEMM_MFMA_16X16X32 | FP_IGEMM_MFMA_32X32X16 | FP_IGEMM_EPILOGUE_GENERIC)) == 0,
+  FP_REQUIRE((e.flags & ~(FP_IGEMM_RELU | FP_IGEMM_ROUND_ACC | FP_IGEMM_HAS_W_TILES | FP_IGEMM_MFMA_16X16X32 | FP_IGEMM_MFMA_32X32X16 | FP_IGEMM_EPILOGUE_GENERIC |
+                           FP_IGEMM_DIRECT_STORE | FP_IGEMM_W_TILES_DIRECT)) == 0,
              "%s: unknown flags 0x%x", who, e.flags);
   FP_REQUIRE((e.flags & (FP_IGEMM_MFMA_16X16X32 | FP_IGEMM_MFMA_32X32X16)) != (FP_IGEMM_MFMA_16X16X32 | FP_IGEMM_MFMA_32X32X16),
              "%s: FP_IGEMM_MFMA_16X16X32 and FP_IGEMM_MFMA_32X32X16 exclude each other", who);
@@ -350,6 +351,7 @@
   if (int err = ig_check_geom(y_geom, "output", who)) return err;
   if (e.residual) if (int err = ig_check_geom(e.r_geom, "residual", who)) return err;
   const void* w_tiles = (e.flags & FP_IGEMM_HAS_W_TILES) ? e.w_tiles : nullptr;
+  FP_REQUIRE(!(e.flags & FP_IGEMM_W_TILES_DIRECT) || w_tiles, "%s: FP_IGEMM_W_TILES_DIRECT without w_tiles (and FP_IGEMM_HAS_W_TILES)", who);
   FP_REQUIRE(!w_tiles || (taps == 9 && (((size_t)w_tiles) & 15) == 0 && w_tiles != w), "%s: w_tiles is for 3x3 convolutions, 16-byte aligned, not w itself", who);
   p.A = (const _Float16*)x; p.Wt = (const _Float16*)w; p.Wpk = (const _Float16*)w_tiles; p.bias = e.bias; p.bn_scale = e.bn_scale; p.bn_shift = e.bn_shift;
   p.R = (const _Float16*)e.residual; p.Y = (_Float16*)y;
@@ -360,6 +362,7 @@
   p.in = ig_geom(x_geom); p.out = ig_geom(y_geom); p.res = e.residual ? ig_geom(e.r_geom) : ig_geom(y_geom);
   p.slab = nullptr; p.nsplit = 0;
   p.epi = ig_epilogue_mode(p, e.flags);
+  p.direct = (e.flags & FP_IGEMM_DIRECT_STORE) ? 1 : 0; p.wpk_direct = (e.flags & FP_IGEMM_W_TILES_DIRECT) ? 1 : 0;
   ig_fastdiv_init(p.pe_period, &p.pe_mul, &p.pe_shr);
   return FP_OK;
 }
diff --git a/foundationpose_amd/csrc/igemm_common.h b/foundationpose_amd/csrc/igemm_common.h
--- a/foundationpose_amd/csrc/igemm_common.h
+++ b/foundationpose_amd/csrc/igemm_common.h
@@ -58,9 +58,12 @@
   int mfma16;
   int epi;
   unsigned pe_mul, pe_shr;
+  int direct;
   float* slab;
   int nsplit;
+  int wpk_direct;
 };
+static_assert(sizeof(IgemmParams) == 336, "IgemmParams grew: the hidden kernel arguments move");
 static_assert(sizeof(IgemmGeom) == 64 && offsetof(IgemmParams, in) == 64 && offsetof(IgemmParams, out) == 128, "the head of IgemmParams is its first 128 bytes");
 
 #define IG_EPI_SPEC 1
diff --git a/foundationpose_amd/csrc/igemm_epilogue.h b/foundationpose_amd/csrc/igemm_epilogue.h
--- a/foundationpose_amd/csrc/igemm_epilogue.h
+++ b/foundationpose_amd/csrc/igemm_epilogue.h
@@ -47,6 +47,19 @@
   half8 r;
 #pragma unroll
   for (int e = 0; e < 4; ++e) {
+    const half2_ x = {v[2 * e], v[2 * e + 1]};
+    half2_ y;
+    asm("v_pk_max_f16 %0, %1, 0" : "=v"(y) : "v"(x));
+    r[2 * e] = y[0]; r[2 * e + 1] = y[1];
+  }
+  return r;
+}
+
+__device__ __forceinline__ half4 ig_relu4(const half4& v) {
+  typedef _Float16 half2_ __attribute__((ext_vector_type(2)));
+  half4 r;
+#pragma unroll
+  for (int e = 0; e < 2; ++e) {
     const half2_ x = {v[2 * e], v[2 * e + 1]};
     half2_ y;
     asm("v_pk_max_f16 %0, %1, 0" : "=v"(y) : "v"(x));
@@ -209,6 +222,87 @@
   }
 #endif
 }
+template <int EPI, bool FULL, typename Acc>
+__device__ __forceinline__ void ig_epilogue_direct(const IgEpiArgs& p, Acc& acc, unsigned char* smem, const int* rowY32, int m0, int n0, int M,
+                                                   int wm, int wn, int tid, int lane, const float* bias_lds) {
+  constexpr int TM = 4;
+  static_assert(std::is_same<Acc, ig_float4[4][2 * TM]>::value, "accumulators of the 16x16x32 loop");
+  static_assert((EPI & IG_EPI_CONV) == IG_EPI_CONV && !(EPI & IG_EPI_PE), "conv rounding + bias + ReLU, without the positional output");
+  constexpr bool HAS_BN = (EPI & IG_EPI_BN) != 0, RES = (EPI & IG_EPI_RES) != 0;
+  typedef float float4_ __attribute__((ext_vector_type(4)));
+  typedef int int4_ __attribute__((ext_vector_type(4)));
+  typedef unsigned uint2_ __attribute__((ext_vector_type(2)));
+  typedef _Float16 half2_ __attribute__((ext_vector_type(2)));
+  constexpr int JG = 2, NG = 2 * TM / JG;
+  const int nl = wn * 64 + 4 * (lane & 15);
+  const int prow = wm * (32 * TM) + 4 * (lane >> 4);
+  int* rowR32 = reinterpret_cast<int*>(smem);
+  IG_CLK(te0);
+  if constexpr (RES) {
+    const int m = FULL || m0 + tid < M ? m0 + tid : M - 1;
+    rowR32[tid] = (int)(ig_row_off(p.res, m) + n0);
+    __syncthreads();
+  }
+  IG_CLK(te1);
+  const float4_ bv = *reinterpret_cast<const float4_*>(bias_lds + nl);
+  const half2_ b01 = {(_Float16)bv[0], (_Float16)bv[1]}, b23 = {(_Float16)bv[2], (_Float16)bv[3]};
+  float4_ sc, sh;
+  if constexpr (HAS_BN) {
+    sc = *reinterpret_cast<const float4_*>(bias_lds + IG_VEC_FLOATS + nl);
+    sh = *reinterpret_cast<const float4_*>(bias_lds + 2 * IG_VEC_FLOATS + nl);
+  }
+  const __amdgpu_buffer_rsrc_t rsY = __builtin_amdgcn_make_buffer_rsrc(ig_uniform_ptr(p.Y), 0, -1, 0x00020000);
+  const __amdgpu_buffer_rsrc_t rsR = __builtin_amdgcn_make_buffer_rsrc(ig_uniform_ptr(p.R), 0, -1, 0x00020000);
+  half4 rv[RES ? 2 : 1][JG * 4];
+  auto res_group = [&](int g) {
+    if constexpr (RES) {
+#pragma unroll
+      for (int jj = 0; jj < JG; ++jj) {
+        const int4_ ro = *reinterpret_cast<const int4_*>(rowR32 + prow + 16 * (g * JG + jj));
+#pragma unroll
+        for (int e = 0; e < 4; ++e)
+          rv[g & 1][jj * 4 + e] = __builtin_bit_cast(half4, __builtin_amdgcn_raw_buffer_load_b64(rsR, (int)((unsigned)(ro[e] + nl) << 1), 0, 0));
+      }
+      __builtin_amdgcn_sched_barrier(0);
+    }
+  };
+  res_group(0);
+#pragma unroll
+  for (int g = 0; g < NG; ++g) {
+    if (g + 1 < NG) res_group(g + 1);
+#pragma unroll
+    for (int jj = 0; jj < JG; ++jj) {
+      const int j = g * JG + jj;
+      const int4_ yo = *reinterpret_cast<const int4_*>(rowY32 + prow + 16 * j);
+#pragma unroll
+      for (int e = 0; e < 4; ++e) {
+        half4 v;
+        half2_ t01 = {(_Float16)acc[0][j][e], (_Float16)acc[1][j][e]};
+        half2_ t23 = {(_Float16)acc[2][j][e], (_Float16)acc[3][j][e]};
+        t01 = t01 + b01;
+        t23 = t23 + b23;
+        if constexpr (HAS_BN) {
+          v[0] = (_Float16)fmaf((float)t01[0], sc[0], sh[0]);
+          v[1] = (_Float16)fmaf((float)t01[1], sc[1], sh[1]);
+          v[2] = (_Float16)fmaf((float)t23[0], sc[2], sh[2]);
+          v[3] = (_Float16)fmaf((float)t23[1], sc[3], sh[3]);
+        } else {
+          v[0] = t01[0]; v[1] = t01[1]; v[2] = t23[0]; v[3] = t23[1];
+        }
+        if constexpr (RES) v = v + rv[g & 1][jj * 4 + e];
+        v = ig_relu4(v);
+        if (FULL || yo[e] != IG_ROW_NONE)
+          __builtin_amdgcn_raw_buffer_store_b64(__builtin_bit_cast(uint2_, v), rsY, (int)((unsigned)(yo[e] + nl) << 1), 0, 0);
+      }
+    }
+    __builtin_amdgcn_sched_barrier(0);
+  }
+#ifdef FP_PROFILE_BUILD
+  IG_CLK(te2);
+  if (tid == 0) { atomicAdd(&ig_epi_dbg[5], te1 - te0); atomicAdd(&ig_epi_dbg[6], te2 - te1); atomicAdd(&ig_epi_dbg[7], 1ull); }
+#endif
+}
+
 template <int BM, int BN, int TM, int THREADS, int DBG, bool FULL, bool SLIM, int EPI = 0, typename Acc, typename P>
 __device__ __forceinline__ void ig_epilogue_body(const P& p, Acc& acc, unsigned char* smem, int m0, int n0,
                                                  int wm, int wn, int tid, int lane, const float* bias_lds) {
diff --git a/foundationpose_amd/engine.py b/foundationpose_amd/engine.py
--- a/foundationpose_amd/engine.py
+++ b/foundationpose_amd/engine.py
@@ -21,6 +21,7 @@
 FUSED_TAIL = True
 CONV_MFMA_16X16X32 = True
 SPECIALIZED_EPILOGUE = True
+CONV_DIRECT_STORE = True
 
 
 def _conv_backend():
@@ -127,15 +128,15 @@
         return F.layer_norm(x + ff, (x.shape[-1],), self.n2[0], self.n2[1], 1e-5)
 
 
-def _conv_params(sd, conv_p, bn_p):
+def _conv_params(sd, conv_p, bn_p, second_output=False):
     w = sd[conv_p + ".weight"].float()
     b = sd.get(conv_p + ".bias")
     scale, shift = _bn_affine(sd, bn_p)
     wk = w.permute(0, 2, 3, 1).reshape(w.shape[0], -1).to(torch.float16).contiguous()
-    tiles = None
+    tiles, direct = None, bool(CONV_DIRECT_STORE and CONV_MFMA_16X16X32 and SPECIALIZED_EPILOGUE and b is not None and not second_output)
     if wk.is_cuda and w.shape[2] == 3 and w.shape[3] == 3 and w.shape[0] % 128 == 0 and w.shape[1] % 32 == 0 and PACKED_CONV_TILES:
-        tiles = ops.pack_conv3x3_tiles(wk, w.shape[0], w.shape[1])
-    return dict(w=wk, w_tiles=tiles, bias=None if b is None else _r16(b.float()), scale=scale, shift=shift)
+        tiles = (ops.pack_conv3x3_tiles_direct if direct else ops.pack_conv3x3_tiles)(wk, w.shape[0], w.shape[1])
+    return dict(w=wk, w_tiles=tiles, tiles_direct=direct and tiles is not None, bias=None if b is None else _r16(b.float()), scale=scale, shift=shift)
 
 
 SPLITK_MAX_HYPS = 12
@@ -143,7 +144,7 @@
 SPLITK_TARGET_WGS = 384
 SMALL_CALL_CEILING = 31
 
-_SWITCHES = ("FUSED_OUT_PROJ_LN", "FUSED_FFN", "ROWS_QKV", "PACKED_CONV_TILES", "MERGED_HEAD_QKV", "FUSED_TAIL", "CONV_MFMA_16X16X32", "SPECIALIZED_EPILOGUE", "SPLITK_MAX_HYPS", "HEADS_TWO_STREAMS_MAX_HYPS")
+_SWITCHES = ("FUSED_OUT_PROJ_LN", "FUSED_FFN", "ROWS_QKV", "PACKED_CONV_TILES", "MERGED_HEAD_QKV", "FUSED_TAIL", "CONV_MFMA_16X16X32", "SPECIALIZED_EPILOGUE", "CONV_DIRECT_STORE", "SPLITK_MAX_HYPS", "HEADS_TWO_STREAMS_MAX_HYPS")
 
 
 @contextlib.contextmanager
@@ -185,7 +186,7 @@
                          ("j3", joint + ".3"), ("j4", joint + ".4")):
             names += [(blk + "a", pre + ".conv1", pre + ".bn1"), (blk + "b", pre + ".conv2", pre + ".bn2")]
         names.append(("j2", joint + ".2.net.0", joint + ".2.net.1"))
-        self.w = {k: _conv_params(sd, c, b) for k, c, b in names}
+        self.w = {k: _conv_params(sd, c, b, second_output=(k == "j4b")) for k, c, b in names}
         self.pe = sd["pos_embed.pe"].float().reshape(-1, sd["pos_embed.pe"].shape[-1]).contiguous()
         self.device = device
         self._bufs = {}
@@ -225,7 +226,7 @@
                                         conv_rounding=True, pe=pe, y_pe=y_pe)
         return ops.igemm_f16(x, gin, c["w"], c["bias"], y, gout, Bn * Ho * Wo, Cout, Cin, 9, relu=relu, residual=res, r_geom=gres,
                              bn_scale=c["scale"], bn_shift=c["shift"], conv_rounding=True, pe=pe, y_pe=y_pe,
-                             w_tiles=c["w_tiles"] if stride == 1 else None)
+                             w_tiles=c["w_tiles"] if stride == 1 else None, w_tiles_direct=c["tiles_direct"] and stride == 1)
 
     def __call__(self, AB, slot=0, shared_b=False, small_calls=True):
         n2, _, H, W = AB.shape
diff --git a/foundationpose_amd/ops.py b/foundationpose_amd/ops.py
--- a/foundationpose_amd/ops.py
+++ b/foundationpose_amd/ops.py
@@ -1136,6 +1136,8 @@
 IGEMM_MFMA_16X16X32 = 16
 IGEMM_MFMA_32X32X16 = 32
 IGEMM_EPILOGUE_GENERIC = 64
+IGEMM_DIRECT_STORE = 256
+IGEMM_W_TILES_DIRECT = 512
 
 
 class IgemmEpilogue(C.Structure):
@@ -1148,6 +1150,13 @@
     w = _dev(w, torch.float16, "w")
     out = torch.empty_like(w)
     _lib.check(_lib.lib().fp_pack_conv3x3_tiles_f16(_ptr(w), _ptr(out), int(N), int(Cin), _stream(w)), "fp_pack_conv3x3_tiles_f16")
+    return out
+
+
+def pack_conv3x3_tiles_direct(w, N, Cin):
+    w = _dev(w, torch.float16, "w")
+    out = torch.empty_like(w)
+    _lib.check(_lib.lib().fp_pack_conv3x3_tiles_direct_f16(_ptr(w), _ptr(out), int(N), int(Cin), _stream(w)), "fp_pack_conv3x3_tiles_direct_f16")
     return out
 
 
@@ -1164,15 +1173,18 @@
 
 
 def igemm_f16(x, x_geom, w, bias, y, y_geom, M, N, Cin, taps, relu=False, residual=None, r_geom=None, bn_scale=None,
-              bn_shift=None, conv_rounding=False, pe=None, y_pe=None, w_tiles=None, mfma16=None):
+              bn_shift=None, conv_rounding=False, pe=None, y_pe=None, w_tiles=None, mfma16=None, direct_store=None, w_tiles_direct=False):
     x = _dev(x, torch.float16, "x"); w = _dev(w, torch.float16, "w"); y = _dev(y, torch.float16, "y")
     from . import engine
     if mfma16 is None:
         mfma16 = engine.CONV_MFMA_16X16X32
+    if direct_store is None:
+        direct_store = engine.CONV_DIRECT_STORE and (w_tiles is None or bool(w_tiles_direct))
     ep = _igemm_epilogue(bias, residual, r_geom, bn_scale, bn_shift, pe, y_pe,
                          (IGEMM_RELU if relu else 0) | (IGEMM_ROUND_ACC if conv_rounding else 0) | IGEMM_HAS_W_TILES |
                          (IGEMM_MFMA_16X16X32 if mfma16 else IGEMM_MFMA_32X32X16) |
-                         (0 if engine.SPECIALIZED_EPILOGUE else IGEMM_EPILOGUE_GENERIC), w_tiles)
+                         (0 if engine.SPECIALIZED_EPILOGUE else IGEMM_EPILOGUE_GENERIC) |
+                         (IGEMM_DIRECT_STORE if direct_store else 0) | (IGEMM_W_TILES_DIRECT if w_tiles_direct else 0), w_tiles)
     st = _lib.lib().fp_igemm_f16_fwd(_ptr(x), C.byref(x_geom), _ptr(w), _ptr(y), C.byref(y_geom), int(M), int(N), int(Cin),
                                      int(taps), C.byref(ep), _stream(x))
     _lib.check(st, "fp_igemm_f16_fwd")
diff --git a/include/fp_amd.h b/include/fp_amd.h
--- a/include/fp_amd.h
+++ b/include/fp_amd.h
@@ -36,7 +36,7 @@
 typedef struct fp_mesh_set fp_mesh_set;
 
 const char* fp_last_error(void);
-#define FP_AMD_ABI_VERSION 226
+#define FP_AMD_ABI_VERSION 227
 int fp_version(void);
 
 int fp_mesh_create(const float* pos , const float* nrm , const int32_t* faces ,
@@ -195,6 +195,9 @@
 
 #define FP_IGEMM_EPILOGUE_GENERIC 64
 
+#define FP_IGEMM_DIRECT_STORE 256
+#define FP_IGEMM_W_TILES_DIRECT 512
+
 typedef struct {
   const float* bias;
   const float* bn_scale;
@@ -213,6 +216,7 @@
                      const fp_igemm_epilogue* epilogue , void* stream);
 
 int fp_pack_conv3x3_tiles_f16(const void* w , void* w_tiles , int N, int Cin, void* stream);
+int fp_pack_conv3x3_tiles_direct_f16(const void* w , void* w_tiles , int N, int Cin, void* stream);
 int fp_conv3x3_sw_lds_bytes(void);
 
 size_t fp_igemm_splitk_workspace_bytes(int M, int N, int splits);
```

New measurement: 8169, median of 6. 1.02x the previous value.
